# StarsX/RayTracedGGX

Hardware: AMD Instinct MI355X
Metric: Mrays/s + ms/frame, bunny 1920x1080 1spp+denoise, 1/2/4/8 GPUs (higher is better)
Workload: dtype f32; 1 GPU; configs[1]: bunny.obj + rnl_cross env, 1920x1080, 1spp GGX reflection + full denoise chain (refl H,V; diff H,V, shared-memory variant; temporal; tone map), all-metal default materials, dt=1/60; parallelism=row strips x1, history_apron_rows=18, history_overreach_rows=0, setup_priming_frames=256, trace_workgroup_waves=12

## Files before the change

### include/rtggx.h

```cpp
#ifndef RTGGX_H
#define RTGGX_H

#include <stddef.h>
#include <stdint.h>

#ifdef __cplusplus
extern "C" {
#endif

typedef struct rtggx_context rtggx_context;

enum { RTGGX_GROUND = 0, RTGGX_MODEL_OBJ = 1, RTGGX_NUM_MESH = 2 };

typedef struct RtggxCBGlobal {
  float    WorldViewProjs[2][16];
  float    WorldViewProjsPrev[2][16];
  float    Worlds[2][12];
  float    WorldITs0[12];
  float    WorldIT1[11];
  uint32_t FrameIndex;
} RtggxCBGlobal;
typedef struct RtggxRayGenConstants {
  float ProjToWorld[16];
  float EyePt[4];
  float ProjBias[2];
  float pad[2];
} RtggxRayGenConstants;
typedef struct RtggxCBPerObject {
  float WorldViewProj[16];
  float ProjBias[2];
  float pad[2];
} RtggxCBPerObject;
typedef struct RtggxCBMaterial {
  float BaseColors[2][4];
  float RoughMetals[2][4];
} RtggxCBMaterial;
typedef struct RtggxFrameConstants {
  RtggxCBGlobal        global;
  RtggxRayGenConstants rayGen;
  RtggxCBPerObject     perObject[2];
  RtggxCBMaterial      material;
} RtggxFrameConstants;

enum { RTGGX_FORMAT_RGBA32F = 2, RTGGX_FORMAT_RGBA16F = 10, RTGGX_FORMAT_BC6H_UF16 = 95, RTGGX_FORMAT_BC6H_SF16 = 96 };

enum {
  RTGGX_BUF_VISIBILITY = 0,
  RTGGX_BUF_DEPTH = 1,
  RTGGX_BUF_NORMAL = 2,
  RTGGX_BUF_ROUGH_METAL = 3,
  RTGGX_BUF_VELOCITY = 4,
  RTGGX_BUF_RT_REFL = 5,
  RTGGX_BUF_RT_DIFF = 6,
  RTGGX_BUF_TSS0 = 7,
  RTGGX_BUF_TSS1 = 8,
  RTGGX_BUF_FLT_RFL = 9,
  RTGGX_BUF_FLT_DFF = 10,
  RTGGX_BUF_BACKBUFFER = 11,
  RTGGX_BUF_SH_COEFFS = 12,
  RTGGX_BUF_BVH_NODES0 = 13,
  RTGGX_BUF_BVH_TRIS0 = 14,
  RTGGX_BUF_BVH_NODES1 = 15,
  RTGGX_BUF_BVH_TRIS1 = 16,
  RTGGX_BUF_TLAS = 17,
  RTGGX_BUF_ENV = 18,
  RTGGX_BUF_BVH4_NODES0 = 19,
  RTGGX_BUF_BVH4_NODES1 = 20,
  RTGGX_BUF_BIN_WORK = 21,
  RTGGX_BUF_BVH4_TOP0 = 22,
  RTGGX_BUF_BVH4_TOP1 = 23,
  RTGGX_BUF_EXCHANGE_TOKENS = 24,
  RTGGX_BUF_ACC_REFL = 25,
  RTGGX_BUF_ACC_DIFF = 26,
  RTGGX_BUF_CONVERGED = 27,
  RTGGX_BUF_COUNT = 28
};

typedef struct RtggxTimings {
  float update_as, visibility, ray_trace, spatial_refl_h, spatial_refl_v, spatial_diff_h, spatial_diff_v,
        temporal, tone_map, frame,
        ray_trace_kernel;
} RtggxTimings;

const char* rtggx_last_error(void);

int  rtggx_create(rtggx_context** out, uint32_t width, uint32_t height, int device);
void rtggx_destroy(rtggx_context* ctx);

int  rtggx_set_strip(rtggx_context* ctx, uint32_t row_begin, uint32_t row_end);

int  rtggx_set_history_apron(rtggx_context* ctx, uint32_t rows);
int  rtggx_history_overreach(rtggx_context* ctx, uint32_t* rows, int reset);

int  rtggx_set_stream(rtggx_context* ctx, void* hip_stream);
int  rtggx_get_stream(rtggx_context* ctx, void** hip_stream);
#define RTGGX_MAX_PEERS 16
#define RTGGX_IPC_HANDLE_BYTES 64
int  rtggx_set_history_peers(rtggx_context* ctx, uint32_t world, const uint32_t* bounds, void* const* tss0, void* const* tss1);
int  rtggx_history_ipc_export(rtggx_context* ctx, void* handles, size_t bytes);
int  rtggx_history_ipc_open(rtggx_context* ctx, const void* handles, size_t bytes, void** tss0, void** tss1);

int  rtggx_set_async_compute(rtggx_context* ctx, int enable);

int  rtggx_set_mesh(rtggx_context* ctx, uint32_t slot, const float* verts, uint32_t num_verts,
                    const uint32_t* indices, uint32_t num_indices);
int  rtggx_set_env(rtggx_context* ctx, int format, uint32_t size, uint32_t mips, const void* data, size_t bytes);
enum { RTGGX_ENV_EQUIRECT = 0, RTGGX_ENV_VCROSS = 1, RTGGX_ENV_HCROSS = 2 };
enum { RTGGX_PIXELS_RGBE8 = 0, RTGGX_PIXELS_RGB32F = 1 };
int  rtggx_set_env_image(rtggx_context* ctx, int layout, int pixels, uint32_t width, uint32_t height, const void* data, size_t bytes,
                         uint32_t cube_size);
int  rtggx_generate_env_mips(rtggx_context* ctx);
int  rtggx_set_material(rtggx_context* ctx, uint32_t mesh, const float base_color[4], float roughness, float metallic);
int  rtggx_set_metallic(rtggx_context* ctx, uint32_t mesh, float metallic);
int  rtggx_set_sampler(rtggx_context* ctx, int vndf);
int  rtggx_set_ray_rate(rtggx_context* ctx, uint32_t pixels_per_ray);
#define RTGGX_MAX_RECURSION_DEPTH 4u
int  rtggx_set_max_recursion_depth(rtggx_context* ctx, uint32_t depth);
#define RTGGX_MAX_SAMPLES_PER_PIXEL 8u
int  rtggx_set_samples_per_pixel(rtggx_context* ctx, uint32_t samples);
#define RTGGX_MIN_SAMPLE_SET 256u
#define RTGGX_MAX_SAMPLE_SET 65536u
int  rtggx_set_sample_set(rtggx_context* ctx, uint32_t size);
int  rtggx_set_accumulation(rtggx_context* ctx, int enable);
int  rtggx_reset_accumulation(rtggx_context* ctx);
int  rtggx_accumulated_frames(rtggx_context* ctx, uint32_t* frames);
int  rtggx_present_accumulation(rtggx_context* ctx);

typedef struct RtggxScore {
  uint64_t index;
  uint32_t frame_index;
  uint32_t pad;
  uint64_t pixels, covered;
  uint64_t skipped_out, skipped_raw;
  double se_out_rgb, se_out_luma;
  double se_raw_rgb, se_raw_luma;
  double ref_rgb2, ref_luma2;
  double se_out_rgb_cov, se_raw_rgb_cov, ref_rgb2_cov;
} RtggxScore;
enum { RTGGX_SCORE_RING = 256 };
int  rtggx_set_reference(rtggx_context* ctx, const void* rgba16f, size_t bytes);
int  rtggx_reference_from_accumulation(rtggx_context* ctx);
int  rtggx_set_scoring(rtggx_context* ctx, int enable);
int  rtggx_read_scores(rtggx_context* ctx, RtggxScore* out, uint32_t capacity, uint32_t* count);

int  rtggx_build_as(rtggx_context* ctx);

int  rtggx_refit_as(rtggx_context* ctx, uint32_t slot, const float* verts, uint32_t num_verts);
int  rtggx_refit_as_device(rtggx_context* ctx, uint32_t slot, const float* device_verts, uint32_t num_verts, void* hip_stream);
int  rtggx_set_refit_policy(rtggx_context* ctx, float rebuild_ratio, uint32_t steps_per_frame);
int  rtggx_refit_stats(rtggx_context* ctx, uint32_t slot, float* cost_ratio, uint32_t* refits, uint32_t* rebuilds);

int  rtggx_update_frame(rtggx_context* ctx, const RtggxFrameConstants* constants);
int  rtggx_update_as(rtggx_context* ctx);
int  rtggx_transform_sh(rtggx_context* ctx);
int  rtggx_render_visibility(rtggx_context* ctx);
int  rtggx_ray_trace(rtggx_context* ctx);
int  rtggx_denoise(rtggx_context* ctx, int use_shared_mem);
int  rtggx_tone_map(rtggx_context* ctx);

int  rtggx_debug_fuse_tone_map(rtggx_context* ctx, int mode);
int  rtggx_debug_placement(rtggx_context* ctx, int force_small, uint32_t* key, uint32_t* where);
int  rtggx_debug_tile_words(rtggx_context* ctx, int enable);
int  rtggx_debug_static_sky(rtggx_context* ctx, int enable);
int  rtggx_debug_sky_runs(rtggx_context* ctx, uint32_t* runs, uint32_t capacity, uint32_t* tiles_x, uint32_t* tiles_y, uint32_t* threshold);
int  rtggx_debug_collapse_weights(rtggx_context* ctx, const float* set, float* get);
int  rtggx_debug_fence_wait(rtggx_context* ctx, double* us_total, uint32_t* waits, int reset);

int  rtggx_sync(rtggx_context* ctx);
int  rtggx_ray_count(rtggx_context* ctx, uint64_t* rays);
int  rtggx_ray_total(rtggx_context* ctx, uint64_t* rays, int reset);
int  rtggx_debug_counters(rtggx_context* ctx, uint32_t* out, uint32_t n, int reset);
int  rtggx_debug_trace_split(rtggx_context* ctx, uint32_t work_per_wave, uint32_t max_shift, int capacity, uint32_t* last_demand);
int  rtggx_debug_trace_residency(rtggx_context* ctx, uint32_t force_waves, uint32_t* waves, float* share);
int  rtggx_debug_environment(rtggx_context* ctx, const float* dirs3, const float* levels, uint32_t n, int level0_path, float* rgb3);
int  rtggx_get_timings(rtggx_context* ctx, RtggxTimings* out);
#define RTGGX_KERNEL_RING 4096
int  rtggx_enable_timing(rtggx_context* ctx, int mode);
int  rtggx_kernel_times(rtggx_context* ctx, float* ms, uint32_t capacity, uint32_t* count);

int  rtggx_debug_shader_clock(rtggx_context* ctx, double* mhz);

int  rtggx_copy_bandwidth(rtggx_context* ctx, size_t bytes, int iterations, double* gbytes_per_s);

int  rtggx_buffer_size(rtggx_context* ctx, int buffer_id, size_t* bytes);
int  rtggx_readback(rtggx_context* ctx, int buffer_id, void* dst, size_t bytes);
int  rtggx_buffer_ptr(rtggx_context* ctx, int buffer_id, void** device_ptr);
int  rtggx_upload(rtggx_context* ctx, int buffer_id, const void* src, size_t bytes);
int  rtggx_frame_parity(rtggx_context* ctx, uint32_t* parity);
int  rtggx_bvh_root(rtggx_context* ctx, uint32_t slot, int32_t* root);

int  rtggx_trace_rays(rtggx_context* ctx, const float* rays, uint32_t n, float* out);

#ifdef __cplusplus
}
#endif
#endif
```

### raytracedggx_amd/capi.py

```python
import ctypes as C
import os

import numpy as np

_HERE = os.path.dirname(os.path.abspath(__file__))
LIB_PATH = os.path.join(_HERE, "librtggx.so")

BUF_VISIBILITY, BUF_DEPTH, BUF_NORMAL, BUF_ROUGH_METAL, BUF_VELOCITY, BUF_RT_REFL, BUF_RT_DIFF, BUF_TSS0, BUF_TSS1, \
    BUF_FLT_RFL, BUF_FLT_DFF, BUF_BACKBUFFER, BUF_SH_COEFFS, BUF_BVH_NODES0, BUF_BVH_TRIS0, BUF_BVH_NODES1, BUF_BVH_TRIS1, \
    BUF_TLAS, BUF_ENV, BUF_BVH4_NODES0, BUF_BVH4_NODES1, BUF_BIN_WORK, BUF_BVH4_TOP0, BUF_BVH4_TOP1, BUF_EXCHANGE_TOKENS, \
    BUF_ACC_REFL, BUF_ACC_DIFF, BUF_CONVERGED = range(28)
MAX_PEERS, IPC_HANDLE_BYTES = 16, 64
FORMAT_RGBA32F, FORMAT_RGBA16F, FORMAT_BC6H_UF16, FORMAT_BC6H_SF16 = 2, 10, 95, 96
ENV_EQUIRECT, ENV_VCROSS, ENV_HCROSS = 0, 1, 2
PIXELS_RGBE8, PIXELS_RGB32F = 0, 1

_BUF_DTYPE = {BUF_VISIBILITY: np.uint32, BUF_DEPTH: np.uint32, BUF_NORMAL: np.uint32, BUF_ROUGH_METAL: np.uint16,
              BUF_VELOCITY: np.uint32, BUF_RT_REFL: np.uint32, BUF_RT_DIFF: np.uint32, BUF_TSS0: np.uint64, BUF_TSS1: np.uint64,
              BUF_FLT_RFL: np.uint64, BUF_FLT_DFF: np.uint64, BUF_BACKBUFFER: np.uint32, BUF_SH_COEFFS: np.float32,
              BUF_BVH_NODES0: np.uint32, BUF_BVH_TRIS0: np.uint32, BUF_BVH_NODES1: np.uint32, BUF_BVH_TRIS1: np.uint32,
              BUF_TLAS: np.float32, BUF_ENV: np.uint16, BUF_BVH4_NODES0: np.uint32, BUF_BVH4_NODES1: np.uint32, BUF_BIN_WORK: np.uint32,
              BUF_BVH4_TOP0: np.uint32, BUF_BVH4_TOP1: np.uint32, BUF_EXCHANGE_TOKENS: np.uint32,
              BUF_ACC_REFL: np.float32, BUF_ACC_DIFF: np.float32, BUF_CONVERGED: np.uint64}

EXPORTS = ["rtggx_last_error", "rtggx_create", "rtggx_destroy", "rtggx_set_strip", "rtggx_set_stream", "rtggx_set_mesh",
           "rtggx_set_env", "rtggx_set_material", "rtggx_set_metallic", "rtggx_build_as", "rtggx_update_frame", "rtggx_update_as",
           "rtggx_transform_sh", "rtggx_render_visibility", "rtggx_ray_trace", "rtggx_denoise", "rtggx_tone_map", "rtggx_sync",
           "rtggx_ray_count", "rtggx_get_timings", "rtggx_enable_timing", "rtggx_buffer_size", "rtggx_readback", "rtggx_buffer_ptr",
           "rtggx_upload", "rtggx_frame_parity", "rtggx_bvh_root", "rtggx_trace_rays", "rtggx_ray_total", "rtggx_kernel_times", "rtggx_debug_counters", "rtggx_debug_trace_split", "rtggx_debug_trace_residency", "rtggx_get_stream", "rtggx_set_history_peers", "rtggx_history_ipc_export", "rtggx_history_ipc_open",
           "rtggx_set_async_compute", "rtggx_set_history_apron", "rtggx_history_overreach", "rtggx_copy_bandwidth", "rtggx_refit_as", "rtggx_refit_as_device", "rtggx_refit_stats", "rtggx_set_refit_policy", "rtggx_set_sampler", "rtggx_set_ray_rate", "rtggx_set_max_recursion_depth", "rtggx_set_samples_per_pixel", "rtggx_debug_fuse_tone_map", "rtggx_debug_placement", "rtggx_debug_tile_words", "rtggx_debug_static_sky", "rtggx_debug_sky_runs", "rtggx_debug_collapse_weights", "rtggx_debug_fence_wait", "rtggx_debug_shader_clock", "rtggx_debug_environment",
           "rtggx_set_accumulation", "rtggx_reset_accumulation", "rtggx_accumulated_frames", "rtggx_present_accumulation", "rtggx_set_sample_set",
           "rtggx_set_reference", "rtggx_reference_from_accumulation", "rtggx_set_scoring", "rtggx_read_scores",
           "rtggx_set_env_image", "rtggx_generate_env_mips"]
SCORE_RING = 256


class Timings(C.Structure):
    _fields_ = [(n, C.c_float) for n in ("update_as", "visibility", "ray_trace", "spatial_refl_h", "spatial_refl_v",
                                         "spatial_diff_h", "spatial_diff_v", "temporal", "tone_map", "frame", "ray_trace_kernel")]


class Score(C.Structure):
    _fields_ = [("index", C.c_uint64), ("frame_index", C.c_uint32), ("pad", C.c_uint32), ("pixels", C.c_uint64), ("covered", C.c_uint64),
                ("skipped_out", C.c_uint64), ("skipped_raw", C.c_uint64)] + \
               [(n, C.c_double) for n in ("se_out_rgb", "se_out_luma", "se_raw_rgb", "se_raw_luma", "ref_rgb2", "ref_luma2",
                                          "se_out_rgb_cov", "se_raw_rgb_cov", "ref_rgb2_cov")]

    def as_dict(self):
        return {n: getattr(self, n) for n, _ in self._fields_ if n != "pad"}


_lib = None


def load():
    global _lib
    if _lib is not None:
        return _lib
    if not os.path.exists(LIB_PATH):
        raise ImportError("librtggx.so is not built: run `python -c 'import __graft_entry__ as g; g.build()'` "
                          "or `make -C raytracedggx_amd` (hipcc, gfx950). There is no CPU path.")
    L = C.CDLL(LIB_PATH)
    L.rtggx_last_error.restype = C.c_char_p
    vp = C.c_void_p
    L.rtggx_create.argtypes = [C.POINTER(vp), C.c_uint32, C.c_uint32, C.c_int]
    L.rtggx_destroy.argtypes = [vp]
    L.rtggx_destroy.restype = None
    L.rtggx_set_strip.argtypes = [vp, C.c_uint32, C.c_uint32]
    L.rtggx_set_stream.argtypes = [vp, vp]
    L.rtggx_set_async_compute.argtypes = [vp, C.c_int]
    L.rtggx_set_ray_rate.argtypes = [vp, C.c_uint32]
    L.rtggx_set_max_recursion_depth.argtypes = [vp, C.c_uint32]
    L.rtggx_set_samples_per_pixel.argtypes = [vp, C.c_uint32]
    L.rtggx_set_sample_set.argtypes = [vp, C.c_uint32]
    L.rtggx_set_accumulation.argtypes = [vp, C.c_int]
    L.rtggx_reset_accumulation.argtypes = [vp]
    L.rtggx_accumulated_frames.argtypes = [vp, C.POINTER(C.c_uint32)]
    L.rtggx_present_accumulation.argtypes = [vp]
    L.rtggx_set_reference.argtypes = [vp, vp, C.c_size_t]
    L.rtggx_reference_from_accumulation.argtypes = [vp]
    L.rtggx_set_scoring.argtypes = [vp, C.c_int]
    L.rtggx_read_scores.argtypes = [vp, C.POINTER(Score), C.c_uint32, C.POINTER(C.c_uint32)]
    L.rtggx_set_history_apron.argtypes = [vp, C.c_uint32]
    L.rtggx_debug_shader_clock.argtypes = [vp, C.POINTER(C.c_double)]
    L.rtggx_refit_as.argtypes = [vp, C.c_uint32, vp, C.c_uint32]
    L.rtggx_set_refit_policy.argtypes = [vp, C.c_float, C.c_uint32]
    L.rtggx_refit_stats.argtypes = [vp, C.c_uint32, C.POINTER(C.c_float), C.POINTER(C.c_uint32), C.POINTER(C.c_uint32)]
    L.rtggx_copy_bandwidth.argtypes = [vp, C.c_size_t, C.c_int, C.POINTER(C.c_double)]
    L.rtggx_history_overreach.argtypes = [vp, C.POINTER(C.c_uint32), C.c_int]
    L.rtggx_set_mesh.argtypes = [vp, C.c_uint32, vp, C.c_uint32, vp, C.c_uint32]
    L.rtggx_set_env.argtypes = [vp, C.c_int, C.c_uint32, C.c_uint32, vp, C.c_size_t]
    L.rtggx_set_env_image.argtypes = [vp, C.c_int, C.c_int, C.c_uint32, C.c_uint32, vp, C.c_size_t, C.c_uint32]
    L.rtggx_generate_env_mips.argtypes = [vp]
    L.rtggx_set_material.argtypes = [vp, C.c_uint32, vp, C.c_float, C.c_float]
    L.rtggx_set_metallic.argtypes = [vp, C.c_uint32, C.c_float]
    for n in ("rtggx_build_as", "rtggx_update_as", "rtggx_transform_sh", "rtggx_render_visibility", "rtggx_ray_trace",
              "rtggx_tone_map", "rtggx_sync"):
        getattr(L, n).argtypes = [vp]
    L.rtggx_update_frame.argtypes = [vp, vp]
    L.rtggx_denoise.argtypes = [vp, C.c_int]
    L.rtggx_ray_count.argtypes = [vp, C.POINTER(C.c_uint64)]
    L.rtggx_get_timings.argtypes = [vp, C.POINTER(Timings)]
    L.rtggx_enable_timing.argtypes = [vp, C.c_int]
    L.rtggx_buffer_size.argtypes = [vp, C.c_int, C.POINTER(C.c_size_t)]
    L.rtggx_readback.argtypes = [vp, C.c_int, vp, C.c_size_t]
    L.rtggx_buffer_ptr.argtypes = [vp, C.c_int, C.POINTER(vp)]
    L.rtggx_upload.argtypes = [vp, C.c_int, vp, C.c_size_t]
    L.rtggx_frame_parity.argtypes = [vp, C.POINTER(C.c_uint32)]
    L.rtggx_bvh_root.argtypes = [vp, C.c_uint32, C.POINTER(C.c_int32)]
    L.rtggx_trace_rays.argtypes = [vp, vp, C.c_uint32, vp]
    L.rtggx_ray_total.argtypes = [vp, C.POINTER(C.c_uint64), C.c_int]
    L.rtggx_kernel_times.argtypes = [vp, vp, C.c_uint32, C.POINTER(C.c_uint32)]
    _lib = L
    return L


class RtggxError(RuntimeError):
    pass


def _p(a):
    return a.ctypes.data_as(C.c_void_p)


class Context:

    def __init__(self, width, height, device=0):
        self.L = load()
        self.W, self.H = int(width), int(height)
        h = C.c_void_p()
        self._check(self.L.rtggx_create(C.byref(h), self.W, self.H, int(device)))
        self.h = h

    def _check(self, rc):
        if rc != 0:
            raise RtggxError("librtggx: %s (code %d)" % (self.L.rtggx_last_error().decode(), rc))

    def close(self):
        if getattr(self, "h", None):
            self.L.rtggx_destroy(self.h)
            self.h = None

    def __del__(self):
        try:
            self.close()
        except Exception:
            pass

    def set_strip(self, row_begin, row_end):
        self._check(self.L.rtggx_set_strip(self.h, row_begin, row_end))

    def set_stream(self, stream_handle):
        self._check(self.L.rtggx_set_stream(self.h, C.c_void_p(stream_handle)))

    def shader_clock_mhz(self):
        m = C.c_double()
        self._check(self.L.rtggx_debug_shader_clock(self.h, C.byref(m)))
        return m.value

    def copy_bandwidth(self, nbytes=1 << 30, iterations=8):
        g = C.c_double()
        self._check(self.L.rtggx_copy_bandwidth(self.h, int(nbytes), int(iterations), C.byref(g)))
        return g.value

    def set_history_apron(self, rows):
        self._check(self.L.rtggx_set_history_apron(self.h, int(rows)))

    def history_overreach(self, reset=True):
        n = C.c_uint32()
        self._check(self.L.rtggx_history_overreach(self.h, C.byref(n), int(reset)))
        return n.value

    def set_async_compute(self, enable):
        self._check(self.L.rtggx_set_async_compute(self.h, int(bool(enable))))

    def set_mesh(self, slot, verts, indices):
        v = np.ascontiguousarray(verts, np.float32).reshape(-1, 6)
        i = np.ascontiguousarray(indices, np.uint32).reshape(-1)
        self._check(self.L.rtggx_set_mesh(self.h, slot, _p(v), v.shape[0], _p(i), i.size))

    def refit_as(self, slot, verts):
        v = np.ascontiguousarray(verts, np.float32).reshape(-1, 6)
        self._check(self.L.rtggx_refit_as(self.h, slot, _p(v), v.shape[0]))

    def refit_as_device(self, slot, device_ptr, num_verts, stream=0):
        self.L.rtggx_refit_as_device.argtypes = [C.c_void_p, C.c_uint32, C.c_void_p, C.c_uint32, C.c_void_p]
        self._check(self.L.rtggx_refit_as_device(self.h, slot, C.c_void_p(int(device_ptr)), int(num_verts), C.c_void_p(int(stream) or None)))

    def fence_wait(self, reset=True):
        us, n = C.c_double(0.0), C.c_uint32(0)
        self.L.rtggx_debug_fence_wait.argtypes = [C.c_void_p, C.POINTER(C.c_double), C.POINTER(C.c_uint32), C.c_int]
        self._check(self.L.rtggx_debug_fence_wait(self.h, C.byref(us), C.byref(n), 1 if reset else 0))
        return us.value, n.value

    def fuse_tone_map(self, mode):
        self._check(self.L.rtggx_debug_fuse_tone_map(self.h, -1 if mode is None else 1 if mode else 0))

    def tile_words(self, enable):
        self._check(self.L.rtggx_debug_tile_words(self.h, 1 if enable else 0))

    def static_sky(self, enable):
        self._check(self.L.rtggx_debug_static_sky(self.h, 1 if enable else 0))

    def sky_runs(self):
        tiles = ((self.W + 15) // 16) * ((self.H + 15) // 16 + 1)
        runs = np.zeros(tiles, np.uint32)
        tx, ty, th = C.c_uint32(), C.c_uint32(), C.c_uint32()
        self.L.rtggx_debug_sky_runs.argtypes = [C.c_void_p, C.c_void_p, C.c_uint32, C.c_void_p, C.c_void_p, C.c_void_p]
        self._check(self.L.rtggx_debug_sky_runs(self.h, _p(runs), tiles, C.byref(tx), C.byref(ty), C.byref(th)))
        return runs[:tx.value * ty.value].reshape(ty.value, tx.value), int(th.value)

    def placement(self, force_small=-1):
        k, w = C.c_uint32(), C.c_uint32()
        self.L.rtggx_debug_placement.argtypes = [C.c_void_p, C.c_int, C.c_void_p, C.c_void_p]
        self._check(self.L.rtggx_debug_placement(self.h, int(force_small), C.byref(k), C.byref(w)))
        names = ("main", "B", "C", "R", "?")
        key = {n: bool((k.value >> i) & 1) for i, n in enumerate(("small", "strip", "deforming", "diffuse", "caller_stream"))}
        where = {"raster": names[(w.value >> 16) & 15], "gen": names[w.value & 15], "trace": names[(w.value >> 4) & 15], "shade": names[(w.value >> 8) & 15], "frames_in_flight": (w.value >> 12) & 15}
        return key, where

    def collapse_weights(self, area=None, tris=None):
        self.L.rtggx_debug_collapse_weights.argtypes = [C.c_void_p, C.c_void_p, C.c_void_p]
        get = (C.c_float * 2)()
        if area is not None:
            st = (C.c_float * 2)(float(area), float(tris))
            self._check(self.L.rtggx_debug_collapse_weights(self.h, st, get))
        else:
            self._check(self.L.rtggx_debug_collapse_weights(self.h, None, get))
        return float(get[0]), float(get[1])

    def set_history_peers(self, bounds, tss0, tss1):
        self.L.rtggx_set_history_peers.argtypes = [C.c_void_p, C.c_uint32, C.c_void_p, C.c_void_p, C.c_void_p]
        if bounds is None:
            self._check(self.L.rtggx_set_history_peers(self.h, 0, None, None, None))
            return
        world = len(bounds) - 1
        b = (C.c_uint32 * (world + 1))(*[int(x) for x in bounds])
        p0 = (C.c_void_p * world)(*[C.c_void_p(int(x) or None) for x in tss0])
        p1 = (C.c_void_p * world)(*[C.c_void_p(int(x) or None) for x in tss1])
        self._check(self.L.rtggx_set_history_peers(self.h, world, b, p0, p1))

    def history_ipc_export(self):
        self.L.rtggx_history_ipc_export.argtypes = [C.c_void_p, C.c_void_p, C.c_size_t]
        buf = C.create_string_buffer(2 * IPC_HANDLE_BYTES)
        self._check(self.L.rtggx_history_ipc_export(self.h, buf, len(buf.raw)))
        return bytes(buf.raw)

    def history_ipc_open(self, handles):
        self.L.rtggx_history_ipc_open.argtypes = [C.c_void_p, C.c_char_p, C.c_size_t, C.c_void_p, C.c_void_p]
        p0, p1 = C.c_void_p(), C.c_void_p()
        self._check(self.L.rtggx_history_ipc_open(self.h, bytes(handles), len(handles), C.byref(p0), C.byref(p1)))
        return int(p0.value), int(p1.value)

    def set_sampler(self, vndf):
        self._check(self.L.rtggx_set_sampler(self.h, 1 if vndf else 0))

    def set_ray_rate(self, pixels_per_ray):
        self._check(self.L.rtggx_set_ray_rate(self.h, int(pixels_per_ray)))

    def set_max_recursion_depth(self, depth):
        self._check(self.L.rtggx_set_max_recursion_depth(self.h, int(depth)))

    def set_samples_per_pixel(self, samples):
        self._check(self.L.rtggx_set_samples_per_pixel(self.h, int(samples)))

    def set_sample_set(self, size):
        self._check(self.L.rtggx_set_sample_set(self.h, int(size)))

    def set_accumulation(self, enable):
        self._check(self.L.rtggx_set_accumulation(self.h, 1 if enable else 0))

    def reset_accumulation(self):
        self._check(self.L.rtggx_reset_accumulation(self.h))

    def accumulated_frames(self):
        n = C.c_uint32()
        self._check(self.L.rtggx_accumulated_frames(self.h, C.byref(n)))
        return int(n.value)

    def present_accumulation(self):
        self._check(self.L.rtggx_present_accumulation(self.h))

    def set_reference(self, rgba16f):
        if rgba16f is None:
            self._check(self.L.rtggx_set_reference(self.h, None, 0))
            return
        a = np.ascontiguousarray(rgba16f)
        self._check(self.L.rtggx_set_reference(self.h, _p(a), a.nbytes))

    def reference_from_accumulation(self):
        self._check(self.L.rtggx_reference_from_accumulation(self.h))

    def set_scoring(self, enable):
        self._check(self.L.rtggx_set_scoring(self.h, 1 if enable else 0))

    def read_scores(self, capacity=None):
        out = []
        while capacity is None or len(out) < capacity:
            room = SCORE_RING if capacity is None else min(SCORE_RING, capacity - len(out))
            buf, n = (Score * room)(), C.c_uint32()
            self._check(self.L.rtggx_read_scores(self.h, buf, room, C.byref(n)))
            out += [buf[i].as_dict() for i in range(n.value)]
            if n.value < room:
                break
        return out

    def set_refit_policy(self, rebuild_ratio=1.2, steps_per_frame=16):
        self._check(self.L.rtggx_set_refit_policy(self.h, rebuild_ratio, steps_per_frame))

    def refit_stats(self, slot=1):
        ratio, refits, rebuilds = C.c_float(), C.c_uint32(), C.c_uint32()
        self._check(self.L.rtggx_refit_stats(self.h, slot, C.byref(ratio), C.byref(refits), C.byref(rebuilds)))
        return {"cost_ratio": ratio.value, "refits": refits.value, "rebuilds": rebuilds.value}

    def set_env(self, fmt, size, mips, data):
        b = np.frombuffer(bytes(data), np.uint8) if not isinstance(data, np.ndarray) else np.ascontiguousarray(data).view(np.uint8).reshape(-1)
        self._check(self.L.rtggx_set_env(self.h, fmt, size, mips, _p(b), b.size))

    def set_env_image(self, layout, pixels, width, height, data, cube_size=0):
        if data is None:
            self._check(self.L.rtggx_set_env_image(self.h, int(layout), int(pixels), int(width), int(height), None, 0, int(cube_size)))
            return
        b = np.frombuffer(bytes(data), np.uint8) if not isinstance(data, np.ndarray) else np.ascontiguousarray(data).view(np.uint8).reshape(-1)
        self._check(self.L.rtggx_set_env_image(self.h, int(layout), int(pixels), int(width), int(height), _p(b), b.size, int(cube_size)))

    def generate_env_mips(self):
        self._check(self.L.rtggx_generate_env_mips(self.h))

    def set_material(self, mesh, base_color, roughness, metallic):
        bc = np.asarray(base_color, np.float32)
        self._check(self.L.rtggx_set_material(self.h, mesh, _p(bc), roughness, metallic))

    def set_metallic(self, mesh, metallic):
        self._check(self.L.rtggx_set_metallic(self.h, mesh, metallic))

    def build_as(self):
        self._check(self.L.rtggx_build_as(self.h))

    def update_frame(self, constants768):
        b = np.frombuffer(bytes(constants768), np.uint8).copy()
        if b.size != 768:
            raise ValueError("RtggxFrameConstants is 768 bytes")
        self._check(self.L.rtggx_update_frame(self.h, _p(b)))

    def update_as(self):
        self._check(self.L.rtggx_update_as(self.h))

    def transform_sh(self):
        self._check(self.L.rtggx_transform_sh(self.h))

    def render_visibility(self):
        self._check(self.L.rtggx_render_visibility(self.h))

    def ray_trace(self):
        self._check(self.L.rtggx_ray_trace(self.h))

    def denoise(self, use_shared_mem=False):
        self._check(self.L.rtggx_denoise(self.h, 1 if use_shared_mem else 0))

    def tone_map(self):
        self._check(self.L.rtggx_tone_map(self.h))

    def sync(self):
        self._check(self.L.rtggx_sync(self.h))

    def ray_count(self):
        n = C.c_uint64()
        self._check(self.L.rtggx_ray_count(self.h, C.byref(n)))
        return int(n.value)

    def ray_total(self, reset=False):
        n = C.c_uint64()
        self._check(self.L.rtggx_ray_total(self.h, C.byref(n), 1 if reset else 0))
        return int(n.value)

    def debug_trace_split(self, work_per_wave, max_shift, capacity=-1):
        d = C.c_uint32()
        self.L.rtggx_debug_trace_split.argtypes = [C.c_void_p, C.c_uint32, C.c_uint32, C.c_int, C.c_void_p]
        self._check(self.L.rtggx_debug_trace_split(self.h, work_per_wave, max_shift, capacity, C.byref(d)))
        return int(d.value)

    def stream(self):
        h = C.c_void_p()
        self.L.rtggx_get_stream.argtypes = [C.c_void_p, C.c_void_p]
        self._check(self.L.rtggx_get_stream(self.h, C.byref(h)))
        return int(h.value or 0)

    def trace_residency(self, force_waves=0):
        w, sh = C.c_uint32(), C.c_float()
        self.L.rtggx_debug_trace_residency.argtypes = [C.c_void_p, C.c_uint32, C.c_void_p, C.c_void_p]
        self._check(self.L.rtggx_debug_trace_residency(self.h, force_waves, C.byref(w), C.byref(sh)))
        return int(w.value), float(sh.value)

    def debug_counters(self, n=8, reset=True):
        out = np.zeros(n, np.uint32)
        self.L.rtggx_debug_counters.argtypes = [C.c_void_p, C.c_void_p, C.c_uint32, C.c_int]
        self._check(self.L.rtggx_debug_counters(self.h, _p(out), n, 1 if reset else 0))
        return out

    def debug_environment(self, dirs, levels, level0=False):
        d = np.ascontiguousarray(dirs, np.float32).reshape(-1, 3)
        lv = np.ascontiguousarray(np.broadcast_to(np.asarray(levels, np.float32), (d.shape[0],)))
        out = np.zeros((d.shape[0], 3), np.float32)
        self.L.rtggx_debug_environment.argtypes = [C.c_void_p, C.c_void_p, C.c_void_p, C.c_uint32, C.c_int, C.c_void_p]
        self._check(self.L.rtggx_debug_environment(self.h, _p(d), _p(lv), d.shape[0], 1 if level0 else 0, _p(out)))
        return out

    def enable_timing(self, mode=1):
        self._check(self.L.rtggx_enable_timing(self.h, int(mode)))

    def kernel_times(self):
        ms = np.zeros(4096, np.float32)
        n = C.c_uint32()
        self._check(self.L.rtggx_kernel_times(self.h, _p(ms), ms.size, C.byref(n)))
        return ms[:n.value].copy()

    def timings(self):
        t = Timings()
        self._check(self.L.rtggx_get_timings(self.h, C.byref(t)))
        return {n: getattr(t, n) for n, _ in Timings._fields_}

    def buffer_size(self, bid):
        n = C.c_size_t()
        self._check(self.L.rtggx_buffer_size(self.h, bid, C.byref(n)))
        return int(n.value)

    def buffer_ptr(self, bid):
        p = C.c_void_p()
        self._check(self.L.rtggx_buffer_ptr(self.h, bid, C.byref(p)))
        return int(p.value)

    def readback(self, bid):
        n = self.buffer_size(bid)
        dt = np.dtype(_BUF_DTYPE[bid])
        out = np.zeros(max(n // dt.itemsize, 0), dt)
        if n:
            self._check(self.L.rtggx_readback(self.h, bid, _p(out), n))
        if bid <= BUF_BACKBUFFER or bid == BUF_CONVERGED:
            return out.reshape(self.H, self.W)
        if bid in (BUF_ACC_REFL, BUF_ACC_DIFF):
            return out.reshape(self.H, self.W, 4)
        if bid == BUF_SH_COEFFS:
            return out.reshape(9, 3)
        if bid in (BUF_BVH_NODES0, BUF_BVH_NODES1):
            return out.reshape(-1, 16)
        if bid in (BUF_BVH_TRIS0, BUF_BVH_TRIS1):
            return out.reshape(-1, 16)
        if bid == BUF_TLAS:
            return out.reshape(2, 4, 4)
        if bid == BUF_ENV:
            return out.reshape(-1, 4)
        if bid in (BUF_BVH4_NODES0, BUF_BVH4_NODES1, BUF_BVH4_TOP0, BUF_BVH4_TOP1):
            return out.reshape(-1, 32)
        return out

    def upload(self, bid, array):
        a = np.ascontiguousarray(array)
        self._check(self.L.rtggx_upload(self.h, bid, _p(a), a.nbytes))

    def frame_parity(self):
        p = C.c_uint32()
        self._check(self.L.rtggx_frame_parity(self.h, C.byref(p)))
        return int(p.value)

    def bvh_root(self, slot):
        r = C.c_int32()
        self._check(self.L.rtggx_bvh_root(self.h, slot, C.byref(r)))
        return int(r.value)

    def trace_rays(self, rays):
        r = np.ascontiguousarray(rays, np.float32).reshape(-1, 8)
        out = np.zeros((r.shape[0], 6), np.float32)
        self._check(self.L.rtggx_trace_rays(self.h, _p(r), r.shape[0], _p(out)))
        return {"t": out[:, 0].copy(), "inst": out[:, 1].copy().view(np.uint32), "prim": out[:, 2].copy().view(np.uint32),
                "b1": out[:, 3].copy(), "b2": out[:, 4].copy(), "valid": out[:, 5] > 0.5}
```

### raytracedggx_amd/csrc/context.hip

```cpp
#include <cstdarg>
#include <cstdio>
#include <cstring>
#include <cmath>
#include <vector>
#include "capi_internal.h"
#include "rt_queue.h"

#ifndef RT_REFIT_REBUILD_RATIO
#define RT_REFIT_REBUILD_RATIO 1.2f
#endif
#ifndef RT_REBUILD_STEPS
#define RT_REBUILD_STEPS 16u
#endif
namespace rt {
static thread_local char g_err[512] = "";
void setError(const char* fmt, ...) {
  va_list ap; va_start(ap, fmt); vsnprintf(g_err, sizeof g_err, fmt, ap); va_end(ap);
}

__global__ void uploadParamsKernel(FrameParams src, FrameParams* dst) {
  const uint32_t* s = reinterpret_cast<const uint32_t*>(&src);
  uint32_t* d = reinterpret_cast<uint32_t*>(dst);
  for (uint32_t i = threadIdx.x; i < sizeof(FrameParams) / 4; i += blockDim.x) d[i] = s[i];
}
int uploadParams(rtggx_context* c, uint32_t slot, hipStream_t s) {
  hipLaunchKernelGGL(uploadParamsKernel, dim3(1), dim3(64), 0, s, c->slots[slot], c->dParams + slot);
  RT_HIP(hipGetLastError());
  return 0;
}
int allocSet(rtggx_context* c, uint32_t i) {
  InputSet& s = c->sets[i];
  const size_t n = (size_t)c->W * c->H, slots = (size_t)c->numBinsMax * c->binSlots;
  for (DevBuf<uint32_t>* p : {&s.normal, &s.depth32, &s.velocity, &s.rtRefl, &s.rtDiff}) if (!*p) RT_HIP(allocFilled(*p, n));
  if (!s.roughMetal) RT_HIP(allocFilled(s.roughMetal, n));
  if (!s.rayQueue) RT_HIP(alloc(s.rayQueue, slots * sizeof(rt::RayRec)));
  if (!s.hitQueue) RT_HIP(alloc(s.hitQueue, slots * 8));
  if (!s.binCount) RT_HIP(allocFilled(s.binCount, (size_t)c->numBinsMax));
  if (!s.splitList) RT_HIP(alloc(s.splitList, (size_t)RT_SPLIT_CAP));
  if (!s.skyRun) RT_HIP(allocFilled(s.skyRun, c->skyTiles));
  c->breakSkyRuns();
  s.splitCount = c->largeCountBase + 2 + i;
  if (!s.evRead) RT_HIP(create(s.evRead, RT_EVENT_FLAGS));
  return 0;
}

static int initContext(rtggx_context* c, uint32_t width, uint32_t height, int device) {
  c->device = device; c->W = width; c->H = height; c->rowBegin = 0; c->rowEnd = height;
  const size_t n = (size_t)width * height;
  int prioLeast = 0, prioGreatest = 0;
  RT_HIP(hipDeviceGetStreamPriorityRange(&prioLeast, &prioGreatest));
  const int prioMid = (prioLeast + prioGreatest) / 2;
  RT_HIP(create(c->ownMain, hipStreamNonBlocking, prioGreatest));
  RT_HIP(create(c->ownAS, hipStreamNonBlocking, prioLeast));
  c->streamMain = c->ownMain; c->streamAS = c->ownAS;
  RT_HIP(create(c->ownVis, hipStreamNonBlocking, prioLeast)); c->streamVis = c->ownVis;
  RT_HIP(create(c->streamRefit, hipStreamNonBlocking, prioMid));
  for (Event* e : {&c->evVis, &c->evRefit, &c->evAS, &c->evRT}) RT_HIP(create(*e, RT_EVENT_FLAGS));
  for (auto& f : c->frames) { RT_HIP(create(f.gen, RT_EVENT_FLAGS)); RT_HIP(create(f.trace, RT_EVENT_FLAGS)); }
  for (auto& e : c->tev) RT_HIP(create(e));
  c->rebuildRatio = RT_REFIT_REBUILD_RATIO; c->rebuildSteps = RT_REBUILD_STEPS;
  {
    hipDeviceProp_t prop;
    RT_HIP(hipGetDeviceProperties(&prop, device));
    c->numCUs = prop.multiProcessorCount > 0 ? (uint32_t)prop.multiProcessorCount : 256u;
  }
  c->numBinsMax = ((width + 15) / 16) * ((height + 15) / 16) * 4u;
  if (c->numBinsMax < 64u) c->numBinsMax = 64u;
  c->binSlots = RT_BIN_MIN;
  c->largeCapacity = 1u << 16;
  c->skyTiles = (size_t)((width + 15) / 16) * ((height + 15) / 16 + 1);
  for (auto& b : c->largeTrisBuf) RT_HIP(alloc(b, (size_t)c->largeCapacity * 56));
  RT_HIP(allocFilled(c->largeCountBase, 2 + RT_SETS));
  for (uint32_t i = 0; i < RT_SETS; ++i) { const int r = allocSet(c, i); if (r) return r; }
  for (auto& v : c->vis) { RT_HIP(allocFilled(v.depth, n)); RT_HIP(allocFilled(v.dirty, c->skyTiles, 0xFF)); }
  RT_HIP(allocFilled(c->visDirtyOnes, c->skyTiles, 0xFF));
  RT_HIP(allocFilled(c->backbuffer, n));
  RT_HIP(allocFilled(c->tss[0], n)); RT_HIP(allocFilled(c->tss[1], n)); RT_HIP(allocFilled(c->fltRfl, n)); RT_HIP(allocFilled(c->fltDff, n));
  RT_HIP(allocFilled(c->rayCounter, 512));
  RT_HIP(allocFilled(c->rayCounterBuf, 1792));
  c->lastRayCounter32 = c->rayCounterBuf;
  RT_HIP(allocFilled(c->traceStamps, 8));
  RT_HIP(alloc(c->hostRayCounters, 264)); memset(c->hostRayCounters, 0, 264 * 4); RT_HIP(create(c->evRayCounters, hipEventDisableTiming));
  for (auto& b : c->binWorkBuf) RT_HIP(allocFilled(b, (size_t)c->numBinsMax));
  c->selectSet(0);
  c->splitWork = RT_SPLIT_WORK; c->splitMaxShift = RT_SPLIT_MAX_SHIFT;
  RT_HIP(allocFilled(c->dEnvMipOffset, 16));
  RT_HIP(allocFilled(c->dummyRecord, 128));
  RT_HIP(allocFilled(c->histReach, 1));
  RT_HIP(allocFilled(c->exchangeTokens, 2 * RT_MAX_PEERS));
  RT_HIP(allocFilled(c->dPeerTable, sizeof(void*) * 2 * RT_MAX_PEERS + 4 * (RT_MAX_PEERS + 1)));
  RT_HIP(allocFilled(c->sh, 27));
  RT_HIP(alloc(c->cosSinTab, 512));
  RT_HIP(alloc(c->dParams, RT_SLOTS));
  {
    float tab[512];
    for (int s = 0; s < 256; ++s) { const double phi = 2.0 * 3.14159265358979323846 * (double)s / 256.0; tab[s] = (float)cos(phi); tab[256 + s] = (float)sin(phi); }
    RT_HIP(hipMemcpy(c->cosSinTab, tab, sizeof tab, hipMemcpyHostToDevice));
  }
  const float bc0[4] = {0.95f, 0.93f, 0.88f, 1.0f}, bc1[4] = {1.0f, 0.71f, 0.29f, 1.0f};
  const float rm0[4] = {0.5f, 1.0f, 0.0f, 0.0f}, rm1[4] = {0.16f, 1.0f, 0.0f, 0.0f};
  memcpy(c->material.BaseColors[0], bc0, 16); memcpy(c->material.BaseColors[1], bc1, 16);
  memcpy(c->material.RoughMetals[0], rm0, 16); memcpy(c->material.RoughMetals[1], rm1, 16);
  memset(c->invWorld, 0, sizeof c->invWorld);
  for (int i = 0; i < 2; ++i) for (int k = 0; k < 4; ++k) c->invWorld[i][k * 5] = 1.0f;
  memset(c->slots, 0, sizeof c->slots);
  { const int r = setMeshImpl(c, RTGGX_GROUND, &kGroundVerts[0][0], 24, kGroundIdx, 36); if (r) return r; }
  RT_HIP(hipStreamSynchronize(nullptr));
  return 0;
}
int allocSamples(rtggx_context* c) {
  if (c->sppAcc && c->sppParams) return 0;
  const size_t n = (size_t)c->W * c->H;
  if (!c->evSpp) RT_HIP(create(c->evSpp, hipEventDisableTiming));
  if (!c->sppParams) RT_HIP(alloc(c->sppParams, RT_SLOTS * RTGGX_MAX_SAMPLES_PER_PIXEL));
  if (!c->sppAcc) {
    RT_HIP(allocFilled(c->sppAcc, n * 2u * 3u));
    RT_HIP(hipStreamSynchronize(nullptr));
  }
  return 0;
}
int allocSampleTable(rtggx_context* c, uint32_t m) {
  DevBuf<float>& tab = c->cosSinWide[rtggx_context::sampleSetSlot(m)];
  if (tab) return 0;
  std::vector<float> host(2u * (size_t)m);
  for (uint32_t s = 0; s < m; ++s) { const double phi = 2.0 * 3.14159265358979323846 * (double)s / (double)m; host[2u * s] = (float)cos(phi); host[2u * s + 1u] = (float)sin(phi); }
  DevBuf<float> d;
  hipError_t e = alloc(d, host.size());
  if (e == hipSuccess) e = hipMemcpy(d, host.data(), host.size() * sizeof(float), hipMemcpyHostToDevice);
  if (e != hipSuccess) { setError("rtggx_set_sample_set: %s (%zu bytes for the table of %u samples)", hipGetErrorString(e), host.size() * sizeof(float), m); return -2; }
  tab = std::move(d);
  return 0;
}
int allocAccumulation(rtggx_context* c) {
  if (c->accRefl) return 0;
  const size_t n = (size_t)c->W * c->H;
  DevBuf<float4> a0, a1; DevBuf<uint2> cv;
  hipError_t e = alloc(a0, n);
  if (e == hipSuccess) e = alloc(a1, n);
  if (e == hipSuccess) e = alloc(cv, n);
  if (e == hipSuccess) e = hipMemset(a0, 0, n * 16);
  if (e == hipSuccess) e = hipMemset(a1, 0, n * 16);
  if (e == hipSuccess) e = hipMemset(cv, 0, n * 8);
  if (e == hipSuccess) e = hipStreamSynchronize(nullptr);
  if (e != hipSuccess) { setError("rtggx_set_accumulation: %s (%zu bytes for the sums and the mean image)", hipGetErrorString(e), n * 40); return -2; }
  c->accRefl = std::move(a0); c->accDiff = std::move(a1); c->converged = std::move(cv);
  return 0;
}
static int allocReference(rtggx_context* c, const char* who) {
  if (c->reference) return 0;
  const size_t n = (size_t)c->W * c->H;
  const hipError_t e = alloc(c->reference, n);
  if (e != hipSuccess) { setError("%s: %s (%zu bytes for the reference image)", who, hipGetErrorString(e), n * 8); return -2; }
  return 0;
}
static int allocScoring(rtggx_context* c) {
  if (c->scoreRing) return 0;
  const size_t chunks = ((size_t)c->W * c->H + RT_SCORE_CHUNK - 1u) / RT_SCORE_CHUNK;
  uint32_t stride = 1u; while (stride < chunks) stride <<= 1;
  const size_t half = stride > 1u ? stride / 2u : 1u;
  DevBuf<double> p0, p1; DevBuf<uint32_t> counts; DevBuf<RtggxScore> ring;
  hipError_t e = alloc(p0, (size_t)RT_SCORE_SUMS * stride);
  if (e == hipSuccess) e = alloc(p1, (size_t)RT_SCORE_SUMS * half);
  if (e == hipSuccess) e = alloc(counts, 3u * (size_t)stride);
  if (e == hipSuccess) e = allocFilled(ring, RTGGX_SCORE_RING);
  if (e == hipSuccess) e = hipStreamSynchronize(nullptr);
  if (e != hipSuccess) { setError("rtggx_set_scoring: %s (the ring of records and the partial sums)", hipGetErrorString(e)); return -2; }
  c->scorePartial[0] = std::move(p0); c->scorePartial[1] = std::move(p1); c->scoreCounts = std::move(counts); c->scoreRing = std::move(ring); c->scoreStride = stride;
  return 0;
}
}
using namespace rt;

extern "C" {
const char* rtggx_last_error(void) { return rt::g_err; }

int rtggx_create(rtggx_context** out, uint32_t width, uint32_t height, int device) {
  if (!out || width == 0 || height == 0 || width > 16384 || height > 16384) { setError("rtggx_create: bad arguments"); return -1; }
  int count = 0;
  if (hipGetDeviceCount(&count) != hipSuccess || count <= 0) { setError("rtggx_create: no HIP device available (this library has no CPU path)"); return -2; }
  if (device < 0 || device >= count) { setError("rtggx_create: device %d out of range (%d devices)", device, count); return -1; }
  RT_HIP(hipSetDevice(device));
  rtggx_context* c = new rtggx_context();
  const int r = initContext(c, width, height, device);
  if (r) { rtggx_destroy(c); return r; }
  *out = c;
  return 0;
}

void rtggx_destroy(rtggx_context* c) {
  if (!c) return;
  hipSetDevice(c->device);
  hipDeviceSynchronize();
  delete c;
}

int rtggx_set_strip(rtggx_context* c, uint32_t rowBegin, uint32_t rowEnd) {
  RT_CHECK_CTX(c);
  if (rowBegin > rowEnd || rowEnd > c->H) { setError("rtggx_set_strip: bad rows [%u,%u) for height %u", rowBegin, rowEnd, c->H); return -1; }
  if (c->rayRate != 1u && (rowBegin > 0u || rowEnd < c->H)) { setError("rtggx_set_strip: rows [%u,%u) of %u: a context tracing one pixel in %u renders whole frames", rowBegin, rowEnd, c->H, c->rayRate); return -1; }
  c->rowBegin = rowBegin; c->rowEnd = rowEnd; c->toneMapDone = false;
  c->breakSkyRuns();
  return 0;
}

int rtggx_set_history_apron(rtggx_context* c, uint32_t rows) {
  RT_CHECK_CTX(c);
  c->historyApron = rows;
  return 0;
}
int rtggx_history_overreach(rtggx_context* c, uint32_t* rows, int reset) {
  RT_CHECK_CTX(c);
  if (!rows) { setError("rtggx_history_overreach: null result"); return -1; }
  RT_HIP(syncStreams(c));
  RT_HIP(hipMemcpy(rows, c->histReach, 4, hipMemcpyDeviceToHost));
  if (reset) { RT_HIP(hipMemset(c->histReach, 0, 4)); RT_HIP(hipStreamSynchronize(nullptr)); }
  return 0;
}

int rtggx_set_stream(rtggx_context* c, void* stream) {
  RT_CHECK_CTX(c);
  RT_HIP(syncStreams(c));
  if (stream) { c->streamMain = (hipStream_t)stream; c->externalStream = true; }
  else { c->streamMain = c->ownMain; c->externalStream = false; }
  c->sppStream = nullptr;
  if (!c->asyncCompute) c->streamAS = c->streamMain;
  return 0;
}

int rtggx_set_history_peers(rtggx_context* c, uint32_t world, const uint32_t* bounds, void* const* tss0, void* const* tss1) {
  RT_CHECK_CTX(c);
  if (world == 0u) { RT_HIP(syncStreams(c)); c->peerWorld = 0u; return 0; }
  if (world > RT_MAX_PEERS || !bounds || !tss0 || !tss1) { setError("rtggx_set_history_peers: 1 .. %d ranks, boundaries and two pointer lists", RT_MAX_PEERS); return -1; }
  if (bounds[0] != 0u || bounds[world] != c->H) { setError("rtggx_set_history_peers: boundaries must run from 0 to the frame height %u", c->H); return -1; }
  for (uint32_t r = 0; r < world; ++r) if (bounds[r] > bounds[r + 1]) { setError("rtggx_set_history_peers: boundaries must ascend"); return -1; }
  RT_HIP(syncStreams(c));
  struct { const void* tss[2][RT_MAX_PEERS]; uint32_t bounds[RT_MAX_PEERS + 1]; } table;
  memset(&table, 0, sizeof table);
  for (uint32_t r = 0; r < world; ++r) {
    const bool own = bounds[r] <= c->rowBegin && c->rowEnd <= bounds[r + 1] && c->rowEnd > c->rowBegin;
    table.tss[0][r] = tss0[r] ? tss0[r] : own ? (void*)c->tss[0] : nullptr; table.tss[1][r] = tss1[r] ? tss1[r] : own ? (void*)c->tss[1] : nullptr;
    if (bounds[r + 1] > bounds[r] && (!table.tss[0][r] || !table.tss[1][r])) { setError("rtggx_set_history_peers: no history images for rank %u", r); return -1; }
  }
  for (uint32_t r = 0; r <= world; ++r) table.bounds[r] = bounds[r];
  for (uint32_t r = world + 1; r <= RT_MAX_PEERS; ++r) table.bounds[r] = c->H;
  static_assert(sizeof table == sizeof(void*) * 2 * RT_MAX_PEERS + 4 * (RT_MAX_PEERS + 1) + 4 || sizeof table == sizeof(void*) * 2 * RT_MAX_PEERS + 4 * (RT_MAX_PEERS + 1), "peer table layout");
  RT_HIP(hipMemcpy(c->dPeerTable, &table, sizeof(void*) * 2 * RT_MAX_PEERS + 4 * (RT_MAX_PEERS + 1), hipMemcpyHostToDevice));
  c->peerWorld = world;
  return 0;
}
int rtggx_history_ipc_export(rtggx_context* c, void* handles, size_t bytes) {
  RT_CHECK_CTX(c);
  static_assert(sizeof(hipIpcMemHandle_t) == RTGGX_IPC_HANDLE_BYTES, "hipIpcMemHandle_t size");
  if (!handles || bytes < 2 * sizeof(hipIpcMemHandle_t)) { setError("rtggx_history_ipc_export: room for two %zu-byte handles", sizeof(hipIpcMemHandle_t)); return -1; }
  hipIpcMemHandle_t h[2];
  for (int p = 0; p < 2; ++p) RT_HIP(hipIpcGetMemHandle(&h[p], c->tss[p]));
  memcpy(handles, h, sizeof h);
  return 0;
}
int rtggx_history_ipc_open(rtggx_context* c, const void* handles, size_t bytes, void** tss0, void** tss1) {
  RT_CHECK_CTX(c);
  if (!handles || bytes < 2 * sizeof(hipIpcMemHandle_t) || !tss0 || !tss1) { setError("rtggx_history_ipc_open: bad arguments"); return -1; }
  hipIpcMemHandle_t h[2]; memcpy(h, handles, sizeof h);
  void* p[2] = {nullptr, nullptr};
  for (int k = 0; k < 2; ++k) {
    IpcMapping mapped;
    RT_HIP(hipIpcOpenMemHandle(mapped.put(), h[k], hipIpcMemLazyEnablePeerAccess));
    p[k] = mapped;
    c->ipcMapped.push_back(std::move(mapped));
  }
  *tss0 = p[0]; *tss1 = p[1];
  return 0;
}

int rtggx_get_stream(rtggx_context* c, void** stream) {
  RT_CHECK_CTX(c);
  if (!stream) { setError("rtggx_get_stream: null"); return -1; }
  *stream = (void*)c->streamMain;
  return 0;
}

int rtggx_set_async_compute(rtggx_context* c, int enable) {
  RT_CHECK_CTX(c);
  if ((enable != 0) == c->asyncCompute) return 0;
  RT_HIP(syncStreams(c));
  c->asyncCompute = enable != 0; c->sppStream = nullptr;
  c->streamAS = c->asyncCompute ? c->ownAS : c->streamMain;
  c->streamVis = c->asyncCompute ? c->ownVis : nullptr;
  c->evVisStream = nullptr; for (auto& f : c->frames) f.genFrame = 0u;
  return 0;
}

int rtggx_set_ray_rate(rtggx_context* c, uint32_t pixelsPerRay) {
  RT_CHECK_CTX(c);
  if (pixelsPerRay != 1u && pixelsPerRay != 4u) { setError("rtggx_set_ray_rate: %u pixels per ray: 1 or 4", pixelsPerRay); return -1; }
  if (pixelsPerRay != 1u && c->samplesRequested > 1u) { setError("rtggx_set_ray_rate: rate %u on a context tracing %u samples per pixel (rtggx_set_samples_per_pixel): one asks for fewer rays, the other for more", pixelsPerRay, c->samplesRequested); return -1; }
  if (pixelsPerRay != 1u && c->accumulateRequested) { setError("rtggx_set_ray_rate: rate %u on an accumulating context (rtggx_set_accumulation): three quarters of such a frame are interpolations", pixelsPerRay); return -1; }
  if (pixelsPerRay != 1u && (c->rowBegin > 0u || c->rowEnd < c->H)) { setError("rtggx_set_ray_rate: rate %u on a strip (rows [%u,%u) of %u): whole frames only", pixelsPerRay, c->rowBegin, c->rowEnd, c->H); return -1; }
  if (pixelsPerRay == c->rayRate) return 0;
  RT_HIP(syncStreams(c));
  c->rayRate = pixelsPerRay;
  for (auto& b : c->binWorkBuf) RT_HIP(hipMemset(b, 0, (size_t)c->numBinsMax * 4));
  RT_HIP(hipDeviceSynchronize());
  c->splitDemand = 0u; c->rayCountersInFlight = false; c->lastFrameRays = 0xFFFFFFFFu; c->traceLaunches = 0u;
  return 0;
}

int rtggx_set_max_recursion_depth(rtggx_context* c, uint32_t depth) {
  RT_CHECK_CTX(c);
  if (depth < 1u || depth > RTGGX_MAX_RECURSION_DEPTH) { setError("rtggx_set_max_recursion_depth: depth %u: 1 to %u", depth, RTGGX_MAX_RECURSION_DEPTH); return -1; }
  c->depthRequested = depth;
  return 0;
}

int rtggx_set_samples_per_pixel(rtggx_context* c, uint32_t samples) {
  RT_CHECK_CTX(c);
  if (samples != 1u && samples != 2u && samples != 4u && samples != 8u) { setError("rtggx_set_samples_per_pixel: %u samples per pixel: 1, 2, 4 or %u", samples, RTGGX_MAX_SAMPLES_PER_PIXEL); return -1; }
  if (samples > 1u && c->rayRate != 1u) { setError("rtggx_set_samples_per_pixel: %u samples per pixel on a context tracing one pixel in %u (rtggx_set_ray_rate): one asks for more rays, the other for fewer", samples, c->rayRate); return -1; }
  if (samples > 1u) { const int r = allocSamples(c); if (r) return r; }
  c->samplesRequested = samples;
  return 0;
}

int rtggx_set_sample_set(rtggx_context* c, uint32_t size) {
  RT_CHECK_CTX(c);
  if (size < RTGGX_MIN_SAMPLE_SET || size > RTGGX_MAX_SAMPLE_SET || (size & (size - 1u)) != 0u) { setError("rtggx_set_sample_set: %u samples: a power of two from %u to %u", size, RTGGX_MIN_SAMPLE_SET, RTGGX_MAX_SAMPLE_SET); return -1; }
  if (size == c->sampleSetRequested) return 0;
  RT_HIP(syncStreams(c));
  if (size > RTGGX_MIN_SAMPLE_SET) { const int r = allocSampleTable(c, size); if (r) return r; }
  c->sampleSetRequested = size;
  return 0;
}

int rtggx_set_accumulation(rtggx_context* c, int enable) {
  RT_CHECK_CTX(c);
  if (enable && c->rayRate != 1u) { setError("rtggx_set_accumulation: on a context tracing one pixel in %u (rtggx_set_ray_rate): three quarters of such a frame are interpolations", c->rayRate); return -1; }
  if (enable) { const int r = allocAccumulation(c); if (r) return r; }
  c->accumulateRequested = enable != 0;
  return 0;
}
int rtggx_reset_accumulation(rtggx_context* c) {
  RT_CHECK_CTX(c);
  if (c->accRefl) {
    const size_t n = (size_t)c->W * c->H;
    RT_HIP(hipMemsetAsync(c->accRefl, 0, n * 16, c->streamMain));
    RT_HIP(hipMemsetAsync(c->accDiff, 0, n * 16, c->streamMain));
  }
  c->accumFrames = 0u;
  return 0;
}
int rtggx_accumulated_frames(rtggx_context* c, uint32_t* frames) {
  RT_CHECK_CTX(c);
  if (!frames) { setError("rtggx_accumulated_frames: null result"); return -1; }
  *frames = c->accumFrames;
  return 0;
}
int rtggx_present_accumulation(rtggx_context* c) {
  RT_CHECK_CTX(c);
  if (!c->accRefl) { setError("rtggx_present_accumulation: accumulation was never enabled (rtggx_set_accumulation)"); return -1; }
  if (c->rowBegin > 0u || c->rowEnd < c->H) { setError("rtggx_present_accumulation: on a strip (rows [%u,%u) of %u): whole frames only", c->rowBegin, c->rowEnd, c->H); return -1; }
  if (c->accumFrames == 0u) { setError("rtggx_present_accumulation: no frame has been accumulated"); return -1; }
  FrameParams fp = c->slots[c->slot];
  fp.W = c->W; fp.H = c->H; fp.rowBegin = 0u; fp.rowEnd = c->H;
  int r = launchPresentAccumulation(c, c->streamMain);
  if (!r) r = launchToneMap(c, fp, c->streamMain, nullptr, c->converged);
  c->toneMapDone = false;
  return r;
}

int rtggx_set_reference(rtggx_context* c, const void* rgba16f, size_t bytes) {
  RT_CHECK_CTX(c);
  const size_t want = (size_t)c->W * c->H * 8u;
  if (!rgba16f && bytes == 0u) {
    RT_HIP(syncStreams(c));
    c->reference.reset();
    c->scoring = c->scoringRequested = false;
    return 0;
  }
  if (!rgba16f || bytes != want) { setError("rtggx_set_reference: %zu bytes for a %u x %u RGBA16F image of %zu", bytes, c->W, c->H, want); return -1; }
// ... 106 lines not shown
```

### raytracedggx_amd/csrc/debug.hip

```cpp
#include <cstring>
#include "capi_internal.h"
#include "rt_queue.h"
namespace rt {
__global__ void __launch_bounds__(256) copyKernel(const float4* __restrict__ src, float4* __restrict__ dst, size_t n) {
  for (size_t i = (size_t)blockIdx.x * 256u + threadIdx.x; i < n; i += (size_t)gridDim.x * 256u) dst[i] = src[i];
}
typedef float __attribute__((ext_vector_type(4))) CopyVec4;
__global__ void __launch_bounds__(256) copyKernelNT(const CopyVec4* __restrict__ src, CopyVec4* __restrict__ dst, size_t n) {
  for (size_t i = (size_t)blockIdx.x * 256u + threadIdx.x; i < n; i += (size_t)gridDim.x * 256u) __builtin_nontemporal_store(__builtin_nontemporal_load(&src[i]), &dst[i]);
}
}
using namespace rt;

extern "C" {
int rtggx_ray_count(rtggx_context* c, uint64_t* rays) {
  RT_CHECK_CTX(c);
  uint32_t h[256];
  RT_HIP(syncStreams(c));
  RT_HIP(hipMemcpy(h, c->lastRayCounter32, sizeof h, hipMemcpyDeviceToHost));
  uint64_t s = 0; for (auto v : h) s += v;
  *rays = s;
  return 0;
}

int rtggx_debug_counters(rtggx_context* c, uint32_t* out, uint32_t n, int reset) {
  RT_CHECK_CTX(c);
  if (n > 768) { setError("rtggx_debug_counters: at most 768 words"); return -1; }
  RT_HIP(syncStreams(c));
  RT_HIP(hipMemcpy(out, c->rayCounterBuf + 1024, (size_t)n * 4, hipMemcpyDeviceToHost));
  if (reset) { RT_HIP(hipMemset(c->rayCounterBuf + 1024, 0, 768 * 4)); RT_HIP(hipStreamSynchronize(nullptr)); }
  return 0;
}

int rtggx_debug_fence_wait(rtggx_context* c, double* usTotal, uint32_t* waits, int reset) {
  RT_CHECK_CTX(c);
  if (usTotal) *usTotal = c->fenceWaitUs;
  if (waits) *waits = c->fenceWaits;
  if (reset) { c->fenceWaitUs = 0.0; c->fenceWaits = 0u; }
  return 0;
}
int rtggx_debug_fuse_tone_map(rtggx_context* c, int mode) {
  RT_CHECK_CTX(c);
  c->fuseToneMap = mode < 0 ? -1 : mode != 0;
  return 0;
}
int rtggx_debug_tile_words(rtggx_context* c, int enable) {
  RT_CHECK_CTX(c);
  c->useTileWords = enable != 0;
  c->breakSkyRuns();
  return 0;
}
int rtggx_debug_static_sky(rtggx_context* c, int enable) {
  RT_CHECK_CTX(c);
  c->staticSky = enable != 0;
  c->breakSkyRuns();
  return 0;
}
int rtggx_debug_sky_runs(rtggx_context* c, uint32_t* runs, uint32_t capacity, uint32_t* tilesX, uint32_t* tilesY, uint32_t* threshold) {
  RT_CHECK_CTX(c);
  const uint32_t n = c->skyGen.tilesX * c->skyGen.tilesY;
  if (!runs || capacity < n || n > c->skyTiles) { setError("rtggx_debug_sky_runs: room for %u words", n); return -1; }
  RT_HIP(syncStreams(c));
  if (n) RT_HIP(hipMemcpy(runs, c->cur().skyRun, (size_t)n * 4, hipMemcpyDeviceToHost));
  for (uint32_t i = 0; i < n; ++i) runs[i] = (runs[i] >> 8) == c->skyEpoch ? runs[i] & 0xFFu : 0u;
  if (tilesX) *tilesX = c->skyGen.tilesX;
  if (tilesY) *tilesY = c->skyGen.tilesY;
  if (threshold) *threshold = RT_SKY_PREV_RUN + 1u;
  return 0;
}
int rtggx_debug_placement(rtggx_context* c, int forceSmall, uint32_t* key, uint32_t* where) {
  RT_CHECK_CTX(c);
  if (forceSmall < -1 || forceSmall > 1) { setError("rtggx_debug_placement: force_small is -1, 0 or 1"); return -1; }
  c->forcePlacement = forceSmall;
  if (forceSmall >= 0) c->lastTraceSmall = forceSmall == 1;
  if (key) *key = c->lastPlacement[0];
  if (where) *where = c->lastPlacement[1];
  return 0;
}
int rtggx_debug_collapse_weights(rtggx_context* c, const float* set, float* get) {
  RT_CHECK_CTX(c);
  if (set) { if (!(set[0] >= 0.0f) || !(set[1] >= 0.0f) || !(set[0] + set[1] > 0.0f)) { setError("rtggx_debug_collapse_weights: two non-negative weights, not both zero"); return -1; }
             c->collapseWeights[0] = set[0]; c->collapseWeights[1] = set[1]; }
  if (get) { get[0] = c->collapseWeights[0]; get[1] = c->collapseWeights[1]; }
  return 0;
}
int rtggx_debug_trace_residency(rtggx_context* c, uint32_t forceWaves, uint32_t* waves, float* share) {
  RT_CHECK_CTX(c);
  if (forceWaves != 0u && forceWaves != 10u && forceWaves != 12u && forceWaves != 14u && forceWaves != 16u) { setError("rtggx_debug_trace_residency: %u waves: 0, 10, 12, 14 or 16", forceWaves); return -1; }
  c->traceWavesForced = forceWaves;
  if (forceWaves) c->traceWaves = forceWaves;
  if (waves) *waves = c->traceWaves;
  if (share) *share = c->traceShare;
  return 0;
}

int rtggx_debug_environment(rtggx_context* c, const float* dirs3, const float* levels, uint32_t n, int level0Path, float* rgb3) {
  RT_CHECK_CTX(c);
  if (!c->env.texels) { setError("rtggx_debug_environment: no environment map"); return -1; }
  if (n == 0 || !dirs3 || !rgb3 || (!levels && !level0Path)) { setError("rtggx_debug_environment: no directions, levels or result (n %u)", n); return -1; }
  DevBuf<float> dD, dL, dO;
  hipError_t e = alloc(dD, (size_t)n * 3);
  if (e == hipSuccess) e = alloc(dO, (size_t)n * 3);
  if (e == hipSuccess && levels) e = alloc(dL, (size_t)n);
  if (e == hipSuccess) e = hipMemcpy(dD, dirs3, (size_t)n * 12, hipMemcpyHostToDevice);
  if (e == hipSuccess && levels) e = hipMemcpy(dL, levels, (size_t)n * 4, hipMemcpyHostToDevice);
  int r = 0;
  if (e == hipSuccess) r = launchDebugEnvironment(c, dD, dL, n, level0Path, dO, c->streamMain);
  if (e == hipSuccess && !r) e = hipStreamSynchronize(c->streamMain);
  if (e == hipSuccess && !r) e = hipMemcpy(rgb3, dO, (size_t)n * 12, hipMemcpyDeviceToHost);
  if (e != hipSuccess) { setError("rtggx_debug_environment: %s", hipGetErrorString(e)); return -2; }
  return r;
}

int rtggx_debug_trace_split(rtggx_context* c, uint32_t workPerWave, uint32_t maxShift, int capacity, uint32_t* lastDemand) {
  RT_CHECK_CTX(c);
  if (maxShift > 3u) { setError("rtggx_debug_trace_split: max_shift %u > 3", maxShift); return -1; }
  if (capacity > (int)RT_SPLIT_CAP) { setError("rtggx_debug_trace_split: capacity %d > %u", capacity, RT_SPLIT_CAP); return -1; }
  RT_HIP(syncStreams(c));
  if (lastDemand) RT_HIP(hipMemcpy(lastDemand, c->cur().splitCount, 4, hipMemcpyDeviceToHost));
  c->splitWork = workPerWave; c->splitMaxShift = maxShift;
  c->splitCapForced = capacity < 0 ? 0xFFFFFFFFu : ((uint32_t)capacity / 32u) * 32u;
  return 0;
}

int rtggx_ray_total(rtggx_context* c, uint64_t* rays, int reset) {
  RT_CHECK_CTX(c);
  unsigned long long h[256];
  RT_HIP(syncStreams(c));
  RT_HIP(hipMemcpy(h, c->rayCounter + 256, sizeof h, hipMemcpyDeviceToHost));
  uint64_t s = 0; for (auto v : h) s += v;
  *rays = s;
  if (reset) { RT_HIP(hipMemset(c->rayCounter + 256, 0, sizeof h)); RT_HIP(hipStreamSynchronize(nullptr)); }
  return 0;
}

int rtggx_enable_timing(rtggx_context* c, int mode) {
  RT_CHECK_CTX(c);
  c->timing = mode == 1; c->timingsPending = false;
  c->kernelRing = mode == 2 || mode == 3; c->kevCount = 0; c->ringStride = mode == 3 ? 8u : 1u; c->ringTick = 0;
  if (c->kernelRing && c->kevBegin.empty()) {
    c->kevBegin.resize(RTGGX_KERNEL_RING); c->kevEnd.resize(RTGGX_KERNEL_RING);
    for (uint32_t i = 0; i < RTGGX_KERNEL_RING; ++i) { RT_HIP(create(c->kevBegin[i])); RT_HIP(create(c->kevEnd[i])); }
  }
  return 0;
}
int rtggx_kernel_times(rtggx_context* c, float* ms, uint32_t capacity, uint32_t* count) {
  RT_CHECK_CTX(c);
  RT_HIP(syncStreams(c));
  const uint32_t n = c->kevCount < capacity ? c->kevCount : capacity;
  for (uint32_t i = 0; i < n; ++i) RT_HIP(hipEventElapsedTime(&ms[i], c->kevBegin[i], c->kevEnd[i]));
  *count = n;
  c->kevCount = 0;
  return 0;
}
int rtggx_get_timings(rtggx_context* c, RtggxTimings* out) {
  RT_CHECK_CTX(c);
  if (!c->timing || !c->timingsPending) { setError("rtggx_get_timings: timing not enabled or no complete frame"); return -1; }
  RT_HIP(syncStreams(c));
  auto ms = [&](int a, int b) { float t = 0.0f; hipEventElapsedTime(&t, c->tev[a], c->tev[b]); return t; };
  RtggxTimings t;
  t.update_as = ms(0, 1); t.visibility = ms(2, 13); t.ray_trace = ms(3, 14); t.spatial_refl_h = ms(9, 4); t.spatial_refl_v = ms(4, 5);
  t.spatial_diff_h = ms(5, 6); t.spatial_diff_v = ms(6, 7); t.temporal = ms(7, 8); t.tone_map = ms(8, 10); t.frame = ms(2, 10);
  t.ray_trace_kernel = ms(11, 12);
  *out = t;
  return 0;
}

static int bufferInfo(rtggx_context* c, int id, void** ptr, size_t* bytes) {
  const size_t n = (size_t)c->W * c->H;
  switch (id) {
    case RTGGX_BUF_VISIBILITY: case RTGGX_BUF_DEPTH: *ptr = nullptr; *bytes = n * 4; return 0;
    case RTGGX_BUF_NORMAL: *ptr = c->cur().normal; *bytes = n * 4; return 0;
    case RTGGX_BUF_ROUGH_METAL: *ptr = c->cur().roughMetal; *bytes = n * 2; return 0;
    case RTGGX_BUF_VELOCITY: *ptr = c->cur().velocity; *bytes = n * 4; return 0;
    case RTGGX_BUF_RT_REFL: *ptr = c->cur().rtRefl; *bytes = n * 4; return 0;
    case RTGGX_BUF_RT_DIFF: *ptr = c->cur().rtDiff; *bytes = n * 4; return 0;
    case RTGGX_BUF_TSS0: *ptr = c->tss[0]; *bytes = n * 8; return 0;
    case RTGGX_BUF_TSS1: *ptr = c->tss[1]; *bytes = n * 8; return 0;
    case RTGGX_BUF_FLT_RFL: *ptr = c->fltRflIsFltDff ? c->fltDff.get() : c->fltRfl.get(); *bytes = n * 8; return 0;
    case RTGGX_BUF_FLT_DFF: *ptr = c->fltDff; *bytes = n * 8; return 0;
    case RTGGX_BUF_BACKBUFFER: *ptr = c->backbuffer; *bytes = n * 4; return 0;
    case RTGGX_BUF_SH_COEFFS: *ptr = c->sh; *bytes = 108; return 0;
    case RTGGX_BUF_BVH_NODES0: case RTGGX_BUF_BVH_NODES1: { const MeshDev& m = c->mesh[id == RTGGX_BUF_BVH_NODES1]; *ptr = m.nodes; *bytes = m.numTris > 1 && m.nodes ? (size_t)(m.numTris - 1) * 64 : 0; return 0; }
    case RTGGX_BUF_BVH_TRIS0: case RTGGX_BUF_BVH_TRIS1: { const MeshDev& m = c->mesh[id == RTGGX_BUF_BVH_TRIS1]; *ptr = m.tris; *bytes = m.tris ? (size_t)m.numTris * 64 : 0; return 0; }
    case RTGGX_BUF_TLAS: *ptr = nullptr; *bytes = 128; return 0;
    case RTGGX_BUF_BVH4_NODES0: case RTGGX_BUF_BVH4_NODES1: { const MeshDev& m = c->mesh[id == RTGGX_BUF_BVH4_NODES1]; *ptr = m.nodes4; *bytes = m.numTris > 1 && m.nodes4 ? (size_t)(m.numTris - 1) * sizeof(Bvh4Node) : 0; return 0; }
    case RTGGX_BUF_BVH4_TOP0: case RTGGX_BUF_BVH4_TOP1: { const MeshDev& m = c->mesh[id == RTGGX_BUF_BVH4_TOP1]; *ptr = m.top; *bytes = m.top ? (size_t)m.topCount * sizeof(Bvh4Node) : 0; return 0; }
    case RTGGX_BUF_BIN_WORK: *ptr = c->binWork; *bytes = (size_t)(((c->W + 15) / 16) * ((c->H + 15) / 16)) * 4u * 4u; return 0;
    case RTGGX_BUF_ENV: *ptr = c->env.texels; *bytes = (size_t)c->env.totalTexels * 8; return 0;
    case RTGGX_BUF_EXCHANGE_TOKENS: *ptr = c->exchangeTokens; *bytes = 4 * 2 * RT_MAX_PEERS; return 0;
    case RTGGX_BUF_ACC_REFL: case RTGGX_BUF_ACC_DIFF: case RTGGX_BUF_CONVERGED:
      if (!c->accRefl) { setError("buffer %d exists once accumulation has been enabled (rtggx_set_accumulation)", id); return -1; }
      *ptr = id == RTGGX_BUF_ACC_REFL ? (void*)c->accRefl : id == RTGGX_BUF_ACC_DIFF ? (void*)c->accDiff : (void*)c->converged;
      *bytes = n * (id == RTGGX_BUF_CONVERGED ? 8u : 16u); return 0;
    default: setError("unknown buffer id %d", id); return -1;
  }
}

int rtggx_buffer_size(rtggx_context* c, int id, size_t* bytes) { RT_CHECK_CTX(c); void* p; return bufferInfo(c, id, &p, bytes); }

int rtggx_buffer_ptr(rtggx_context* c, int id, void** dptr) {
  RT_CHECK_CTX(c);
  size_t bytes;
  const int r = bufferInfo(c, id, dptr, &bytes);
  if (r) return r;
  if (id == RTGGX_BUF_VISIBILITY || id == RTGGX_BUF_DEPTH) *dptr = c->curVis().depth;
  if (!*dptr) { setError("buffer %d has no device storage", id); return -1; }
  return 0;
}

int rtggx_readback(rtggx_context* c, int id, void* dst, size_t bytes) {
  RT_CHECK_CTX(c);
  void* p; size_t need;
  int r = bufferInfo(c, id, &p, &need);
  if (r) return r;
  if (bytes < need) { setError("rtggx_readback: buffer %d needs %zu bytes, %zu given", id, need, bytes); return -1; }
  RT_HIP(syncStreams(c));
  if (id == RTGGX_BUF_TLAS) { memcpy(dst, c->invWorld, 128); return 0; }
  if (id == RTGGX_BUF_VISIBILITY || id == RTGGX_BUF_DEPTH) {
    DevBuf<uint32_t> dVis, dDepth;
    RT_HIP(alloc(dVis, need / 4)); RT_HIP(alloc(dDepth, need / 4));
    r = unpackVisDepth(c, dVis, dDepth, c->streamMain);
    if (!r && hipStreamSynchronize(c->streamMain) != hipSuccess) { setError("readback: stream sync failed"); r = -2; }
    if (!r) { hipError_t e = hipMemcpy(dst, id == RTGGX_BUF_VISIBILITY ? dVis.get() : dDepth.get(), need, hipMemcpyDeviceToHost); if (e != hipSuccess) { setError("hipMemcpy: %s", hipGetErrorString(e)); r = -2; } }
    return r;
  }
  if (need == 0) return 0;
  RT_HIP(hipMemcpy(dst, p, need, hipMemcpyDeviceToHost));
  return 0;
}

int rtggx_upload(rtggx_context* c, int id, const void* src, size_t bytes) {
  RT_CHECK_CTX(c);
  void* p; size_t need;
  int r = bufferInfo(c, id, &p, &need);
  if (r) return r;
  if (bytes != need) { setError("rtggx_upload: buffer %d is %zu bytes, %zu given", id, need, bytes); return -1; }
  RT_HIP(syncStreams(c));
  c->toneMapDone = false;
  c->curVis().flags.rasterFrame = 0u;
  c->breakSkyRuns();
  if (id == RTGGX_BUF_VISIBILITY || id == RTGGX_BUF_DEPTH) {
    DevBuf<uint32_t> dVis, dDepth;
    RT_HIP(alloc(dVis, need / 4)); RT_HIP(alloc(dDepth, need / 4));
    r = unpackVisDepth(c, dVis, dDepth, c->streamMain);
    if (!r && hipStreamSynchronize(c->streamMain) != hipSuccess) { setError("upload: stream sync failed"); r = -2; }
    if (!r) { hipError_t e = hipMemcpy(id == RTGGX_BUF_VISIBILITY ? dVis.get() : dDepth.get(), src, need, hipMemcpyHostToDevice); if (e != hipSuccess) { setError("hipMemcpy: %s", hipGetErrorString(e)); r = -2; } }
    if (!r) r = packVisDepth(c, dVis, dDepth, c->streamMain);
    if (!r && id == RTGGX_BUF_DEPTH && hipMemcpy(c->cur().depth32, src, need, hipMemcpyHostToDevice) != hipSuccess) { setError("upload: depth copy failed"); r = -2; }
    hipStreamSynchronize(c->streamMain);
    return r;
  }
  if (id == RTGGX_BUF_SH_COEFFS) c->shDone = true;
  if (!p || id >= RTGGX_BUF_BVH_NODES0) { setError("rtggx_upload: buffer %d is not writable", id); return -1; }
  RT_HIP(hipMemcpy(p, src, need, hipMemcpyHostToDevice));
  return 0;
}

static const uint32_t kCopyShapes[] = {2u, 4u, 8u, 16u};
int rtggx_copy_bandwidth(rtggx_context* c, size_t bytes, int iterations, double* gbytesPerS) {
  RT_CHECK_CTX(c);
  if (!gbytesPerS || bytes < 1024 || iterations < 1) { setError("rtggx_copy_bandwidth: bad arguments"); return -1; }
  RT_HIP(syncStreams(c));
  const size_t n = bytes / 16;
  DevBuf<float4> src, dst;
  RT_HIP(alloc(src, n));
  if (alloc(dst, n) != hipSuccess) { setError("rtggx_copy_bandwidth: out of device memory"); return -2; }
  hipMemsetAsync(src, 0x3C, n * 16, c->streamMain);
  Event e0, e1; RT_HIP(create(e0)); RT_HIP(create(e1));
  hipError_t e = hipSuccess;
  double best = 0.0;
  for (uint32_t shape : kCopyShapes) {
    const uint32_t blocks = c->numCUs * shape;
    for (int nt = 0; nt < 2 && e == hipSuccess; ++nt) {
      const auto launch = [&]() { if (nt) hipLaunchKernelGGL(copyKernelNT, dim3(blocks), dim3(256), 0, c->streamMain, (const CopyVec4*)src.get(), (CopyVec4*)dst.get(), n);
                                  else hipLaunchKernelGGL(copyKernel, dim3(blocks), dim3(256), 0, c->streamMain, (const float4*)src, dst.get(), n); };
      for (int i = 0; i < 2; ++i) launch();
      hipEventRecord(e0, c->streamMain);
      for (int i = 0; i < iterations; ++i) launch();
      hipEventRecord(e1, c->streamMain);
      e = hipEventSynchronize(e1);
      float ms = 0.0f;
      if (e == hipSuccess) e = hipEventElapsedTime(&ms, e0, e1);
      if (e != hipSuccess || !(ms > 0.0f)) { if (e == hipSuccess) e = hipErrorUnknown; break; }
      const double rate = 2.0 * (double)(n * 16) * iterations / ((double)ms * 1e-3) / 1e9;
      if (rate > best) best = rate;
    }
    if (e != hipSuccess) break;
  }
  if (e != hipSuccess) { setError("rtggx_copy_bandwidth: %s", hipGetErrorString(e)); return -2; }
  *gbytesPerS = best;
  return 0;
}

__global__ void clockProbeKernel(unsigned long long* out) {
  const unsigned long long c0 = __builtin_amdgcn_s_memtime(), r0 = __builtin_amdgcn_s_memrealtime();
  unsigned long long r1 = r0;
  while (r1 - r0 < 2000ull) { __builtin_amdgcn_s_sleep(32); r1 = __builtin_amdgcn_s_memrealtime(); }
  const unsigned long long c1 = __builtin_amdgcn_s_memtime();
  if (threadIdx.x == 0) { out[0] = c1 - c0; out[1] = r1 - r0; }
}
int rtggx_debug_shader_clock(rtggx_context* c, double* mhz) {
  RT_CHECK_CTX(c);
  if (!mhz) { setError("rtggx_debug_shader_clock: null result"); return -1; }
  DevBuf<unsigned long long> d; unsigned long long h[2] = {0, 1};
  RT_HIP(alloc(d, 2));
  hipLaunchKernelGGL(clockProbeKernel, dim3(1), dim3(64), 0, c->streamRefit, d.get());
  RT_HIP(hipMemcpyAsync(h, d, 16, hipMemcpyDeviceToHost, c->streamRefit));
  RT_HIP(hipStreamSynchronize(c->streamRefit));
  *mhz = (double)h[0] / (double)h[1] * 100.0;
  return 0;
}

int rtggx_frame_parity(rtggx_context* c, uint32_t* parity) { RT_CHECK_CTX(c); *parity = c->frameParity; return 0; }
int rtggx_bvh_root(rtggx_context* c, uint32_t slot, int32_t* root) { RT_CHECK_CTX(c); if (slot > 1) { setError("bad slot"); return -1; } *root = c->mesh[slot].root; return 0; }

int rtggx_trace_rays(rtggx_context* c, const float* rays, uint32_t n, float* out) {
  RT_CHECK_CTX(c);
  if (!c->asBuilt || !c->haveConstants) { setError("rtggx_trace_rays: build_as / update_frame / update_as first"); return -1; }
  RT_HIP(syncStreams(c));
  c->breakSkyRuns();
  { const int r = ensureParams(c); if (r) return r; }
  DevBuf<float> dR, dO;
  RT_HIP(alloc(dR, (size_t)n * 8)); RT_HIP(alloc(dO, (size_t)n * 6));
  RT_HIP(hipMemcpy(dR, rays, (size_t)n * 32, hipMemcpyHostToDevice));
  int r = 0;
  const uint32_t perLaunch = c->numBinsMax * c->binSlots;
  for (uint32_t done = 0; done < n && !r; done += perLaunch) {
    const uint32_t m = n - done < perLaunch ? n - done : perLaunch;
    r = launchTraceRays(c, c->slots[c->slot], dR + (size_t)done * 8, m, dO + (size_t)done * 6, c->streamMain);
  }
  if (!r) { hipError_t e = hipStreamSynchronize(c->streamMain); if (e == hipSuccess) e = hipMemcpy(out, dO, (size_t)n * 24, hipMemcpyDeviceToHost); if (e != hipSuccess) { setError("trace_rays: %s", hipGetErrorString(e)); r = -2; } }
  return r;
}

}
```

### raytracedggx_amd/csrc/denoise.hip

```cpp
#include <cstring>
#include <type_traits>
#include "rtggx_context.h"

namespace rt {

#define RT_RADIUS 16
#ifndef RT_VBW
#define RT_VBW 16
#define RT_VBH 16
#endif

RT_DEV float rcpFast(float x) { return __builtin_amdgcn_rcpf(x); }

struct GTexel { float nx, ny, nz, nw, rough, metal, depth; };

RT_DEV GTexel loadG(const uint32_t* __restrict__ normal, const uint16_t* __restrict__ roughMetal, const uint32_t* __restrict__ depth32,
                    int x, int y, int W, int H) {
  GTexel g;
  if (x < 0 || y < 0 || x >= W || y >= H) { g.nx = g.ny = g.nz = -1023.0f; g.nw = 0.0f; g.rough = 0.0f; g.metal = 0.0f; g.depth = 0.0f; return g; }
  const size_t i = (size_t)y * W + x;
  const uint32_t n = normal[i];
  g.nx = (float)(2 * (int)(n & 1023u) - 1023);
  g.ny = (float)(2 * (int)((n >> 10) & 1023u) - 1023);
  g.nz = (float)(2 * (int)((n >> 20) & 1023u) - 1023);
  g.nw = (float)(n >> 30) * (1.0f / 3.0f);
  const uint32_t rm = roughMetal[i];
  g.rough = (float)(rm & 0xFFu) * (1.0f / 255.0f); g.metal = (rm >> 8) == 255u ? 1.0f : (float)(rm >> 8) * (1.0f / 255.0f);
  g.depth = (float)depth32[i] * (1.0f / 16777215.0f);
  return g;
}
RT_DEV f3 TM3(f3 c) { const float r = rcpFast(1.0f + ((c.x * 0.25f + c.y * 0.5f) + c.z * 0.25f)); return mk3(c.x * r, c.y * r, c.z * r); }
RT_DEV f3 ITM3(f3 c) { const float r = rcpFast(1.0f - ((c.x * 0.25f + c.y * 0.5f) + c.z * 0.25f)); return mk3(c.x * r, c.y * r, c.z * r); }
struct Targets {
  const uint32_t* normal; const uint16_t* roughMetal; const uint32_t* depth32; const uint32_t* velocity;
  const uint32_t* rtRefl; const uint32_t* rtDiff;
  uint2* scratch; const uint2* history; uint2* fltRfl; uint2* fltDff; uint32_t* backbuffer;
  int W, H, rowBegin, rowEnd;
  int histLo, histHi; uint32_t* histReach;
  const uint2* const* peerHist; const uint32_t* peerBounds; int peerWorld;
  int outBegin, outEnd;
  const uint32_t* tileWords; int tilesX, tileRow0;
  const uint32_t* skyRun; uint32_t skyEpoch;
};
#define RT_SGPR(v) ((uint32_t)__builtin_amdgcn_readfirstlane((int)(v)))
RT_DEV uint32_t tileWordsOr(const uint32_t* words, uint32_t i0, uint32_t i1, uint32_t i2, uint32_t i3) {
  uint32_t a, b, c, d;
  asm volatile("s_load_dword %0, %4, %5\n\ts_load_dword %1, %4, %6\n\ts_load_dword %2, %4, %7\n\ts_load_dword %3, %4, %8\n\ts_waitcnt lgkmcnt(0)"
               : "=&s"(a), "=&s"(b), "=&s"(c), "=&s"(d) : "s"(words), "s"(RT_SGPR(i0 * 4u)), "s"(RT_SGPR(i1 * 4u)), "s"(RT_SGPR(i2 * 4u)), "s"(RT_SGPR(i3 * 4u)) : "memory");
  return a | b | c | d;
}

RT_DEV uint32_t tileWordsOr6(const uint32_t* words, uint32_t i0, uint32_t i1, uint32_t i2, uint32_t i3, uint32_t i4, uint32_t i5) {
  uint32_t a, b, c, d, e, f;
  asm volatile("s_load_dword %0, %6, %7\n\ts_load_dword %1, %6, %8\n\ts_load_dword %2, %6, %9\n\ts_load_dword %3, %6, %10\n\ts_load_dword %4, %6, %11\n\ts_load_dword %5, %6, %12\n\ts_waitcnt lgkmcnt(0)"
               : "=&s"(a), "=&s"(b), "=&s"(c), "=&s"(d), "=&s"(e), "=&s"(f)
               : "s"(words), "s"(RT_SGPR(i0 * 4u)), "s"(RT_SGPR(i1 * 4u)), "s"(RT_SGPR(i2 * 4u)), "s"(RT_SGPR(i3 * 4u)), "s"(RT_SGPR(i4 * 4u)), "s"(RT_SGPR(i5 * 4u)) : "memory");
  return a | b | c | d | e | f;
}
RT_DEV uint32_t skyRunMin6(const uint32_t* words, uint32_t epoch, uint32_t i0, uint32_t i1, uint32_t i2, uint32_t i3, uint32_t i4, uint32_t i5) {
  uint32_t w[6];
  asm volatile("s_load_dword %0, %6, %7\n\ts_load_dword %1, %6, %8\n\ts_load_dword %2, %6, %9\n\ts_load_dword %3, %6, %10\n\ts_load_dword %4, %6, %11\n\ts_load_dword %5, %6, %12\n\ts_waitcnt lgkmcnt(0)"
               : "=&s"(w[0]), "=&s"(w[1]), "=&s"(w[2]), "=&s"(w[3]), "=&s"(w[4]), "=&s"(w[5])
               : "s"(words), "s"(RT_SGPR(i0 * 4u)), "s"(RT_SGPR(i1 * 4u)), "s"(RT_SGPR(i2 * 4u)), "s"(RT_SGPR(i3 * 4u)), "s"(RT_SGPR(i4 * 4u)), "s"(RT_SGPR(i5 * 4u)) : "memory");
  uint32_t run = 0xFFu;
#pragma unroll
  for (int k = 0; k < 6; ++k) run = min(run, (w[k] >> 8) == epoch ? w[k] & 0xFFu : 0u);
  return run;
}

#define RT_LOG2E 1.44269504088896341f

struct Centre { float nx, ny, nz, depth, rough, gaussK , depthK ; };
#define RT_NORMAL_SCALE_SQ 1046529.0f
RT_DEV float log2OfDot(float I) {
  const float d = fmaxf((I - RT_NORMAL_SCALE_SQ) * (1.0f / RT_NORMAL_SCALE_SQ), -1.0f);
  const float xr = 1.0f + d;
  const float dropped = (1.0f - xr) + d;
  return __builtin_fmaf(dropped, RT_LOG2E, __builtin_amdgcn_logf(xr));
}
template <bool DIFFUSE, int UNIFORM = 0>
RT_DEV float tapWeight(const Centre& c, int i, float nx, float ny, float nz, float depth, float rough) {
#pragma clang fp contract(fast)
  const float I = __builtin_fmaf(c.nz, nz, __builtin_fmaf(c.ny, ny, c.nx * nx));
  const float lg = log2OfDot(I);
  const float dd = fabsf(c.depth - depth) * c.depthK;
  if (DIFFUSE) return __builtin_amdgcn_exp2f(__builtin_fmaf(32.0f, lg, -dd));
  const float pw = 512.0f * lg;
  const float e = __builtin_fmaf(c.gaussK, (float)(i * i), -dd);
  const float w = __builtin_amdgcn_exp2f(pw >= 128.0f ? pw : pw + e);
  if (UNIFORM == 2) return w;
  const float flag = (__float_as_uint(rough) >> 31) ? 0.0f : 1.0f;
  if (UNIFORM == 1) return w * flag;
  const float t = saturatef(fabsf(fabsf(rough) - c.rough) * 2.0f);
  return (w * (1.0f - t * t * (3.0f - 2.0f * t))) * flag;
}
template <bool DIFFUSE>
RT_DEV Centre makeCentre(float nx, float ny, float nz, float depth, float rough, int W, int H) {
  Centre c; c.nx = nx; c.ny = ny; c.nz = nz; c.depth = depth; c.rough = rough;
  const int br = DIFFUSE ? 0 : (int)clampf(0.1f * rough * (float)W, 0.0f, (float)H * 0.05f);
  const float sigma = (float)(br + 1) * (1.0f / 3.0f);
  c.gaussK = (-0.5f * RT_LOG2E) * rcpFast(sigma * sigma);
  c.depthK = depth * (4.0f * RT_LOG2E);
  return c;
}
template <int MODE>
RT_DEV void storeFiltered(const Targets& T, size_t pix, float mx, float my, float mz, float wsum) {
  const float rw = rcpFast(wsum);
  f3 mu = mk3(mx * rw, my * rw, mz * rw);
  if (MODE == 0 || MODE == 2) T.scratch[pix] = packRGBA16F(mu.x, mu.y, mu.z, 0.0f);
  if (MODE == 1) { mu = ITM3(mu); const uint2 v = packRGBA16F(mu.x, mu.y, mu.z, 1.0f); if (T.fltRfl) T.fltRfl[pix] = v; T.fltDff[pix] = v; }
  if (MODE == 3) {
    const f4 dest = unpackRGBA16F(T.fltRfl[pix]);
    mu = ITM3(mu);
    T.fltDff[pix] = packRGBA16F(dest.x + mu.x, dest.y + mu.y, dest.z + mu.z, dest.w);
  }
}
template <int MODE>
RT_DEV void storeSkipped(const Targets& T, size_t pix) {
  if (MODE == 1) { const f3 s = unpackR11G11B10F(T.rtRefl[pix]); const uint2 v = packRGBA16F(s.x, s.y, s.z, 0.0f); if (T.fltRfl) T.fltRfl[pix] = v; T.fltDff[pix] = v; }
}
template <int MODE>
RT_DEV f3 tapColour(const Targets& T, size_t ti) {
  if (MODE & 1) { const f4 v = unpackRGBA16F(T.scratch[ti]); return mk3(v.x, v.y, v.z); }
  return TM3(unpackR11G11B10F(MODE >= 2 ? T.rtDiff[ti] : T.rtRefl[ti]));
}

template <int MODE>
__global__ void __launch_bounds__(256) spatialDirectKernel(Targets T) {
  constexpr bool vertical = (MODE & 1) != 0;
  constexpr bool diffuse = MODE >= 2;
  const int x = blockIdx.x * 64 + (threadIdx.x & 63);
  const int y = T.rowBegin + blockIdx.y * 4 + (threadIdx.x >> 6);
  if (x >= T.W || y >= T.rowEnd) return;
  const size_t pix = (size_t)y * T.W + x;
  const GTexel gc = loadG(T.normal, T.roughMetal, T.depth32, x, y, T.W, T.H);
  if (diffuse ? (gc.nw <= 0.0f || gc.metal >= 1.0f) : (gc.nw <= 0.0f)) { storeSkipped<MODE>(T, pix); return; }
  const Centre c = makeCentre<diffuse>(gc.nx, gc.ny, gc.nz, gc.depth, gc.rough, T.W, T.H);
  float mx = 0.0f, my = 0.0f, mz = 0.0f, wsum = 0.0f;
  for (int i = -RT_RADIUS; i <= RT_RADIUS; ++i) {
    const int tx = vertical ? x : x + i, ty = vertical ? y + i : y;
    const bool inside = tx >= 0 && ty >= 0 && tx < T.W && ty < T.H;
    const GTexel g = loadG(T.normal, T.roughMetal, T.depth32, tx, ty, T.W, T.H);
    if (diffuse && (g.nw <= 0.0f || g.metal >= 1.0f)) continue;
    const f3 src = inside ? tapColour<MODE>(T, (size_t)ty * T.W + tx) : mk3(0.0f, 0.0f, 0.0f);
    const float w = tapWeight<diffuse>(c, i, g.nx, g.ny, g.nz, g.depth, g.nw > 0.0f ? g.rough : __uint_as_float(__float_as_uint(g.rough) | 0x80000000u));
    mx = __builtin_fmaf(src.x, w, mx); my = __builtin_fmaf(src.y, w, my); mz = __builtin_fmaf(src.z, w, mz);
    wsum += w;
  }
  storeFiltered<MODE>(T, pix, mx, my, mz, wsum);
}

typedef float V4 __attribute__((ext_vector_type(4)));
template <int MODE>
__global__ void __launch_bounds__(256) spatialTiledKernel(Targets T) {
  constexpr bool vertical = (MODE & 1) != 0;
  constexpr bool diffuse = MODE >= 2;
  constexpr int BW = vertical ? RT_VBW : 64, BH = vertical ? RT_VBH : 4;
  constexpr int TW = vertical ? RT_VBW : 96, TH = vertical ? RT_VBH + 2 * RT_RADIUS : 4;
  constexpr int PER = vertical ? BW * BH / 256 : 1, ROWSTEP = 256 / BW;
  constexpr int N = TW * TH;
  __shared__ V4 smA[N], smB[N];
  __shared__ uint32_t roughLo, roughHi, unflagged;
  if (threadIdx.x == 0) { roughLo = 0xFFFFFFFFu; roughHi = 0u; unflagged = 0u; }
  const int bx0 = blockIdx.x * BW, by0 = T.rowBegin + blockIdx.y * BH;
  const int lx = threadIdx.x % BW, ly = threadIdx.x / BW;
  const int x = bx0 + lx;

  static_assert(RT_VBW <= 32 && RT_VBH <= 32, "the V block spans at most two tiles across and three down");
  bool nothingDrawn;
  { const uint32_t txLast = (uint32_t)T.tilesX - 1u, tx0 = (uint32_t)bx0 >> 4, tx1 = min(tx0 + 1u, txLast);
    const uint32_t ty0 = (uint32_t)(by0 - T.tileRow0) >> 4, ty1 = (uint32_t)(min(by0 + BH, T.rowEnd) - 1 - T.tileRow0) >> 4;
    const uint32_t r0 = ty0 * (uint32_t)T.tilesX, r1 = ty1 * (uint32_t)T.tilesX, rm = ((ty0 + ty1) >> 1) * (uint32_t)T.tilesX;
    if (MODE == 1 && T.skyRun != nullptr && skyRunMin6(T.skyRun, T.skyEpoch, r0 + tx0, r0 + tx1, rm + tx0, rm + tx1, r1 + tx0, r1 + tx1) >= RT_SKY_V_RUN) return;
    nothingDrawn = vertical ? tileWordsOr6(T.tileWords, r0 + tx0, r0 + tx1, rm + tx0, rm + tx1, r1 + tx0, r1 + tx1) == 0u
                            : tileWordsOr(T.tileWords, r0 + tx0, r0 + tx1, r0 + min(tx0 + 2u, txLast), r0 + min(tx0 + 3u, txLast)) == 0u; }
  if (nothingDrawn) {
    if (MODE == 1) {
#pragma unroll
      for (int k = 0; k < PER; ++k) { const int y = by0 + ly + k * ROWSTEP; if (x < T.W && y < T.rowEnd) storeSkipped<MODE>(T, (size_t)y * T.W + x); }
    }
    return;
  }
  bool todo[PER]; bool any = false;
#pragma unroll
  for (int k = 0; k < PER; ++k) {
    const int y = by0 + ly + k * ROWSTEP;
    todo[k] = false;
    if (x < T.W && y < T.rowEnd) {
      const size_t pix = (size_t)y * T.W + x;
      const bool skip = (T.normal[pix] >> 30) == 0u || (diffuse && (T.roughMetal[pix] >> 8) == 255u);
      if (skip) storeSkipped<MODE>(T, pix); else { todo[k] = true; any = true; }
    }
  }
  if (!__syncthreads_or(any ? 1 : 0)) return;

  const int ox = vertical ? bx0 : bx0 - RT_RADIUS, oy = vertical ? by0 - RT_RADIUS : by0;
  uint32_t myLo = 0xFFFFFFFFu, myHi = 0u, myUnflagged = 0u;
  for (int t = threadIdx.x; t < N; t += 256) {
    const int tx = ox + t % TW, ty = oy + t / TW;
    float v[8] = {0.0f, 0.0f, 0.0f, 0.0f, 0.0f, 0.0f, 0.0f, 0.0f};
    const bool inside = tx >= 0 && ty >= 0 && tx < T.W && ty < T.H;
    const GTexel g = loadG(T.normal, T.roughMetal, T.depth32, tx, ty, T.W, T.H);
    v[3] = g.depth; v[4] = g.rough;
    if (diffuse) {
      if (g.nw > 0.0f && g.metal < 1.0f) {
        const f3 src = tapColour<MODE>(T, (size_t)ty * T.W + tx);
        v[0] = g.nx; v[1] = g.ny; v[2] = g.nz; v[5] = src.x; v[6] = src.y; v[7] = src.z;
      }
    } else {
      v[0] = g.nx; v[1] = g.ny; v[2] = g.nz;
      if (g.nw <= 0.0f) { v[4] = __uint_as_float(__float_as_uint(g.rough) | 0x80000000u); myUnflagged = 1u; }
      else { myLo = min(myLo, __float_as_uint(g.rough)); myHi = max(myHi, __float_as_uint(g.rough)); }
      if (inside) { const f3 src = tapColour<MODE>(T, (size_t)ty * T.W + tx); v[5] = src.x; v[6] = src.y; v[7] = src.z; }
    }
    smA[t] = V4{v[0], v[1], v[2], v[3]}; smB[t] = V4{v[4], v[5], v[6], v[7]};
  }
  if (!diffuse) {
    for (int o = 32; o > 0; o >>= 1) { myLo = min(myLo, (uint32_t)__shfl_down((int)myLo, o)); myHi = max(myHi, (uint32_t)__shfl_down((int)myHi, o)); }
    const unsigned long long anyUnflagged = __ballot(myUnflagged != 0u);
    if ((threadIdx.x & 63) == 0) { atomicMin(&roughLo, myLo); atomicMax(&roughHi, myHi); if (anyUnflagged) atomicOr(&unflagged, 1u); }
  }
  __syncthreads();
  const int uniform = diffuse ? 0 : (roughLo != roughHi ? 0 : unflagged ? 1 : 2);

  auto filter = [&](auto uniformTag) {
    constexpr int UNIFORM = decltype(uniformTag)::value;
#pragma unroll
    for (int k = 0; k < PER; ++k) {
      if (!todo[k]) continue;
      const int y = by0 + ly + k * ROWSTEP;
      const int ci = vertical ? (ly + k * ROWSTEP + RT_RADIUS) * TW + lx : ly * TW + lx + RT_RADIUS;
      const V4 ca = smA[ci];
      const Centre c = makeCentre<diffuse>(ca.x, ca.y, ca.z, ca.w, smB[ci].x, T.W, T.H);
      float mx = 0.0f, my = 0.0f, mz = 0.0f, wsum = 0.0f;
      typedef __attribute__((address_space(3))) const V4 LdsV4;
      LdsV4* pa = (LdsV4*)&smA[ci - RT_RADIUS * (vertical ? TW : 1)]; LdsV4* pb = (LdsV4*)&smB[ci - RT_RADIUS * (vertical ? TW : 1)];
      asm volatile("" : "+v"(pa)); asm volatile("" : "+v"(pb));
#pragma unroll
      for (int i = -RT_RADIUS; i <= RT_RADIUS; ++i) {
        const int ti = (i + RT_RADIUS) * (vertical ? TW : 1);
        const V4 a = pa[ti], b = pb[ti];
        const float w = tapWeight<diffuse, UNIFORM>(c, i, a.x, a.y, a.z, a.w, b.x);
        mx = __builtin_fmaf(b.y, w, mx); my = __builtin_fmaf(b.z, w, my); mz = __builtin_fmaf(b.w, w, mz);
        wsum += w;
      }
      storeFiltered<MODE>(T, (size_t)y * T.W + x, mx, my, mz, wsum);
    }
  };
  if (uniform == 2) filter(std::integral_constant<int, 2>{});
  else if (uniform == 1) filter(std::integral_constant<int, 1>{});
  else filter(std::integral_constant<int, 0>{});
}

RT_DEV f3 rgbToYCoCg(f3 c) {
  return mk3((c.x * 1.0f + c.y * 2.0f) + c.z * 1.0f, (c.x * 2.0f + c.y * 0.0f) + c.z * -2.0f, (c.x * -1.0f + c.y * 2.0f) + c.z * -1.0f);
}
RT_DEV f3 yCoCgToRGB(f3 c) {
  const float y = c.x * 0.25f, co = c.y * 0.25f, cg = c.z * 0.25f;
  return mk3(y + co - cg, y + cg, y - co - cg);
}
RT_DEV f3 tssTM(f3 hdr) {
  const f3 c = rgbToYCoCg(hdr); const float d = 4.0f + c.x;
  f3 q; div3Shared(c.x, c.y, c.z, d, q.x, q.y, q.z); return q;
}
RT_DEV f3 tssITM(f3 col) { const float k = 4.0f * rcpFast(1.0f - col.x); return yCoCgToRGB(mk3(col.x * k, col.y * k, col.z * k)); }
RT_DEV f3 tssTMSmooth(f3 hdr) { const f3 c = rgbToYCoCg(hdr); const float r = rcpFast(4.0f + c.x); return mk3(c.x * r, c.y * r, c.z * r); }
RT_DEV f2 loadVel(const uint32_t* __restrict__ vel, int x, int y, int W, int H) {
  f2 v; v.x = 0.0f; v.y = 0.0f;
  if (x < 0 || y < 0 || x >= W || y >= H) return v;
  const uint32_t p = vel[(size_t)y * W + x];
  v.x = f16ToF32(p & 0xFFFFu); v.y = f16ToF32(p >> 16);
  return v;
}
RT_DEV f4 loadRGBA16(const uint2* __restrict__ b, int x, int y, int W, int H) {
  if (x < 0 || y < 0 || x >= W || y >= H) { f4 z; z.x = z.y = z.z = z.w = 0.0f; return z; }
  return unpackRGBA16F(b[(size_t)y * W + x]);
}

RT_DEV const uint2* peerHistoryRow(const Targets& T, int iy) {
  int r = 0;
  while (r + 1 < T.peerWorld && (int)T.peerBounds[r + 1] <= iy) ++r;
  return T.peerHist[r] + (size_t)iy * T.W;
}
template <int ROWS, int PITCH>
RT_DEV uint2 temporalPixel(const Targets& T, const float4 (&tile)[ROWS][PITCH], const uint32_t (&velRaw)[ROWS][PITCH], const float (&velSq)[ROWS][PITCH], int x, int y, int lx, int ly) {
  const int W = T.W, H = T.H;
  const float Wf = (float)W, Hf = (float)H;
  const float uvx = ((float)x + 0.5f) * rcpFast(Wf), uvy = ((float)y + 0.5f) * rcpFast(Hf);
  const float4 cur = tile[ly][lx];
  const f3 currentTM = mk3(cur.x, cur.y, cur.z);
  f4 current; current.x = current.y = current.z = 0.0f; current.w = cur.w;
  const int ox[8] = {-1, 1, 0, 0, -1, 1, 1, -1}, oy[8] = {0, 0, -1, 1, -1, -1, 1, 1};
  f2 vmax;
  {
    float speedSq = velSq[ly][lx];
    uint32_t raw = velRaw[ly][lx];
    for (int i = 4; i < 8; ++i) {
      const float sq = velSq[ly + oy[i]][lx + ox[i]];
      const uint32_t r = velRaw[ly + oy[i]][lx + ox[i]];
      if (sq > speedSq) { raw = r; speedSq = sq; }
    }
    vmax.x = f16ToF32(raw & 0xFFFFu); vmax.y = f16ToF32(raw >> 16);
  }
  float alphaFiltered = cur.w;
  for (int i = 0; i < 8; ++i) alphaFiltered = __builtin_fmaf(tile[ly + oy[i]][lx + ox[i]].w, i < 4 ? 0.5f : 0.25f, alphaFiltered);
  alphaFiltered /= 4.0f;
  const bool plain = !(alphaFiltered > 0.0f);
  f4 history;
  {
#pragma clang fp contract(fast)
    const float sx = (uvx - vmax.x) * Wf - 0.5f, sy = (uvy - vmax.y) * Hf - 0.5f;
    const float x0 = floorf(sx), y0 = floorf(sy);
    const float fx = sx - x0, fy = sy - y0;
    const int ix0 = x0 < 0.0f ? 0 : (x0 > (float)(W - 1) ? W - 1 : (int)x0);
    const int ix1 = x0 + 1.0f < 0.0f ? 0 : (x0 + 1.0f > (float)(W - 1) ? W - 1 : (int)(x0 + 1.0f));
    const int iy0 = y0 < 0.0f ? 0 : (y0 > (float)(H - 1) ? H - 1 : (int)y0);
    const int iy1 = y0 + 1.0f < 0.0f ? 0 : (y0 + 1.0f > (float)(H - 1) ? H - 1 : (int)(y0 + 1.0f));
    const float w00 = (1.0f - fx) * (1.0f - fy), w10 = fx * (1.0f - fy), w01 = (1.0f - fx) * fy, w11 = fx * fy;
    const uint2* row0 = T.history + (size_t)iy0 * W; const uint2* row1 = T.history + (size_t)iy1 * W;
    if (T.histReach != nullptr) {
      const int over = max(T.histLo - iy0, iy1 - (T.histHi - 1));
      if (over > 0) {
        atomicMax(T.histReach, (uint32_t)over);
        if (T.peerHist != nullptr) {
          if (iy0 < T.histLo || iy0 >= T.histHi) row0 = peerHistoryRow(T, iy0);
          if (iy1 < T.histLo || iy1 >= T.histHi) row1 = peerHistoryRow(T, iy1);
        }
      }
    }
    const uint2* h00 = row0 + ix0; const uint2* h10 = row0 + ix1;
    const uint2* h01 = row1 + ix0; const uint2* h11 = row1 + ix1;
    if (plain) {
      history.x = history.y = history.z = 0.0f;
      history.w = ((f16ToF32(h00->y >> 16) * w00 + f16ToF32(h10->y >> 16) * w10) + f16ToF32(h01->y >> 16) * w01) + f16ToF32(h11->y >> 16) * w11;
    } else {
      const f4 t00 = unpackRGBA16F(*h00), t10 = unpackRGBA16F(*h10), t01 = unpackRGBA16F(*h01), t11 = unpackRGBA16F(*h11);
      history.x = ((t00.x * w00 + t10.x * w10) + t01.x * w01) + t11.x * w11;
      history.y = ((t00.y * w00 + t10.y * w10) + t01.y * w01) + t11.y * w11;
      history.z = ((t00.z * w00 + t10.z * w10) + t01.z * w01) + t11.z * w11;
      history.w = ((t00.w * w00 + t10.w * w10) + t01.w * w01) + t11.w * w11;
    }
  }
  float curHistoryBlur = fabsf(vmax.x) * (4.0f * Wf) + fabsf(vmax.y) * (4.0f * Hf);
  float historyBlur = 1.0f - history.w;
  historyBlur = fmaxf(historyBlur, curHistoryBlur);
  history.w = history.w * 15.0f + 1.0f;
  f3 result; float hw;
  if (plain) {
    float fl[3] = {currentTM.x, currentTM.y, currentTM.z};
    float mu0 = currentTM.x, m20 = mu0 * mu0;
    for (int i = 0; i < 8; ++i) {
      const float4 t = tile[ly + oy[i]][lx + ox[i]];
      const float wgt = i < 4 ? 0.5f : 0.25f;
      fl[0] = __builtin_fmaf(t.x, wgt, fl[0]); fl[1] = __builtin_fmaf(t.y, wgt, fl[1]); fl[2] = __builtin_fmaf(t.z, wgt, fl[2]);
      mu0 += t.x; m20 += t.x * t.x;
    }
    for (int k = 0; k < 3; ++k) fl[k] /= 4.0f;
    mu0 = divBy9(mu0);
    const float sigma0 = sqrtRN(fabsf(divBy9(m20) - mu0 * mu0));
    const float nmin3 = mu0 - sigma0, nmax3 = mu0 + sigma0;
    {
#pragma clang fp contract(fast)
      curHistoryBlur = saturatef(curHistoryBlur);
      historyBlur = saturatef(historyBlur);
      const float contrast = nmax3 - nmin3;
      float addAlias = historyBlur * 0.5f + 0.25f;
      addAlias = saturatef(addAlias + rcpFast(1.0f + contrast * (32.0f * 4.0f)));
      result = tssITM(mk3(lerpf(fl[0], currentTM.x, addAlias), lerpf(fl[1], currentTM.y, addAlias), lerpf(fl[2], currentTM.z, addAlias)));
      hw = fminf(history.w * (1.0f / 15.0f), 1.0f - curHistoryBlur);
    }
  } else {
  float gamma = current.w <= 0.0f ? 1.0f : clampf(8.0f * rcpFast(historyBlur), 1.0f, 32.0f);
  float fl[4] = {currentTM.x, currentTM.y, currentTM.z, current.w};
  float nmin[4], nmax[4];
  {
    float mu[3] = {currentTM.x, currentTM.y, currentTM.z};
    const float alpha = current.w;
    float m2[3] = {mu[0] * mu[0], mu[1] * mu[1], mu[2] * mu[2]};
    for (int i = 0; i < 8; ++i) {
      const float4 t = tile[ly + oy[i]][lx + ox[i]];
      const float nb[4] = {t.x, t.y, t.z, t.w};
      const float wgt = i < 4 ? 0.5f : 0.25f;
      for (int k = 0; k < 4; ++k) fl[k] = __builtin_fmaf(nb[k], wgt, fl[k]);
      for (int k = 0; k < 3; ++k) { mu[k] += nb[k]; m2[k] += nb[k] * nb[k]; }
    }
    for (int k = 0; k < 4; ++k) fl[k] /= 4.0f;
    gamma = fabsf(alpha - fl[3]) < 1.0f / 255.0f ? gamma : 1.0f;
    float sigma[3];
    for (int k = 0; k < 3; ++k) {
      mu[k] = divBy9(mu[k]);
      sigma[k] = sqrtRN(fabsf(divBy9(m2[k]) - mu[k] * mu[k]));
      const float gs = gamma * sigma[k];
      nmin[k] = fminf(mu[k] - gs, fl[k]);
      nmax[k] = fmaxf(mu[k] + gs, fl[k]);
    }
    nmin[3] = mu[0] - sigma[0]; nmax[3] = mu[0] + sigma[0];
  }
  {
#pragma clang fp contract(fast)
  curHistoryBlur = saturatef(curHistoryBlur);
  historyBlur = saturatef(historyBlur);
  const f3 hTM = tssTMSmooth(mk3(history.x, history.y, history.z));
  float historyTM[3] = {fminf(fmaxf(hTM.x, nmin[0]), nmax[0]), fminf(fmaxf(hTM.y, nmin[1]), nmax[1]), fminf(fmaxf(hTM.z, nmin[2]), nmax[2])};
  const float contrast = nmax[3] - nmin[3];
  const float lumContrastFactor = 32.0f * 4.0f;
  float addAlias = historyBlur * 0.5f + 0.25f;
  addAlias = saturatef(addAlias + rcpFast(1.0f + contrast * lumContrastFactor));
  const float ctm[3] = {currentTM.x, currentTM.y, currentTM.z};
  for (int k = 0; k < 3; ++k) fl[k] = lerpf(fl[k], ctm[k], addAlias);
  const float lumHist = historyTM[0];
  const float distToClamp = fminf(fabsf(nmin[3] - lumHist), fabsf(nmax[3] - lumHist));
  const float historyAmt = fminf(rcpFast(history.w) + historyBlur * 0.125f, 1.0f);
  float blend = 0.25f * rcpFast(lerpf(8.0f, distToClamp + contrast, historyAmt));
  blend = fminf(blend, 0.25f);
  blend = fl[3] > 0.0f ? blend : 1.0f;
  result = tssITM(mk3(lerpf(historyTM[0], fl[0], blend), lerpf(historyTM[1], fl[1], blend), lerpf(historyTM[2], fl[2], blend)));
  if (isnan(result.x) || isnan(result.y) || isnan(result.z)) result = tssITM(mk3(fl[0], fl[1], fl[2]));
  hw = fminf(history.w * (1.0f / 15.0f), 1.0f - curHistoryBlur);
  }
  }
  return packRGBA16F(result.x, result.y, result.z, hw);
}
template <int ROWS, int PITCH, int THREADS>
RT_DEV void stageTemporalTiles(const Targets& T, float4 (&tile)[ROWS][PITCH], uint32_t (&velRaw)[ROWS][PITCH], float (&velSq)[ROWS][PITCH], int ox, int oy) {
  const int W = T.W, H = T.H;
  for (int t = threadIdx.x; t < ROWS * PITCH; t += THREADS) {
    const int tx = ox + t % PITCH, ty = oy + t / PITCH;
    const bool inside = tx >= 0 && ty >= 0 && tx < W && ty < H;
    const size_t ti = inside ? (size_t)ty * W + tx : 0;
    const f4 raw = inside ? unpackRGBA16F(T.fltDff[ti]) : f4{0.0f, 0.0f, 0.0f, 0.0f};
    const uint32_t vr = inside ? T.velocity[ti] : 0u;
    const f3 tm = tssTM(mk3(raw.x, raw.y, raw.z));
    tile[t / PITCH][t % PITCH] = make_float4(tm.x, tm.y, tm.z, raw.w);
    const float vx = f16ToF32(vr & 0xFFFFu), vy = f16ToF32(vr >> 16);
    velRaw[t / PITCH][t % PITCH] = vr;
    velSq[t / PITCH][t % PITCH] = vx * vx + vy * vy;
  }
}
#define RT_TP_ROWS 4
__global__ void __launch_bounds__(256) temporalKernel(Targets T) {
  __shared__ float4 tile[RT_TP_ROWS + 2][66];
  __shared__ uint32_t velRaw[RT_TP_ROWS + 2][66];
  __shared__ float velSq[RT_TP_ROWS + 2][66];
  stageTemporalTiles<RT_TP_ROWS + 2, 66, 256>(T, tile, velRaw, velSq, (int)blockIdx.x * 64 - 1, T.rowBegin + (int)blockIdx.y * RT_TP_ROWS - 1);
  __syncthreads();
  const int lx = (threadIdx.x & 63) + 1, ly = (threadIdx.x >> 6) + 1;
  const int x = blockIdx.x * 64 + (threadIdx.x & 63), y = T.rowBegin + blockIdx.y * RT_TP_ROWS + (threadIdx.x >> 6);
  if (x >= T.W || y >= T.rowEnd) return;
  T.scratch[(size_t)y * T.W + x] = temporalPixel<RT_TP_ROWS + 2, 66>(T, tile, velRaw, velSq, x, y, lx, ly);
}

#ifndef RT_TT_TW
#define RT_TT_TW 64
#define RT_TT_TH 16
#endif
#define RT_TT_W (RT_TT_TW - 2)
#define RT_TT_H (RT_TT_TH - 2)
__global__ void __launch_bounds__(RT_TT_TW * RT_TT_TH) temporalToneKernel(Targets T) {
  constexpr int TW = RT_TT_TW, TH = RT_TT_TH;
  __shared__ float4 tile[TH + 2][TW + 2];
  __shared__ uint32_t velRaw[TH + 2][TW + 2];
  __shared__ float velSq[TH + 2][TW + 2];
  __shared__ float4 tm[TH][TW];
  const int x0 = (int)blockIdx.x * RT_TT_W - 1, y0 = T.outBegin + (int)blockIdx.y * RT_TT_H - 1;
  stageTemporalTiles<TH + 2, TW + 2, TW * TH>(T, tile, velRaw, velSq, x0 - 1, y0 - 1);
  __syncthreads();
  const int tx = threadIdx.x % TW, ty = threadIdx.x / TW;
  const int x = x0 + tx, y = y0 + ty;
  float4 c = make_float4(0.0f, 0.0f, 0.0f, 0.0f);
  if (x >= 0 && x < T.W && y >= T.rowBegin && y < T.rowEnd) {
    const uint2 packed = temporalPixel<TH + 2, TW + 2>(T, tile, velRaw, velSq, x, y, tx + 1, ty + 1);
    const bool mine = tx >= 1 && tx <= RT_TT_W && (ty >= 1 && ty <= RT_TT_H ? true : ty == 0 ? blockIdx.y == 0 : blockIdx.y == gridDim.y - 1);
    if (mine) T.scratch[(size_t)y * T.W + x] = packed;
    {
#pragma clang fp contract(fast)
      const f4 v = unpackRGBA16F(packed);
      c = make_float4(v.x * rcpFast(v.x + 0.5f), v.y * rcpFast(v.y + 0.5f), v.z * rcpFast(v.z + 0.5f), v.w);
    }
  }
  tm[ty][tx] = c;
  __syncthreads();
  if (tx < 1 || tx > RT_TT_W || ty < 1 || ty > RT_TT_H || x >= T.W || y >= T.outEnd) return;
  {
#pragma clang fp contract(fast)
    const float4 c0 = tm[ty][tx], c1 = tm[ty][tx - 1], c2 = tm[ty][tx + 1], c3 = tm[ty - 1][tx], c4 = tm[ty + 1][tx];
    float lx_ = -4.0f * c0.x, ly_ = -4.0f * c0.y, lz_ = -4.0f * c0.z;
    lx_ += c1.x; ly_ += c1.y; lz_ += c1.z;
    lx_ += c2.x; ly_ += c2.y; lz_ += c2.z;
    lx_ += c3.x; ly_ += c3.y; lz_ += c3.z;
    lx_ += c4.x; ly_ += c4.y; lz_ += c4.z;
    T.backbuffer[(size_t)y * T.W + x] = packRGBA8(c0.x - 0.2f * lx_, c0.y - 0.2f * ly_, c0.z - 0.2f * lz_, c0.w);
  }
}

#ifndef RT_TM_ROWS
#define RT_TM_ROWS 16
#endif
__global__ void __launch_bounds__(256) toneMapKernel(Targets T) {
#pragma clang fp contract(fast)
  __shared__ float4 tile[RT_TM_ROWS + 2][66];
  const int W = T.W, H = T.H;
  {
    const int ox = blockIdx.x * 64 - 1, oy = T.rowBegin + blockIdx.y * RT_TM_ROWS - 1;
    constexpr int N = (RT_TM_ROWS + 2) * 66, PER = (N + 255) / 256;
    f4 c[PER];
#pragma unroll
    for (int k = 0; k < PER; ++k) { const int t = threadIdx.x + 256 * k; c[k] = t < N ? loadRGBA16(T.scratch, ox + t % 66, oy + t / 66, W, H) : f4{0.0f, 0.0f, 0.0f, 0.0f}; }
#pragma unroll
    for (int k = 0; k < PER; ++k) {
      const int t = threadIdx.x + 256 * k;
      if (t < N) tile[t / 66][t % 66] = make_float4(c[k].x * rcpFast(c[k].x + 0.5f), c[k].y * rcpFast(c[k].y + 0.5f), c[k].z * rcpFast(c[k].z + 0.5f), c[k].w);
    }
  }
  __syncthreads();
  const int lx = (threadIdx.x & 63) + 1;
  const int x = blockIdx.x * 64 + (threadIdx.x & 63);
  if (x >= T.W) return;
#pragma unroll
  for (int k = 0; k < RT_TM_ROWS / 4; ++k) {
    const int ly = (threadIdx.x >> 6) + 4 * k + 1;
    const int y = T.rowBegin + blockIdx.y * RT_TM_ROWS + (threadIdx.x >> 6) + 4 * k;
    if (y >= T.rowEnd) continue;
    const float4 c0 = tile[ly][lx], c1 = tile[ly][lx - 1], c2 = tile[ly][lx + 1], c3 = tile[ly - 1][lx], c4 = tile[ly + 1][lx];
    float lx_ = -4.0f * c0.x, ly_ = -4.0f * c0.y, lz_ = -4.0f * c0.z;
    lx_ += c1.x; ly_ += c1.y; lz_ += c1.z;
    lx_ += c2.x; ly_ += c2.y; lz_ += c2.z;
    lx_ += c3.x; ly_ += c3.y; lz_ += c3.z;
    lx_ += c4.x; ly_ += c4.y; lz_ += c4.z;
    T.backbuffer[(size_t)y * W + x] = packRGBA8(c0.x - 0.2f * lx_, c0.y - 0.2f * ly_, c0.z - 0.2f * lz_, c0.w);
  }
}

static Targets makeTargets(rtggx_context* c, const FrameParams& fp, RowPass pass) {
  Targets T;
  const InputSet& set = c->cur();
  T.normal = set.normal; T.roughMetal = set.roughMetal; T.depth32 = set.depth32; T.velocity = set.velocity;
  T.rtRefl = set.rtRefl; T.rtDiff = set.rtDiff;
  T.scratch = c->tss[c->frameParity]; T.history = c->tss[c->frameParity ^ 1u]; T.fltRfl = c->fltRfl; T.fltDff = c->fltDff; T.backbuffer = c->backbuffer;
  T.W = (int)fp.W; T.H = (int)fp.H;
  uint32_t rb, re; passRows(fp, pass, rb, re);
  T.rowBegin = (int)rb; T.rowEnd = (int)re;
  passRows(fp, ROWS_FINAL, rb, re);
  T.outBegin = (int)rb; T.outEnd = (int)re;
  const bool strip = fp.rowBegin > 0u || fp.rowEnd < fp.H;
  T.histLo = (int)(fp.rowBegin > c->historyApron ? fp.rowBegin - c->historyApron : 0u);
  T.histHi = (int)(fp.rowEnd + c->historyApron < fp.H ? fp.rowEnd + c->historyApron : fp.H);
  T.histReach = strip ? c->histReach : nullptr;
  const bool peers = strip && c->peerWorld > 1u && c->dPeerTable != nullptr;
  T.peerHist = peers ? reinterpret_cast<const uint2* const*>(c->dPeerTable.get()) + (c->frameParity ^ 1u) * RT_MAX_PEERS : nullptr;
  T.peerBounds = peers ? reinterpret_cast<const uint32_t*>(reinterpret_cast<const uint2* const*>(c->dPeerTable.get()) + 2 * RT_MAX_PEERS) : nullptr;
  T.peerWorld = peers ? (int)c->peerWorld : 0;
  { uint32_t gb, ge; passRows(fp, ROWS_GBUFFER, gb, ge);
    T.tileWords = c->tileWords(gb, ge); T.tilesX = (int)((fp.W + 15) / 16); T.tileRow0 = (int)gb; }
  T.skyRun = nullptr; T.skyEpoch = 0u;
  return T;
}

static bool skyVPassMaySkip(rtggx_context* c, const Targets& TV, uint32_t gbufferRow0, uint32_t* epoch) {
  rtggx_context::SkyV now;
  const bool genValid = c->skyGen.any && c->skyGen.frame == c->frameCounter && c->skyGen.epoch == c->skyEpoch && c->skyGen.rows[0] == gbufferRow0;
  now.any = true; now.fltRflNull = TV.fltRfl == nullptr; now.frame = c->frameCounter; now.genEpoch = genValid ? c->skyGen.epoch : 0xFFFFFFFFu;
  now.rows[0] = (uint32_t)TV.rowBegin; now.rows[1] = (uint32_t)TV.rowEnd;
  const rtggx_context::SkyV& was = c->skyV;
  const bool may = c->staticSky && genValid && was.any && (was.frame == now.frame || was.frame + 1u == now.frame) && was.genEpoch == now.genEpoch
                   && was.rows[0] == now.rows[0] && was.rows[1] == now.rows[1] && was.fltRflNull == now.fltRflNull;
  c->skyV = now;
  *epoch = c->skyEpoch;
  return may;
}

int launchDenoise(rtggx_context* c, const FrameParams& fp, int useLds, hipStream_t s, hipEvent_t done, bool fuseToneMap) {
  c->frameParity ^= 1u;
  if (fp.rowEnd <= fp.rowBegin) return 0;
  const Targets TH = makeTargets(c, fp, ROWS_GBUFFER), TV = makeTargets(c, fp, ROWS_VFILTER), TT = makeTargets(c, fp, ROWS_TEMPORAL);
  const dim3 block(256);
  auto grid = [&](const Targets& T, uint32_t bw, uint32_t bh) { return dim3((fp.W + bw - 1) / bw, (T.rowEnd - T.rowBegin + bh - 1) / bh); };
  auto mark = [&](int i) { if (c->timing) hipEventRecord(c->tev[i], s); };
  const bool anyDiffuse = fp.mat.RoughMetals[0][1] < 1.0f || fp.mat.RoughMetals[1][1] < 1.0f;
  c->fltRflIsFltDff = !anyDiffuse;
  Targets TVr = TV; if (!anyDiffuse) TVr.fltRfl = nullptr;
  { uint32_t epoch;
    if (skyVPassMaySkip(c, TVr, (uint32_t)TV.tileRow0, &epoch) && useLds) { TVr.skyRun = c->cur().skyRun; TVr.skyEpoch = epoch; } }
  if (useLds) {
    hipLaunchKernelGGL(spatialTiledKernel<0>, grid(TH, 64, 4), block, 0, s, TH); mark(4);
    hipLaunchKernelGGL(spatialTiledKernel<1>, grid(TV, RT_VBW, RT_VBH), block, 0, s, TVr); mark(5);
    if (anyDiffuse) hipLaunchKernelGGL(spatialTiledKernel<2>, grid(TH, 64, 4), block, 0, s, TH);
    mark(6);
    if (anyDiffuse) hipLaunchKernelGGL(spatialTiledKernel<3>, grid(TV, RT_VBW, RT_VBH), block, 0, s, TV);
    mark(7);
  } else if (!anyDiffuse) {
    hipLaunchKernelGGL(spatialDirectKernel<0>, grid(TH, 64, 4), block, 0, s, TH); mark(4);
    hipLaunchKernelGGL(spatialDirectKernel<1>, grid(TV, 64, 4), block, 0, s, TVr); mark(5); mark(6); mark(7);
  } else {
    hipLaunchKernelGGL(spatialDirectKernel<0>, grid(TH, 64, 4), block, 0, s, TH); mark(4);
    hipLaunchKernelGGL(spatialDirectKernel<1>, grid(TV, 64, 4), block, 0, s, TV); mark(5);
    hipLaunchKernelGGL(spatialDirectKernel<2>, grid(TH, 64, 4), block, 0, s, TH); mark(6);
    hipLaunchKernelGGL(spatialDirectKernel<3>, grid(TV, 64, 4), block, 0, s, TV); mark(7);
  }
  if (fuseToneMap) {
    const dim3 g((fp.W + RT_TT_W - 1) / RT_TT_W, (uint32_t)(TT.outEnd - TT.outBegin + RT_TT_H - 1) / RT_TT_H), b(RT_TT_TW * RT_TT_TH);
    launch(temporalToneKernel, g, b, s, nullptr, done, TT);
  } else launch(temporalKernel, grid(TT, 64, RT_TP_ROWS), block, s, nullptr, done, TT);
  mark(8);
  RT_HIP(hipGetLastError());
  return 0;
}

int launchToneMap(rtggx_context* c, const FrameParams& fp, hipStream_t s, hipEvent_t done, const uint2* source) {
  if (fp.rowEnd <= fp.rowBegin) return 0;
  Targets T = makeTargets(c, fp, ROWS_FINAL);
  if (source) T.scratch = const_cast<uint2*>(source);
  const dim3 grid((fp.W + 63) / 64, (uint32_t)(T.rowEnd - T.rowBegin + RT_TM_ROWS - 1) / RT_TM_ROWS), block(256);
  launch(toneMapKernel, grid, block, s, nullptr, done, T);
  RT_HIP(hipGetLastError());
  return 0;
}

}
```

### raytracedggx_amd/csrc/raytrace.hip

```cpp
#include <cstring>
#include "rt_queue.h"
#include "rt_traverse.h"

namespace rt {

#define RT_PI 3.1415926535897f
#define RT_SGPR(v) ((uint32_t)__builtin_amdgcn_readfirstlane((int)(v)))

struct EnvRef { const uint2* __restrict__ texels; uint32_t size, mips; const uint32_t* __restrict__ mipOffset; };

RT_DEV void cubeFaceUV(f3 d, int& face, float& u, float& v) {
  const float ax = fabsf(d.x), ay = fabsf(d.y), az = fabsf(d.z);
  if (ax >= ay && ax >= az) { face = d.x >= 0.0f ? 0 : 1; u = (d.x >= 0.0f ? -d.z : d.z) / ax; v = -d.y / ax; }
  else if (ay >= az) { face = d.y >= 0.0f ? 2 : 3; u = d.x / ay; v = (d.y >= 0.0f ? d.z : -d.z) / ay; }
  else { face = d.z >= 0.0f ? 4 : 5; u = (d.z >= 0.0f ? d.x : -d.x) / az; v = -d.y / az; }
}
RT_DEV f3 cubeFaceDir(int face, float u, float v) {
  switch (face) {
    case 0: return mk3(1.0f, -v, -u);
    case 1: return mk3(-1.0f, -v, u);
    case 2: return mk3(u, 1.0f, v);
    case 3: return mk3(u, -1.0f, -v);
    case 4: return mk3(u, -v, 1.0f);
    default: return mk3(-u, -v, -1.0f);
// ... 540 lines not shown
            uint32_t s = rng(rc.x); s += fp.g.FrameIndex; s = rng(s); s %= 256u;
            xiY = (float)(rng(s) & 0xffffu) / 65536.0f; cosPhi = A.cosSin[s]; sinPhi = A.cosSin[256 + s];
          }
          const uint32_t toDiffImage = (rc.z ^ (rc.z >> 1)) & 1u;
          f3 w, L;
          if (rm.y > 0.5f) {
            const bool vndf = (fp.flags & RT_FLAG_VNDF) != 0u;
            const f3 Hh = reflectionHalfVector(vndf, N, V, rm.x * rm.x, cosPhi, sinPhi, xiY);
            L = reflect3(-V, Hh);
            const float NoL = dot3(N, L);
            if (NoL <= 0.0f) col = mk3(0.0f, 0.0f, 0.0f);
            else { w = reflectionWeight(vndf, N, V, Hh, NoL, rm, color); child = true; cr.flags = toDiffImage << 1; }
          } else {
            if (diffuseGroup) color = color * (1.0f - rm.y);
            L = diffuseDirection(N, cosPhi, sinPhi, xiY);
            w = color; child = true; cr.flags = 1u | ((toDiffImage ^ 1u) << 1);
          }
          if (child) {
            cr.ox = P.x; cr.oy = P.y; cr.oz = P.z; cr.dx = L.x; cr.dy = L.y; cr.dz = L.z;
            cr.pixel = rc.x; cr.skip = hitId;
            cr.wx = rw.x * w.x; cr.wy = rw.y * w.y; cr.wz = rw.z * w.z;
          }
        }
      }
    }
    if constexpr (shadeSpawns(PASS)) {
      const unsigned long long mask = __ballot(child);
      if (child) {
        const size_t k = (size_t)bin * A.binSlots + spawned + (uint32_t)__popcll(mask & ((1ull << (threadIdx.x & 63u)) - 1ull));
        A.spawnRays[k] = cr; A.spawnHits[k] = hitKey(RT_RAY_TMAX, 0xFFFFFFFFu);
      }
      spawned += (uint32_t)__popcll(mask);
      if (child) continue;
    }
    if constexpr (shadeAccumulates(PASS)) {
      float* acc = (((rc.z ^ (rc.z >> 1)) & 1u) != 0u ? A.accDiff : A.accRefl) + 3u * (size_t)rc.x;
      acc[0] = acc[0] + col.x * rw.x; acc[1] = acc[1] + col.y * rw.y; acc[2] = acc[2] + col.z * rw.z;
      continue;
    }
    const uint32_t packed = packR11G11B10F(mk3(col.x * rw.x, col.y * rw.y, col.z * rw.z));
    const bool toDiff = PASS == SHADE_FINAL ? diffuseGroup : ((rc.z ^ (rc.z >> 1)) & 1u) != 0u;
    if (toDiff) A.diffOut[rc.x] = packed; else A.reflOut[rc.x] = packed;
  }
  if constexpr (shadeSpawns(PASS)) { if ((threadIdx.x & 63u) == 0u) A.spawnCount[bin] = spawned; }
}

struct ReconArgs {
  const unsigned long long* visDepth; const uint32_t* normal; const uint16_t* roughMetal; const uint32_t* depth32;
  uint32_t* reflOut; uint32_t* diffOut;
  const uint32_t* diffPrev; uint32_t carryMask, diffMask;
  const uint32_t* tileWords; uint32_t tilesX, rowBegin, rowEnd;
};
struct ReconTexel { float nx, ny, nz, depth, rough; };
RT_DEV ReconTexel reconTexel(const ReconArgs& A, size_t i) {
  const uint32_t n = A.normal[i];
  ReconTexel t;
  t.nx = (float)(2 * (int)(n & 1023u) - 1023); t.ny = (float)(2 * (int)((n >> 10) & 1023u) - 1023); t.nz = (float)(2 * (int)((n >> 20) & 1023u) - 1023);
  t.depth = (float)A.depth32[i] * (1.0f / 16777215.0f);
  t.rough = (float)(A.roughMetal[i] & 0xFFu) * (1.0f / 255.0f);
  return t;
}
RT_DEV float reconNormalDepthWeight(const ReconTexel& c, const ReconTexel& q) {
  const float I = (c.nx * q.nx + c.ny * q.ny) + c.nz * q.nz;
  float x = fmaxf(I * (1.0f / 1046529.0f), 0.0f);
  x = x * x; x = x * x; x = x * x; x = x * x; x = x * x;
  return x * (float)exp((double)(-fabsf(c.depth - q.depth) * c.depth * 4.0f));
}
RT_DEV f3 reconDivide(f3 s, float w) {
  const double d = (double)w;
  return mk3((float)((double)s.x / d), (float)((double)s.y / d), (float)((double)s.z / d));
}
__global__ void __launch_bounds__(256) reconstructKernel(const FrameParams* __restrict__ fpp, ReconArgs A) {
  const FrameParams& fp = *fpp;
  const uint32_t tile = blockIdx.x;
  { uint32_t word;
    asm volatile("s_load_dword %0, %1, %2\n\ts_waitcnt lgkmcnt(0)" : "=s"(word) : "s"(A.tileWords), "s"(tile * 4u) : "memory");
    if (word == 0u) return; }
  const uint32_t W = fp.W;
  const uint32_t px = (tile % A.tilesX) * 16u + (threadIdx.x & 15u), py = A.rowBegin + (tile / A.tilesX) * 16u + (threadIdx.x >> 4);
  if (px >= W || py >= A.rowEnd) return;
  const size_t pix = (size_t)py * W + px;
  const uint32_t vis = (uint32_t)A.visDepth[pix];
  if (vis == 0u) return;
  const uint32_t inst = (vis - 1u) >> 24;
  if ((A.carryMask >> inst) & 1u) A.diffOut[pix] = A.diffPrev[pix];
  const uint32_t f = fp.g.FrameIndex & 3u, ox = (0x6u >> f) & 1u, oy = (0xAu >> f) & 1u;
  if ((px & 1u) == ox && (py & 1u) == oy) return;
  const bool diffuse = ((A.diffMask >> inst) & 1u) != 0u;
  const ReconTexel c = reconTexel(A, pix);
  f3 sumR = mk3(0.0f, 0.0f, 0.0f), sumD = sumR, meanR = sumR, meanD = sumR;
  float wR = 0.0f, wD = 0.0f;
  uint32_t n = 0u;
  for (int dy = -1; dy <= 1; ++dy)
    for (int dx = -1; dx <= 1; ++dx) {
      const int qx = (int)px + dx, qy = (int)py + dy;
      if (qx < 0 || qy < 0 || qx >= (int)W || qy >= (int)fp.H || ((uint32_t)qx & 1u) != ox || ((uint32_t)qy & 1u) != oy) continue;
      const size_t q = (size_t)qy * W + (uint32_t)qx;
      const uint32_t vq = (uint32_t)A.visDepth[q];
      if (vq == 0u || ((vq - 1u) >> 24) != inst) continue;
      const ReconTexel t = reconTexel(A, q);
      const float wnd = reconNormalDepthWeight(c, t);
      const float ts = saturatef(fabsf(t.rough - c.rough) * 2.0f);
      const float w = wnd * (1.0f - ts * ts * (3.0f - 2.0f * ts));
      const f3 L = unpackR11G11B10F(A.reflOut[q]);
      sumR = sumR + L * w; wR += w; meanR = meanR + L;
      if (diffuse) { const f3 Ld = unpackR11G11B10F(A.diffOut[q]); sumD = sumD + Ld * wnd; wD += wnd; meanD = meanD + Ld; }
      ++n;
    }
  if (n == 0u) {
#pragma unroll 1
    for (int dy = -2; dy <= 2; ++dy)
#pragma unroll 1
      for (int dx = -2; dx <= 2; ++dx) {
        const int qx = (int)px + dx, qy = (int)py + dy;
        if (qx < 0 || qy < 0 || qx >= (int)W || qy >= (int)fp.H || ((uint32_t)qx & 1u) != ox || ((uint32_t)qy & 1u) != oy) continue;
        const size_t q = (size_t)qy * W + (uint32_t)qx;
        const uint32_t vq = (uint32_t)A.visDepth[q];
        if (vq == 0u || ((vq - 1u) >> 24) != inst) continue;
        meanR = meanR + unpackR11G11B10F(A.reflOut[q]);
        if (diffuse) meanD = meanD + unpackR11G11B10F(A.diffOut[q]);
        ++n;
      }
  }
  A.reflOut[pix] = packR11G11B10F(wR > 0.0f ? reconDivide(sumR, wR) : n ? reconDivide(meanR, (float)n) : meanR);
  if (diffuse) A.diffOut[pix] = packR11G11B10F(wD > 0.0f ? reconDivide(sumD, wD) : n ? reconDivide(meanD, (float)n) : meanD);
}

__global__ void sampleParamsKernel(const FrameParams* __restrict__ src, FrameParams* __restrict__ dst, uint32_t samples) {
  constexpr uint32_t words = sizeof(FrameParams) / 4u, indexWord = (offsetof(FrameParams, g) + offsetof(RtggxCBGlobal, FrameIndex)) / 4u;
  for (uint32_t i = threadIdx.x; i < words * samples; i += blockDim.x) {
    const uint32_t k = i / words, w = i % words, v = reinterpret_cast<const uint32_t*>(src)[w];
    reinterpret_cast<uint32_t*>(dst + k)[w] = w == indexWord ? v * samples + k : v;
  }
}

struct SampleGenArgs {
  const unsigned long long* visDepth; const float4* fat0; const float4* fat1; const float* cosSin;
  RayRec* rays; HitKey* hits; uint32_t* binCount; uint32_t binSlots;
  const uint32_t* tileWords; uint32_t tilesX, rowBegin, rowEnd;
};
template <bool WIDE>
__global__ void __launch_bounds__(256, RT_GEN_MIN_BLOCKS) sampleGenKernel(const FrameParams* __restrict__ fpp, SampleGenArgs A) {
  const FrameParams& fp = *fpp;
  const uint32_t tile = blockIdx.x;
  { uint32_t word;
    asm volatile("s_load_dword %0, %1, %2\n\ts_waitcnt lgkmcnt(0)" : "=s"(word) : "s"(A.tileWords), "s"(tile * 4u) : "memory");
    if (word == 0u) return; }
  const uint32_t wave = threadIdx.x >> 6, lane = threadIdx.x & 63u;
  const uint32_t px = (tile % A.tilesX) * 16 + (wave & 1u) * 8 + (lane & 7u);
  const uint32_t py = A.rowBegin + (tile / A.tilesX) * 16 + (wave >> 1) * 8 + (lane >> 3);
  bool wantRefl = false, wantDiff = false;
  RayRec rr, rd;
  if (px < fp.W && py < A.rowEnd) {
    const uint32_t W = fp.W, H = fp.H;
    const size_t pix = (size_t)py * W + px;
    uint32_t visibility = (uint32_t)A.visDepth[pix];
    float xiY, cosPhi, sinPhi;
    if constexpr (WIDE) sampleParamWide(fp, A.cosSin, py * W + px, xiY, cosPhi, sinPhi);
    else {
      uint32_t s = py * W + px;
      s = rng(s); s += fp.g.FrameIndex; s = rng(s); s %= 256u;
      xiY = (float)(rng(s) & 0xffffu) / 65536.0f; cosPhi = A.cosSin[s]; sinPhi = A.cosSin[256 + s];
    }
    if (visibility > 0) {
      --visibility;
      const uint32_t inst = visibility >> 24;
      uint32_t prim = visibility & 0xFFFFFFu;
      asm volatile("" : "+v"(prim));
      f2 screenPos; screenPos.x = ((float)px + 0.5f) / (float)W * 2.0f - 1.0f; screenPos.y = ((float)py + 0.5f) / (float)H * 2.0f - 1.0f;
      screenPos.y = -screenPos.y;
      const f3 eye = mk3(fp.rg.EyePt[0], fp.rg.EyePt[1], fp.rg.EyePt[2]);
      const Tri3 v = getVertices(inst ? A.fat1 : A.fat0, prim);
      const M4 wvp = cbLoad4x4(fp.g.WorldViewProjs[inst]);
      f4 p[3];
      for (int k = 0; k < 3; ++k) p[k] = mulPoint(v.pos[k], wvp);
      screenPos.x -= fp.rg.ProjBias[0]; screenPos.y -= fp.rg.ProjBias[1];
      const f2 bary = calcBarycentrics(p, screenPos);
      const Attrib a = interpAttrib(v, bary.x, bary.y);
      const f3 color = mk3(fp.mat.BaseColors[inst][0], fp.mat.BaseColors[inst][1], fp.mat.BaseColors[inst][2]);
      const f2 rghMtl = getRoughMetal(fp.mat, inst, a.UV);
      const f4 P4 = mulPoint(a.Pos, cbLoad4x3(fp.g.Worlds[inst]));
      const f3 P = mk3(P4.x, P4.y, P4.z);
      const f3 N = normalize3(mulDir(a.Nrm, cbLoad3x3(inst ? fp.g.WorldIT1 : fp.g.WorldITs0)));
      const f3 V = normalize3(eye - P);
      const uint32_t skip = (inst << 24) | prim;
      {
        const bool vndf = (fp.flags & RT_FLAG_VNDF) != 0u;
        const f3 Hh = reflectionHalfVector(vndf, N, V, rghMtl.x * rghMtl.x, cosPhi, sinPhi, xiY);
        const f3 R = reflect3(-V, Hh);
        const float NoL = dot3(N, R);
        if (NoL > 0.0f) {
          const f3 w = reflectionWeight(vndf, N, V, Hh, NoL, rghMtl, color);
          wantRefl = true;
          rr.ox = P.x; rr.oy = P.y; rr.oz = P.z; rr.dx = R.x; rr.dy = R.y; rr.dz = R.z;
          rr.pixel = (uint32_t)pix; rr.skip = skip; rr.flags = 0u;
          rr.wx = w.x; rr.wy = w.y; rr.wz = w.z;
        }
      }
      if (rghMtl.y < 1.0f) {
        const f3 dir = diffuseDirection(N, cosPhi, sinPhi, xiY);
        wantDiff = true;
        rd.ox = P.x; rd.oy = P.y; rd.oz = P.z; rd.dx = dir.x; rd.dy = dir.y; rd.dz = dir.z;
        rd.pixel = (uint32_t)pix; rd.skip = skip; rd.flags = 1u;
        rd.wx = color.x * (1.0f - 0.04f); rd.wy = color.y * (1.0f - 0.04f); rd.wz = color.z * (1.0f - 0.04f);
      }
    }
  }
  const uint32_t bin = blockIdx.x * 4u + wave;
  const unsigned long long maskR = __ballot(wantRefl), maskD = __ballot(wantDiff), below = (1ull << lane) - 1ull;
  const uint32_t nR = (uint32_t)__popcll(maskR);
  RayRec* dst = A.rays + (size_t)bin * A.binSlots;
  HitKey* keys = A.hits + (size_t)bin * A.binSlots;
  if (wantRefl) { const uint32_t k = (uint32_t)__popcll(maskR & below); dst[k] = rr; keys[k] = hitKey(RT_RAY_TMAX, 0xFFFFFFFFu); }
  const uint32_t kD = nR + (uint32_t)__popcll(maskD & below);
  if (wantDiff && kD < A.binSlots) { dst[kD] = rd; keys[kD] = hitKey(RT_RAY_TMAX, 0xFFFFFFFFu); }
  if (lane == 0) A.binCount[bin] = min(nR + (uint32_t)__popcll(maskD), A.binSlots);
}

struct ResolveArgs {
  const unsigned long long* visDepth; float* accRefl; float* accDiff; uint32_t* reflOut; uint32_t* diffOut;
  const uint32_t* tileWords; uint32_t tilesX, rowBegin, rowEnd, diffMask; float scale;
};
__global__ void __launch_bounds__(256) resolveSamplesKernel(const FrameParams* __restrict__ fpp, ResolveArgs A) {
  const FrameParams& fp = *fpp;
  const uint32_t tile = blockIdx.x;
  { uint32_t word;
    asm volatile("s_load_dword %0, %1, %2\n\ts_waitcnt lgkmcnt(0)" : "=s"(word) : "s"(A.tileWords), "s"(tile * 4u) : "memory");
    if (word == 0u) return; }
  const uint32_t px = (tile % A.tilesX) * 16u + (threadIdx.x & 15u), py = A.rowBegin + (tile / A.tilesX) * 16u + (threadIdx.x >> 4);
  if (px >= fp.W || py >= A.rowEnd) return;
  const size_t pix = (size_t)py * fp.W + px;
  const uint32_t vis = (uint32_t)A.visDepth[pix];
  if (vis == 0u) return;
  float* r = A.accRefl + 3u * pix;
  A.reflOut[pix] = packR11G11B10F(mk3(r[0] * A.scale, r[1] * A.scale, r[2] * A.scale));
  r[0] = 0.0f; r[1] = 0.0f; r[2] = 0.0f;
  if ((A.diffMask >> ((vis - 1u) >> 24)) & 1u) {
    float* d = A.accDiff + 3u * pix;
    A.diffOut[pix] = packR11G11B10F(mk3(d[0] * A.scale, d[1] * A.scale, d[2] * A.scale));
    d[0] = 0.0f; d[1] = 0.0f; d[2] = 0.0f;
  }
}

static uint32_t skyEpochForGen(rtggx_context* c, const FrameParams& fp, uint32_t rb, uint32_t re, hipStream_t sGen, bool adaptive, uint32_t sliceShift) {
  rtggx_context::SkyGen now;
  now.any = true; now.adaptive = adaptive; now.frame = c->frameCounter; now.rows[0] = rb; now.rows[1] = re; now.rate = c->rayRate; now.sliceShift = sliceShift; now.stream = sGen;
  now.tilesX = (fp.W + 15u) / 16u; now.tilesY = (re - rb + 15u) / 16u;
  memcpy(now.camera, fp.rg.ProjToWorld, 64); memcpy(now.camera + 16, fp.rg.EyePt, 16);
  const rtggx_context::SkyGen& was = c->skyGen;
  bool same = was.any && (was.frame == now.frame || was.frame + 1u == now.frame) && was.rows[0] == rb && was.rows[1] == re && was.rate == now.rate
              && was.adaptive == adaptive && was.sliceShift == sliceShift && was.stream == sGen;
#ifndef RT_SKY_NO_CAMERA_CHECK
  same = same && memcmp(was.camera, now.camera, sizeof now.camera) == 0;
#endif
  if (!same) c->breakSkyRuns();
  now.epoch = c->skyEpoch;
  c->skyGen = now;
  return now.epoch;
}

int launchRayTrace(rtggx_context* c, const FrameParams& fp, hipStream_t sGen, hipStream_t s, hipEvent_t done) {
  uint32_t rb, re;
  passRows(fp, ROWS_GBUFFER, rb, re);
  if (re <= rb) return 0;
  const uint32_t tilesX = (fp.W + 15) / 16, tilesY = (re - rb + 15) / 16;
  const bool quad = c->rayRate == 4u;
  const uint32_t quadX = (tilesX + 1u) / 2u, quadY = (tilesY + 1u) / 2u;
  if ((fp.mat.RoughMetals[0][1] < 1.0f || fp.mat.RoughMetals[1][1] < 1.0f) && c->binSlots < RT_BIN) {
    setError("rtggx_ray_trace: a material with metallic below 1 (a diffuse ray per pixel as well) but ray bins of %u slots: rtggx_update_frame sizes them", c->binSlots); return -1;
  }
  GenArgs G;
  const InputSet& set = c->cur();
  { const uint32_t thenFrame = c->frameCounter + 2u;
    VisTarget& vn = c->visOf(thenFrame);
    G.visNext = vn.depth; G.zeroNext0 = c->largeCountBase + (thenFrame & 1u); G.zeroNext1 = c->next().splitCount;
    vn.cleared.frame = thenFrame; vn.cleared.rows[0] = rb; vn.cleared.rows[1] = re;
    if (c->traceShare > 0.93f) c->traversalBound = true; else if (c->traceShare < 0.89f) c->traversalBound = false;
    G.visDirty = c->tileWords(rb, re); c->traceTileWords = quad ? c->visDirtyOnes : G.visDirty;
    G.visDirtyNextOut = vn.dirty;
    G.visDirtyNext = c->useTileWords && !c->traversalBound && vn.flags.rows[0] == rb && vn.flags.rows[1] == re ? vn.dirty : c->visDirtyOnes;
    vn.flags.rows[0] = rb; vn.flags.rows[1] = re;
  }
  G.visDepth = c->curVis().depth; G.depthOut = set.depth32; G.normalOut = set.normal; G.roughMetalOut = set.roughMetal; G.velocityOut = set.velocity; G.reflOut = set.rtRefl; G.diffOut = set.rtDiff;
  G.roughMetalPrev = c->prev().roughMetal;
  G.diffPrev = c->genCarriesDiff ? c->prev().rtDiff : nullptr;
  G.fat0 = c->mesh[0].fat; G.fat1 = c->mesh[1].fat;
  G.env = c->env.texels; G.envMipOffset = c->dEnvMipOffset; G.envSize = c->env.size; G.envMips = c->env.mips; G.cosSin = c->sampleTable();
  G.rays = (RayRec*)set.rayQueue.get(); G.hits = (HitKey*)set.hitQueue.get(); G.binCount = set.binCount; G.binSlots = c->binSlots; G.frameRays = c->rayCounter32;
  G.tilesX = tilesX; G.numTiles = tilesX * tilesY; G.rowBegin = rb; G.rowEnd = re;
  const uint32_t splitWork = c->splitWork, splitMaxShift = c->splitMaxShift;
  const uint32_t numBins = quad ? quadX * quadY * 4u : G.numTiles * 4u;
  const uint32_t sliceShift = chooseSliceShift(c, true, numBins);
  c->lastTraceSmall = c->forcePlacement >= 0 ? c->forcePlacement == 1 : (sliceShift > 0u || c->lastFrameRays < RT_WIDE_RAYS);
  const bool adaptive = splitWork != 0u && sliceShift == 0u;
  const uint32_t splitCap = !adaptive ? 0u : c->splitCapForced != 0xFFFFFFFFu ? c->splitCapForced
                          : c->splitDemand == 0u ? 0u : ((c->splitDemand + c->splitDemand / 8u + 64u + 31u) / 32u) * 32u;
  G.binWork = adaptive ? c->binWork : nullptr; G.splitList = set.splitList; G.splitCount = set.splitCount;
  G.frontWork = RT_SPLIT_FRONT < splitWork ? RT_SPLIT_FRONT : splitWork;
  G.splitWork = splitWork; G.splitMaxShift = splitMaxShift < 3u ? splitMaxShift : 3u; G.splitCap = splitCap < RT_SPLIT_CAP ? splitCap : RT_SPLIT_CAP;
  G.skyEpoch = skyEpochForGen(c, fp, rb, re, sGen, adaptive, sliceShift);
  if (c->skyEpochWrapped) {
    RT_HIP(hipDeviceSynchronize());
    for (auto& st : c->sets) RT_HIP(hipMemset(st.skyRun, 0, c->skyTiles * 4));
    RT_HIP(hipStreamSynchronize(nullptr));
    c->skyEpochWrapped = false;
  }
  G.skyPrev = c->prev().skyRun; G.skyOut = set.skyRun; G.skyPrevRun = c->staticSky ? RT_SKY_PREV_RUN : RT_SKY_RUN_CAP + 1u;
  FrameEvents& ev = c->frameEvents(c->frameCounter);
  const FrameParams* genParams = c->dParams + c->slot;
  if (c->samples > 1u) {
    FrameParams* const sp = c->sppParams + (size_t)c->slot * RTGGX_MAX_SAMPLES_PER_PIXEL;
    hipLaunchKernelGGL(sampleParamsKernel, dim3(1), dim3(256), 0, sGen, genParams, sp, c->samples);
    genParams = sp;
  }
  const bool wide = c->sampleSet > RTGGX_MIN_SAMPLE_SET;
  launch(wide ? (quad ? rayGenKernel<4, true> : rayGenKernel<1, true>) : quad ? rayGenKernel<4> : rayGenKernel<1>, dim3(quad ? numBins : G.numTiles), dim3(256), sGen, nullptr, sGen != s ? ev.gen : nullptr, genParams, G);
  ev.genFrame = 0u; ev.genStream = sGen;
  if (sGen != s) {
    RT_HIP(hipStreamWaitEvent(s, ev.gen, 0));
    ev.genFrame = c->frameCounter;
  }
  if (c->timing) hipEventRecord(c->tev[11], s);
  const bool ring = c->kernelRing && c->kevCount < c->kevBegin.size() && (c->ringTick++ % c->ringStride) == 0u;
  const TraceQueue q{G.rays, G.hits, G.binCount};
  c->traceGrid[0] = numBins; c->traceGrid[1] = quad ? quadX : tilesX; c->traceGrid[2] = quad ? quadY : tilesY; c->traceGrid[3] = sliceShift;
  { const int r = launchTrace(c, fp, s, q, numBins, true, quad ? quadX : tilesX, quad ? quadY : tilesY, sliceShift, adaptive ? (int)G.splitCap : -1,
                              ring ? c->kevBegin[c->kevCount] : nullptr, ring ? c->kevEnd[c->kevCount] : done); if (r) return r; }
  if (c->timing) hipEventRecord(c->tev[12], s);
  if (ring) ++c->kevCount;
  if (done && ring) hipEventRecord(done, s);
  RT_HIP(hipGetLastError());
  return 0;
}

static void (*const kShade[3][2])(const FrameParams*, ShadeArgs) = {
    {shadeKernel<1, SHADE_FINAL>, shadeKernel<4, SHADE_FINAL>}, {shadeKernel<1, SHADE_SPAWN>, shadeKernel<4, SHADE_SPAWN>},
    {shadeKernel<1, SHADE_FINAL_DEEP>, shadeKernel<4, SHADE_FINAL_DEEP>}};
static void (*const kShadeSpawnWide[2])(const FrameParams*, ShadeArgs) = {shadeKernel<1, SHADE_SPAWN, true>, shadeKernel<4, SHADE_SPAWN, true>};
static int launchShadeSamples(rtggx_context* c, const FrameParams& fp, hipStream_t s, hipEvent_t done, ShadeArgs S, uint32_t numTiles, int spillPart) {
  const uint32_t N = c->samples, depth = c->maxDepth;
  const bool wide = c->sampleSet > RTGGX_MIN_SAMPLE_SET;
  if (!c->sppAcc || !c->sppParams) { setError("rtggx_ray_trace: %u samples per pixel without their buffers", N); return -1; }
  if (c->sppStream && c->sppStream != s) { RT_HIP(hipEventRecord(c->evSpp, c->sppStream)); RT_HIP(hipStreamWaitEvent(s, c->evSpp, 0)); }
  c->sppStream = s;
  const InputSet& set = c->cur();
  const FrameParams* const sp = c->sppParams + (size_t)c->slot * RTGGX_MAX_SAMPLES_PER_PIXEL;
  S.accRefl = c->sppAcc; S.accDiff = c->sppAcc + 3u * (size_t)c->W * c->H;
  SampleGenArgs G;
  G.visDepth = S.visDepth; G.fat0 = S.fat0; G.fat1 = S.fat1; G.cosSin = S.cosSin;
  G.rays = S.spawnRays; G.hits = S.spawnHits; G.binCount = S.spawnCount; G.binSlots = S.binSlots;
  G.tileWords = S.tileWords; G.tilesX = S.tilesX; G.rowBegin = S.rowBegin; G.rowEnd = S.rowEnd;
  const TraceQueue q{S.rays, S.spawnHits, S.binCount};
  for (uint32_t k = 0; k < N; ++k) {
    for (uint32_t level = 0; level < depth; ++level) {
      if (k > 0 && level == 0) launch(wide ? sampleGenKernel<true> : sampleGenKernel<false>, dim3(numTiles), dim3(256), s, nullptr, nullptr, sp + k, G);
      if (k > 0 || level > 0) {
        const int r = launchTrace(c, fp, s, q, c->traceGrid[0], true, c->traceGrid[1], c->traceGrid[2], c->traceGrid[3], -1, nullptr, nullptr, spillPart);
        if (r) return r;
      }
      launch(level + 1u < depth ? (wide ? shadeKernel<1, SHADE_SPAWN_ACCUM, true> : shadeKernel<1, SHADE_SPAWN_ACCUM>) : shadeKernel<1, SHADE_ACCUM>, dim3(numTiles), dim3(256), s, nullptr, nullptr, sp + k, S);
      S.carryMask = 0u;
      RT_HIP(hipGetLastError());
    }
  }
  ResolveArgs R;
  R.visDepth = S.visDepth; R.accRefl = S.accRefl; R.accDiff = S.accDiff; R.reflOut = set.rtRefl; R.diffOut = set.rtDiff;
  R.tileWords = S.tileWords; R.tilesX = S.tilesX; R.rowBegin = S.rowBegin; R.rowEnd = S.rowEnd;
  R.diffMask = (fp.mat.RoughMetals[0][1] < 1.0f ? 1u : 0u) | (fp.mat.RoughMetals[1][1] < 1.0f ? 2u : 0u);
  R.scale = 1.0f / (float)N;
  launch(resolveSamplesKernel, dim3(numTiles), dim3(256), s, nullptr, done, c->dParams + c->slot, R);
  RT_HIP(hipGetLastError());
  return 0;
}
int launchShade(rtggx_context* c, const FrameParams& fp, hipStream_t s, hipEvent_t done) {
  uint32_t rb, re;
  passRows(fp, ROWS_GBUFFER, rb, re);
  if (re <= rb) return 0;
  const uint32_t tilesX = (fp.W + 15) / 16, numTiles = tilesX * ((re - rb + 15) / 16);
  const InputSet& set = c->cur();
  ShadeArgs S;
  S.diffPrev = c->prev().rtDiff; S.visDepth = c->curVis().depth; S.tilesX = tilesX; S.rowBegin = rb; S.rowEnd = re;
  S.carryMask = (fp.mat.RoughMetals[0][1] >= 1.0f ? 1u : 0u) | (fp.mat.RoughMetals[1][1] >= 1.0f ? 2u : 0u);
  if (c->genCarriesDiff) S.carryMask = 0u;
  S.tileWords = c->tileWords(rb, re);
  const bool quad = c->rayRate == 4u;
  const uint32_t grid = quad ? ((tilesX + 1u) / 2u) * ((re - rb + 31u) / 32u) : numTiles;
  if (quad) S.carryMask = 0u;
  S.rays = (const RayRec*)set.rayQueue.get(); S.hits = (const HitKey*)set.hitQueue.get(); S.binCount = set.binCount; S.binSlots = c->binSlots;
  S.fat0 = c->mesh[0].fat; S.fat1 = c->mesh[1].fat;
  S.env = c->env.texels; S.envMipOffset = c->dEnvMipOffset; S.envSize = c->env.size; S.envMips = c->env.mips; S.sh = c->sh;
  S.reflOut = set.rtRefl; S.diffOut = set.rtDiff;
  S.spawnRays = (RayRec*)set.rayQueue.get(); S.spawnHits = (HitKey*)set.hitQueue.get(); S.spawnCount = set.binCount; S.cosSin = c->sampleTable();
  S.accRefl = nullptr; S.accDiff = nullptr;
  const FrameParams* const dfp = c->dParams + c->slot;
  const uint32_t depth = c->maxDepth;
  const int spillPart = s == c->streamMain ? 2 : (int)c->traceSpillHalf;
  if (c->samples > 1u && !quad) return launchShadeSamples(c, fp, s, done, S, numTiles, spillPart);
  for (uint32_t level = 0; level < depth; ++level) {
    if (level > 0) {
      const TraceQueue q{S.rays, S.spawnHits, S.binCount};
      const int r = launchTrace(c, fp, s, q, c->traceGrid[0], true, c->traceGrid[1], c->traceGrid[2], c->traceGrid[3], -1, nullptr, nullptr, spillPart);
      if (r) return r;
      S.carryMask = 0u;
    }
    const int pass = level + 1u < depth ? SHADE_SPAWN : level == 0 ? SHADE_FINAL : SHADE_FINAL_DEEP;
    launch(pass == SHADE_SPAWN && c->sampleSet > RTGGX_MIN_SAMPLE_SET ? kShadeSpawnWide[quad] : kShade[pass][quad], dim3(grid), dim3(256), s, nullptr, pass == SHADE_SPAWN ? nullptr : done, dfp, S);
    RT_HIP(hipGetLastError());
  }
  return 0;
}

int launchReconstruct(rtggx_context* c, const FrameParams& fp, hipStream_t s) {
  uint32_t rb, re;
  passRows(fp, ROWS_GBUFFER, rb, re);
  if (re <= rb) return 0;
  const uint32_t tilesX = (fp.W + 15) / 16, numTiles = tilesX * ((re - rb + 15) / 16);
  const InputSet& set = c->cur();
  ReconArgs R;
  R.visDepth = c->curVis().depth; R.normal = set.normal; R.roughMetal = set.roughMetal; R.depth32 = set.depth32;
  R.reflOut = set.rtRefl; R.diffOut = set.rtDiff;
  R.diffPrev = c->prev().rtDiff;
  const uint32_t metal = (fp.mat.RoughMetals[0][1] >= 1.0f ? 1u : 0u) | (fp.mat.RoughMetals[1][1] >= 1.0f ? 2u : 0u);
  R.carryMask = c->genCarriesDiff ? 0u : metal; R.diffMask = ~metal & 3u;
  R.tileWords = c->tileWords(rb, re); R.tilesX = tilesX; R.rowBegin = rb; R.rowEnd = re;
  hipLaunchKernelGGL(reconstructKernel, dim3(numTiles), dim3(256), 0, s, c->dParams + c->slot, R);
  RT_HIP(hipGetLastError());
  return 0;
}

__global__ void fillTestQueue(const float* __restrict__ rays, uint32_t n, uint32_t binSlots, RayRec* q0, HitKey* keys, uint32_t* binCount, float2* tRange) {
  const uint32_t i = blockIdx.x * blockDim.x + threadIdx.x;
  if (i % binSlots == 0 && i < n) binCount[i / binSlots] = n - i < binSlots ? n - i : binSlots;
  if (i >= n) return;
  const float* r = rays + 8 * (size_t)i;
  RayRec rr;
  rr.ox = r[0]; rr.oy = r[1]; rr.oz = r[2]; rr.dx = r[3]; rr.dy = r[4]; rr.dz = r[5];
  rr.pixel = 0u; rr.skip = 0xFFFFFFFFu; rr.flags = 0u; rr.wx = rr.wy = rr.wz = 0.0f;
  q0[i] = rr;
  tRange[i] = make_float2(r[6], r[7]);
  keys[i] = hitKey(r[7], 0xFFFFFFFFu);
}
__global__ void exportTestHits(const FrameParams* __restrict__ fpp, const RayRec* __restrict__ rays, const HitKey* __restrict__ hits, uint32_t n,
                               const float4* __restrict__ fat0, const float4* __restrict__ fat1, float* __restrict__ out) {
  const uint32_t i = blockIdx.x * blockDim.x + threadIdx.x;
  if (i >= n) return;
  const HitKey k = hits[i];
  const uint32_t id = hitKeyId(k);
  float* o = out + 6 * (size_t)i;
  const bool valid = id != 0xFFFFFFFFu;
  float t = hitKeyT(k), b1 = 0.0f, b2 = 0.0f;
  if (valid) {
    const RayRec rr = rays[i];
    const uint32_t inst = id >> 24;
    uint32_t prim = id & 0xFFFFFFu;
    asm volatile("" : "+v"(prim));
    const Tri3 v = getVertices(inst ? fat1 : fat0, prim);
    woopTestVerts(toObject(rr.ox, rr.oy, rr.oz, rr.dx, rr.dy, rr.dz, inst ? fpp->invWorld[1] : fpp->invWorld[0]), v.pos[0], v.pos[1], v.pos[2], t, b1, b2);
  }
  o[0] = t; o[1] = u2f(valid ? id >> 24 : 0u); o[2] = u2f(valid ? id & 0xFFFFFFu : 0u); o[3] = b1; o[4] = b2; o[5] = valid ? 1.0f : 0.0f;
}
int launchTraceRays(rtggx_context* c, const FrameParams& fp, const float* dRays, uint32_t n, float* dOut, hipStream_t s) {
  if (!n) return 0;
  if (n > c->numBinsMax * c->binSlots) { setError("rtggx_trace_rays: at most %u rays per launch", c->numBinsMax * c->binSlots); return -1; }
  const uint32_t numBins = (((n + c->binSlots - 1u) / c->binSlots) + 3u) & ~3u;
  const InputSet& set = c->cur();
  RT_HIP(hipMemsetAsync(set.binCount, 0, (size_t)numBins * 4, s));
  if (!c->testRayRange) RT_HIP(alloc(c->testRayRange, (size_t)c->numBinsMax * RT_BIN * sizeof(float2)));
  hipLaunchKernelGGL(fillTestQueue, dim3((n + 255) / 256), dim3(256), 0, s, dRays, n, c->binSlots, (RayRec*)set.rayQueue.get(), (HitKey*)set.hitQueue.get(), set.binCount, (float2*)c->testRayRange.get());
  c->traceRayRange = c->testRayRange;
  const TraceQueue q{(const RayRec*)set.rayQueue.get(), (HitKey*)set.hitQueue.get(), set.binCount};
  { const int r = launchTrace(c, fp, s, q, numBins, false, 0u, 0u, chooseSliceShift(c, false, numBins), -1); c->traceRayRange = nullptr; if (r) return r; }
  hipLaunchKernelGGL(exportTestHits, dim3((n + 255) / 256), dim3(256), 0, s, c->dParams + c->slot, (const RayRec*)set.rayQueue.get(), (const HitKey*)set.hitQueue.get(), n,
                     (const float4*)c->mesh[0].fat, (const float4*)c->mesh[1].fat, dOut);
  RT_HIP(hipGetLastError());
  return 0;
}

__global__ void debugEnvironmentKernel(EnvRef env, const float* __restrict__ dirs, const float* __restrict__ levels, uint32_t n, int level0, float* __restrict__ rgb) {
  const uint32_t i = blockIdx.x * blockDim.x + threadIdx.x;
  if (i >= n) return;
  const f3 d = mk3(dirs[3 * (size_t)i], dirs[3 * (size_t)i + 1], dirs[3 * (size_t)i + 2]);
  const f3 c = level0 ? environmentLevel0(env, d) : environment(env, d, levels[i]);
  rgb[3 * (size_t)i] = c.x; rgb[3 * (size_t)i + 1] = c.y; rgb[3 * (size_t)i + 2] = c.z;
}
int launchDebugEnvironment(rtggx_context* c, const float* dDirs, const float* dLevels, uint32_t n, int level0, float* dOut, hipStream_t s) {
  const EnvRef env{c->env.texels, c->env.size, c->env.mips, c->dEnvMipOffset};
  hipLaunchKernelGGL(debugEnvironmentKernel, dim3((n + 255) / 256), dim3(256), 0, s, env, dDirs, dLevels, n, level0, dOut);
  RT_HIP(hipGetLastError());
  return 0;
}

struct AccumArgs {
  const unsigned long long* visDepth; const uint32_t* refl; const uint32_t* diff; float4* accRefl; float4* accDiff;
  uint32_t first, count, diffMask;
};
RT_DEV float4 accumulateWord(float4 a, uint32_t word) {
#pragma clang fp contract(off)
  const f3 c = unpackR11G11B10F(word);
  const float y = (0.25f * c.x + 0.5f * c.y) + 0.25f * c.z;
  return make_float4(a.x + c.x, a.y + c.y, a.z + c.z, a.w + y * y);
}
__global__ void __launch_bounds__(256) accumulateKernel(AccumArgs A) {
  const uint32_t i = blockIdx.x * 256u + threadIdx.x;
  if (i >= A.count) return;
  const size_t pix = (size_t)A.first + i;
  const uint32_t vis = (uint32_t)A.visDepth[pix];
  A.accRefl[pix] = accumulateWord(A.accRefl[pix], A.refl[pix]);
  const uint32_t inst = (vis - 1u) >> 24;
  if (vis != 0u && inst < 2u && ((A.diffMask >> inst) & 1u)) A.accDiff[pix] = accumulateWord(A.accDiff[pix], A.diff[pix]);
}
int launchAccumulate(rtggx_context* c, const FrameParams& fp, hipStream_t s) {
  if (!c->accRefl || !c->accDiff) { setError("rtggx_ray_trace: accumulation without its buffers"); return -1; }
  if (fp.rowEnd <= fp.rowBegin) return 0;
  const InputSet& set = c->cur();
  AccumArgs A;
  A.visDepth = c->curVis().depth; A.refl = set.rtRefl; A.diff = set.rtDiff; A.accRefl = c->accRefl; A.accDiff = c->accDiff;
  A.first = fp.rowBegin * fp.W; A.count = (fp.rowEnd - fp.rowBegin) * fp.W;
  A.diffMask = (fp.mat.RoughMetals[0][1] < 1.0f ? 1u : 0u) | (fp.mat.RoughMetals[1][1] < 1.0f ? 2u : 0u);
  hipLaunchKernelGGL(accumulateKernel, dim3((A.count + 255u) / 256u), dim3(256), 0, s, A);
  RT_HIP(hipGetLastError());
  return 0;
}

__global__ void __launch_bounds__(256) presentAccumulationKernel(const float4* __restrict__ accRefl, const float4* __restrict__ accDiff, uint2* __restrict__ out, uint32_t count, uint32_t frames) {
#pragma clang fp contract(off)
  const uint32_t i = blockIdx.x * 256u + threadIdx.x;
  if (i >= count) return;
  const double n = (double)frames;
  const float4 a = accRefl[i], d = accDiff[i];
  const float r = (float)((double)a.x / n) + (float)((double)d.x / n);
  const float g = (float)((double)a.y / n) + (float)((double)d.y / n);
  const float b = (float)((double)a.z / n) + (float)((double)d.z / n);
  out[i] = packRGBA16F(r, g, b, 1.0f);
}
int launchPresentAccumulation(rtggx_context* c, hipStream_t s) {
  const uint32_t count = c->W * c->H;
  hipLaunchKernelGGL(presentAccumulationKernel, dim3((count + 255u) / 256u), dim3(256), 0, s, (const float4*)c->accRefl, (const float4*)c->accDiff, c->converged, count, c->accumFrames);
  RT_HIP(hipGetLastError());
  return 0;
}

}
```

### raytracedggx_amd/csrc/rtggx_context.h

```cpp
#pragma once
#include <hip/hip_runtime.h>
#include <hip/hip_ext.h>
#include <stdint.h>
#include <stdlib.h>
#include <string>
#include <utility>
#include <vector>
#include <memory>
#include "rtggx_device.h"
#include "rt_owned_hip.h"

#ifndef RT_SETS
#define RT_SETS 4
#endif
#define RT_SLOTS (RT_SETS + 1)
#define RT_VIS_RING (RT_SETS + 2)
#define RT_VIS_CLEAR 0x00FFFFFF00000000ull
#define RT_SKY_PREV_RUN (RT_SETS + 2)
#define RT_SKY_V_RUN 2u
#define RT_SKY_RUN_CAP 255u
namespace rt {

#define RT_TREELET_LEVELS 3
struct BuildResult {
  uint32_t numRounds;
  uint32_t treelets[RT_TREELET_LEVELS];
  uint32_t topCount;
  uint32_t depth;
  uint32_t stack4, depth4, nodes4;
  uint32_t error;
  uint32_t itemCursor, roundCursor;
  uint32_t finalEntry, finalLds;
  float cost, pad2;
};
struct BvhTopo {
  DevBuf<uint32_t> order;
  DevBuf<int32_t> left, right, nodeParent, leafParent;
  DevBuf<float> nodeBox, triBox;
  DevBuf<uint32_t> cnt[RT_TREELET_LEVELS];
  DevBuf<uint32_t> roundBase;
  DevBuf<void> dTreelets, dRefitItems; DevBuf<uint32_t> dRefitRounds; DevBuf<int32_t> treeletRoots;
  DevBuf<int32_t> topList, topRank;
  DevBuf<float4> cost4;
  DevBuf<int4> ent4; DevBuf<uint32_t> lvl4;
  DevBuf<BuildResult> dResult; PinnedBuf<BuildResult> hResult;
  BuildResult result{};
  uint32_t numTris = 0; int32_t root = -1;
  bool refittable = false;
};

struct MeshDev {
  MeshDev(); ~MeshDev();
  float* verts = nullptr;
  DevBuf<float> vertsOwn[RT_SETS]; float* vertsBuf[RT_SETS] = {};
  float4* fat = nullptr; DevBuf<float4> fatOwn[RT_SETS]; float4* fatBuf[RT_SETS] = {};
  uint32_t vertsVersion[RT_SETS] = {}, version = 0, latestSet = 0;
  bool deforming = false;
  PinnedBuf<float> stage[RT_SLOTS];
  uint32_t stageNext = 0; int pendingStage = -1;
  DevBuf<float> deviceStage[RT_SLOTS];
  uint32_t deviceStageNext = 0; int pendingDeviceStage = -1; Event evProduced, evStaged;
  BvhTopo topo;
  std::unique_ptr<struct BuildJob> job;
  bool wantRebuild = false;
  uint32_t topoVersion = 0, topoVersionOfSet[RT_SETS] = {};
  DevBuf<float> dCost;
  PinnedBuf<float> hCost;
  Event evCost; bool costInFlight = false;
  float builtCost = 0.0f, lastCost = 0.0f;
  uint32_t refits = 0, rebuilds = 0;
  DevBuf<uint32_t> indices;
  uint32_t numVerts = 0, numIndices = 0, numTris = 0;
  BvhNode* nodes = nullptr;
  Bvh4Node* nodes4 = nullptr;
  BvhTri* tris = nullptr;
  DevBuf<BvhNode> nodesOwn[RT_SETS]; DevBuf<Bvh4Node> nodes4Own[RT_SETS]; DevBuf<BvhTri> trisOwn[RT_SETS];
  BvhNode* nodesBuf[RT_SETS] = {}; Bvh4Node* nodes4Buf[RT_SETS] = {}; BvhTri* trisBuf[RT_SETS] = {};
  uint32_t topCount = 0; uint32_t topCountBuf[RT_SETS] = {};
  Bvh4Node* top = nullptr; DevBuf<Bvh4Node> topOwn[RT_SETS]; Bvh4Node* topBuf[RT_SETS] = {};
  int32_t root = -1;
  uint32_t depth = 0;
  uint32_t stack4 = 0;
  float bmin[3] = {0, 0, 0}, bmax[3] = {0, 0, 0};
};

struct EnvDev {
  DevBuf<uint2> texels;
  uint32_t size = 0, mips = 0;
  uint32_t mipOffset[16] = {};
  uint64_t totalTexels = 0;
};

struct FrameParams {
  RtggxCBGlobal g;
  RtggxRayGenConstants rg;
  RtggxCBPerObject po[2];
  RtggxCBMaterial mat;
  float invWorld[2][16];
  uint32_t W, H;
  uint32_t rowBegin, rowEnd;
  uint32_t flags;
  uint32_t sampleMask;
  uint32_t pad[2];
};
#define RT_FLAG_VNDF 1u

struct InputSet {
  DevBuf<uint32_t> normal, velocity, rtRefl, rtDiff;
  DevBuf<uint16_t> roughMetal;
  DevBuf<uint32_t> depth32;
  DevBuf<void> rayQueue, hitQueue;
  DevBuf<uint32_t> binCount;
  DevBuf<uint32_t> splitList; uint32_t* splitCount = nullptr;
  DevBuf<uint32_t> skyRun;
  Event evRead;
  bool readRecorded = false;
};

struct VisTarget {
  DevBuf<unsigned long long> depth;
  DevBuf<uint32_t> dirty;
  struct { uint32_t frame = 0, rows[2] = {0, 0}; } cleared;
  struct { uint32_t rows[2] = {0, 0}; uint32_t rasterFrame = 0; } flags;
};

struct FrameEvents {
  Event gen;
  uint32_t genFrame = 0;
  hipStream_t genStream = nullptr;
  Event trace;
  bool traceRecorded = false;
};

}

#ifndef RT_COLLAPSE_AREA_WEIGHT
#define RT_COLLAPSE_AREA_WEIGHT 1.0f
#define RT_COLLAPSE_TRIS_WEIGHT 0.0f
#endif
#define RT_MAX_PEERS 16

struct rtggx_context {
  int device = 0;
  uint32_t W = 0, H = 0;
  uint32_t rowBegin = 0, rowEnd = 0;
  uint32_t historyApron = 18;
  rt::DevBuf<uint32_t> histReach;
  rt::Stream ownMain; hipStream_t streamMain = nullptr, streamAS = nullptr;
  rt::Stream streamRefit;
  bool refitIssued = false;
  uint32_t frameCounter = 0;
  rt::FrameEvents frames[4];
  rt::FrameEvents& frameEvents(uint32_t f) { return frames[f & 3u]; }
  rt::Stream ownAS, ownVis;
  bool asyncCompute = true;
  hipStream_t streamVis = nullptr;
  rt::Event evVis;
  hipStream_t evVisStream = nullptr;
  rt::Event evAS;
  rt::Event evRefit;
  rt::Event evRT;
  int setReadDeferred = -1;
  double fenceWaitUs = 0.0; uint32_t fenceWaits = 0;
  int fuseToneMap = -1; bool toneMapDone = false, denoiseIssued = false;
  rt::DevBuf<uint32_t> exchangeTokens;
  float collapseWeights[2] = {RT_COLLAPSE_AREA_WEIGHT, RT_COLLAPSE_TRIS_WEIGHT};
  uint32_t peerWorld = 0; rt::DevBuf<void> dPeerTable; std::vector<rt::IpcMapping> ipcMapped;
  uint32_t lastPlacement[2] = {0, 0};
  int forcePlacement = -1;
  bool fltRflIsFltDff = false;
  bool externalStream = false;

  bool vndf = false;
  uint32_t rayRate = 1;
  uint32_t maxDepth = 1, depthRequested = 1;
  uint32_t samples = 1, samplesRequested = 1;
  rt::DevBuf<float> sppAcc; rt::DevBuf<rt::FrameParams> sppParams;
  hipStream_t sppStream = nullptr; rt::Event evSpp;
  bool accumulate = false, accumulateRequested = false;
  uint32_t accumFrames = 0;
  rt::DevBuf<float4> accRefl, accDiff; rt::DevBuf<uint2> converged;
  bool scoring = false, scoringRequested = false;
  rt::DevBuf<uint2> reference;
  rt::DevBuf<double> scorePartial[2]; rt::DevBuf<uint32_t> scoreCounts; uint32_t scoreStride = 0;
  rt::DevBuf<RtggxScore> scoreRing;
  uint64_t scoreIndex = 0, scoreRead = 0;
  uint32_t traceGrid[4] = {};
  float rebuildRatio = 1.2f; uint32_t rebuildSteps = 16;
  rt::MeshDev mesh[2];
  rt::EnvDev env;
  rt::DevBuf<float> sh;
  rt::DevBuf<float> cosSinTab;
  uint32_t sampleSet = RTGGX_MIN_SAMPLE_SET, sampleSetRequested = RTGGX_MIN_SAMPLE_SET;
  rt::DevBuf<float> cosSinWide[8];
  static uint32_t sampleSetSlot(uint32_t m) { uint32_t k = 0; while ((512u << k) < m) ++k; return k; }
  const float* sampleTable() const { return sampleSet > RTGGX_MIN_SAMPLE_SET ? cosSinWide[sampleSetSlot(sampleSet)] : cosSinTab; }

  rt::InputSet sets[RT_SETS];
  uint32_t setIndex = 0;
  uint32_t setAhead(uint32_t k) const { return (setIndex + k) % RT_SETS; }
  rt::InputSet& cur() { return sets[setIndex]; }
  rt::InputSet& prev() { return sets[setAhead(RT_SETS - 1u)]; }
  rt::InputSet& next() { return sets[setAhead(1u)]; }
  rt::VisTarget vis[RT_VIS_RING];
  rt::VisTarget& visOf(uint32_t frame) { return vis[frame % RT_VIS_RING]; }
  rt::VisTarget& curVis() { return visOf(frameCounter); }
  void selectSet(uint32_t i) {
    setIndex = i;
    largeTris = largeTrisBuf[frameCounter & 1u]; largeCount = largeCountBase ? largeCountBase + (frameCounter & 1u) : nullptr;
    for (auto& m : mesh) { m.verts = m.vertsBuf[i]; m.fat = m.fatBuf[i]; m.nodes = m.nodesBuf[i]; m.nodes4 = m.nodes4Buf[i]; m.top = m.topBuf[i]; m.topCount = m.topCountBuf[i]; m.tris = m.trisBuf[i]; }
    binWork = binWorkBuf[frameCounter & 1u]; rayCounter32 = rayCounterBuf + (frameCounter & 3u) * 256u;
  }
  rt::DevBuf<uint32_t> backbuffer;
  rt::DevBuf<uint2> tss[2], fltRfl, fltDff;
  uint32_t frameParity = 0;

  void* largeTris = nullptr; rt::DevBuf<void> largeTrisBuf[2];
  uint32_t* largeCount = nullptr;
  rt::DevBuf<uint32_t> largeCountBase;
  uint32_t* binWork = nullptr;
  rt::DevBuf<uint32_t> binWorkBuf[2];
  const uint32_t* tileWords(uint32_t rb, uint32_t re) {
    const rt::VisTarget& v = curVis();
    return useTileWords && !traversalBound && v.flags.rasterFrame == frameCounter && v.flags.rows[0] == rb && v.flags.rows[1] == re ? v.dirty.get() : visDirtyOnes.get();
  }
  bool staticSky = true;
  uint32_t skyEpoch = 1u; bool skyEpochWrapped = false; size_t skyTiles = 0;
  void breakSkyRuns() { skyEpoch = (skyEpoch + 1u) & 0xFFFFFFu; if (skyEpoch == 0u) skyEpochWrapped = true; }
  struct SkyGen { bool any = false, adaptive = false; uint32_t frame = 0, epoch = 0, rows[2] = {0, 0}, rate = 0, sliceShift = 0, tilesX = 0, tilesY = 0; hipStream_t stream = nullptr; float camera[20] = {}; } skyGen;
  struct SkyV { bool any = false, fltRflNull = false; uint32_t frame = 0, genEpoch = 0, rows[2] = {0, 0}; } skyV;
  bool useTileWords = true;
  bool traversalBound = false;
  const uint32_t* traceTileWords = nullptr;
  rt::DevBuf<uint32_t> visDirtyOnes;
  uint32_t splitDemand = 0;
  uint32_t splitCapForced = 0xFFFFFFFFu;
  uint32_t splitWork = 0, splitMaxShift = 0;
  uint32_t largeCapacity = 0;

  uint32_t numBinsMax = 0, binSlots = 64;
  rt::DevBuf<void> testRayRange; void* traceRayRange = nullptr;
  rt::DevBuf<int32_t> stackOverflow;
  uint32_t spillEntries = 0;
  rt::DevBuf<void> dummyRecord;
  rt::DevBuf<uint32_t> dEnvMipOffset;
  bool lastTraceSmall = false; uint32_t traceSpillHalf = 0;
  hipStream_t shadeStream = nullptr;
  bool genCarriesDiff = false, shadeWroteDiff = false, lastFrameDiffuse = false;
  hipStream_t diffStream = nullptr;
  uint32_t numCUs = 256;
  uint32_t traceWaves = 12, traceWavesForced = 0; float traceShare = 0.0f; rt::DevBuf<unsigned long long> traceStamps; uint32_t traceStampLaunch = 0;
  unsigned long long traceStampSum = 0, traceStampStart = 0; uint32_t traceStampAt = 0, traceSampleLaunch = 0;
  uint32_t traceTrial = 0, traceCooldown = 0, traceWavesSince = 0; float traceTrialBase = 0.0f;

  rt::PinnedBuf<uint32_t> hostRayCounters;
  rt::Event evRayCounters; bool rayCountersInFlight = false; uint32_t traceLaunches = 0;
  uint32_t lastFrameRays = 0xFFFFFFFFu;
  uint32_t* rayCounter32 = nullptr;
  rt::DevBuf<uint32_t> rayCounterBuf;
  uint32_t* lastRayCounter32 = nullptr;
  rt::DevBuf<unsigned long long> rayCounter;

  rt::FrameParams slots[RT_SLOTS];
  uint32_t slot = 0;
  rt::DevBuf<rt::FrameParams> dParams;
  bool slotUploaded = false;
  bool slotRendered = false;
  RtggxCBMaterial material;
  float invWorld[2][16];
  bool haveConstants = false, asBuilt = false, shDone = false;

  bool timing = false;
  bool kernelRing = false;
  uint32_t ringStride = 1, ringTick = 0;
  std::vector<rt::Event> kevBegin, kevEnd;
  uint32_t kevCount = 0;
  rt::Event tev[16];
  bool timingsPending = false;
};

namespace rt {
enum RowPass { ROWS_GBUFFER , ROWS_VFILTER , ROWS_TEMPORAL , ROWS_FINAL };
inline void passRows(const FrameParams& fp, RowPass pass, uint32_t& b, uint32_t& e) {
  const uint32_t apron = pass == ROWS_GBUFFER ? 18u : pass == ROWS_VFILTER ? 2u : pass == ROWS_TEMPORAL ? 1u : 0u;
  b = fp.rowBegin > apron ? fp.rowBegin - apron : 0u;
  e = fp.rowEnd + apron < fp.H ? fp.rowEnd + apron : fp.H;
  if (fp.rowEnd <= fp.rowBegin) { b = e = 0; }
}
void setError(const char* fmt, ...);
#define RT_HIP(expr) do { hipError_t _e = (expr); if (_e != hipSuccess) { rt::setError("%s failed: %s (%s:%d)", #expr, hipGetErrorString(_e), __FILE__, __LINE__); return -2; } } while (0)
template <class... P, class... A>
inline void launch(void (*k)(P...), dim3 grid, dim3 block, hipStream_t s, hipEvent_t start, hipEvent_t stop, A&&... a) {
  if (start || stop) hipExtLaunchKernelGGL(k, grid, block, 0, s, start, stop, 0, static_cast<P>(a)...);
  else hipLaunchKernelGGL(k, grid, block, 0, s, static_cast<P>(a)...);
}

int uploadParams(rtggx_context* c, uint32_t slot, hipStream_t s);
int launchVisibility(rtggx_context* c, const FrameParams& fp, hipStream_t s, hipEvent_t done = nullptr);
int buildLbvh(rtggx_context* c, uint32_t slot, hipStream_t s);
int startRebuild(rtggx_context* c, uint32_t slot, uint32_t set);
int continueRebuild(rtggx_context* c, uint32_t slot, hipStream_t s, uint32_t maxSteps, bool* swapped);
int prepareRebuild(rtggx_context* c, uint32_t slot);
void abandonRebuild(rtggx_context* c, uint32_t slot);
int refitLbvh(rtggx_context* c, uint32_t slot, uint32_t set, hipStream_t s);
void freeBuildProducts(MeshDev& m);
int buildFatTris(rtggx_context* c, uint32_t slot, uint32_t set, hipStream_t s);
int launchRayTrace(rtggx_context* c, const FrameParams& fp, hipStream_t sGen, hipStream_t sTrace, hipEvent_t done = nullptr);
int launchShade(rtggx_context* c, const FrameParams& fp, hipStream_t s, hipEvent_t done = nullptr);
int launchReconstruct(rtggx_context* c, const FrameParams& fp, hipStream_t s);
int allocSamples(rtggx_context* c);
int allocAccumulation(rtggx_context* c);
int launchAccumulate(rtggx_context* c, const FrameParams& fp, hipStream_t s);
int launchPresentAccumulation(rtggx_context* c, hipStream_t s);
#define RT_SCORE_CHUNK 1024u
#define RT_SCORE_SUMS 9u
int launchScore(rtggx_context* c, const FrameParams& fp, hipStream_t s);
int launchReferenceFromAccumulation(rtggx_context* c, hipStream_t s);
int launchTraceRays(rtggx_context* c, const FrameParams& fp, const float* dRays, uint32_t n, float* dOut, hipStream_t s);
int launchDebugEnvironment(rtggx_context* c, const float* dDirs, const float* dLevels, uint32_t n, int level0, float* dOut, hipStream_t s);
int launchDenoise(rtggx_context* c, const FrameParams& fp, int useLds, hipStream_t s, hipEvent_t done = nullptr, bool fuseToneMap = false);
int launchToneMap(rtggx_context* c, const FrameParams& fp, hipStream_t s, hipEvent_t done = nullptr, const uint2* source = nullptr);
int decodeEnv(rtggx_context* c, int format, uint32_t size, uint32_t mips, const void* hostData, size_t bytes, hipStream_t s);
int buildEnvFromImage(rtggx_context* c, int layout, int pixels, uint32_t width, uint32_t height, const void* hostData, uint32_t size, hipStream_t s);
int generateEnvMips(rtggx_context* c, hipStream_t s);
int projectSH(rtggx_context* c, hipStream_t s);
int unpackVisDepth(rtggx_context* c, uint32_t* dVis, uint32_t* dDepth, hipStream_t s);
int packVisDepth(rtggx_context* c, const uint32_t* dVis, const uint32_t* dDepth, hipStream_t s);
}
```

Measured before the change: 3166 Mrays/s.

## Skip temporal and tone-map blocks whose sky pixels have settled across frames

Adds per-block settled words, double-buffered by frame parity. The temporal kernel records whether a block lies in a static-sky window and its output equals the existing history. On the next frame, blocks whose 3x3 neighbourhood is settled in the current sky epoch skip the temporal pass, and tone-map blocks over fully settled regions skip writing the backbuffer. This removes redundant work on static sky regions, at the cost of a comparison, a block-wide reduction and scalar loads of flag words, plus fragile validity bookkeeping across frames.

```diff
diff --git a/include/rtggx.h b/include/rtggx.h
--- a/include/rtggx.h
+++ b/include/rtggx.h
@@ -163,6 +163,8 @@
 int  rtggx_debug_tile_words(rtggx_context* ctx, int enable);
 int  rtggx_debug_static_sky(rtggx_context* ctx, int enable);
 int  rtggx_debug_sky_runs(rtggx_context* ctx, uint32_t* runs, uint32_t capacity, uint32_t* tiles_x, uint32_t* tiles_y, uint32_t* threshold);
+int  rtggx_debug_settled_sky(rtggx_context* ctx, int enable);
+int  rtggx_debug_settled_words(rtggx_context* ctx, uint32_t* words0, uint32_t* words1, uint32_t capacity, uint32_t* blocks_x, uint32_t* blocks_y, uint32_t* epoch);
 int  rtggx_debug_collapse_weights(rtggx_context* ctx, const float* set, float* get);
 int  rtggx_debug_fence_wait(rtggx_context* ctx, double* us_total, uint32_t* waits, int reset);
 
diff --git a/raytracedggx_amd/capi.py b/raytracedggx_amd/capi.py
--- a/raytracedggx_amd/capi.py
+++ b/raytracedggx_amd/capi.py
@@ -28,7 +28,7 @@
            "rtggx_transform_sh", "rtggx_render_visibility", "rtggx_ray_trace", "rtggx_denoise", "rtggx_tone_map", "rtggx_sync",
            "rtggx_ray_count", "rtggx_get_timings", "rtggx_enable_timing", "rtggx_buffer_size", "rtggx_readback", "rtggx_buffer_ptr",
            "rtggx_upload", "rtggx_frame_parity", "rtggx_bvh_root", "rtggx_trace_rays", "rtggx_ray_total", "rtggx_kernel_times", "rtggx_debug_counters", "rtggx_debug_trace_split", "rtggx_debug_trace_residency", "rtggx_get_stream", "rtggx_set_history_peers", "rtggx_history_ipc_export", "rtggx_history_ipc_open",
-           "rtggx_set_async_compute", "rtggx_set_history_apron", "rtggx_history_overreach", "rtggx_copy_bandwidth", "rtggx_refit_as", "rtggx_refit_as_device", "rtggx_refit_stats", "rtggx_set_refit_policy", "rtggx_set_sampler", "rtggx_set_ray_rate", "rtggx_set_max_recursion_depth", "rtggx_set_samples_per_pixel", "rtggx_debug_fuse_tone_map", "rtggx_debug_placement", "rtggx_debug_tile_words", "rtggx_debug_static_sky", "rtggx_debug_sky_runs", "rtggx_debug_collapse_weights", "rtggx_debug_fence_wait", "rtggx_debug_shader_clock", "rtggx_debug_environment",
+           "rtggx_set_async_compute", "rtggx_set_history_apron", "rtggx_history_overreach", "rtggx_copy_bandwidth", "rtggx_refit_as", "rtggx_refit_as_device", "rtggx_refit_stats", "rtggx_set_refit_policy", "rtggx_set_sampler", "rtggx_set_ray_rate", "rtggx_set_max_recursion_depth", "rtggx_set_samples_per_pixel", "rtggx_debug_fuse_tone_map", "rtggx_debug_placement", "rtggx_debug_tile_words", "rtggx_debug_static_sky", "rtggx_debug_settled_sky", "rtggx_debug_settled_words", "rtggx_debug_sky_runs", "rtggx_debug_collapse_weights", "rtggx_debug_fence_wait", "rtggx_debug_shader_clock", "rtggx_debug_environment",
            "rtggx_set_accumulation", "rtggx_reset_accumulation", "rtggx_accumulated_frames", "rtggx_present_accumulation", "rtggx_set_sample_set",
            "rtggx_set_reference", "rtggx_reference_from_accumulation", "rtggx_set_scoring", "rtggx_read_scores",
            "rtggx_set_env_image", "rtggx_generate_env_mips"]
@@ -210,6 +210,18 @@
         self._check(self.L.rtggx_debug_sky_runs(self.h, _p(runs), tiles, C.byref(tx), C.byref(ty), C.byref(th)))
         return runs[:tx.value * ty.value].reshape(ty.value, tx.value), int(th.value)
 
+    def settled_sky(self, enable):
+        self.L.rtggx_debug_settled_sky.argtypes = [C.c_void_p, C.c_int]
+        self._check(self.L.rtggx_debug_settled_sky(self.h, 1 if enable else 0))
+
+    def settled_words(self):
+        n = ((self.W + 63) // 64) * ((self.H + 3) // 4)
+        w = np.zeros((2, n), np.uint32)
+        bx, by, ep = C.c_uint32(), C.c_uint32(), C.c_uint32()
+        self.L.rtggx_debug_settled_words.argtypes = [C.c_void_p, C.c_void_p, C.c_void_p, C.c_uint32, C.c_void_p, C.c_void_p, C.c_void_p]
+        self._check(self.L.rtggx_debug_settled_words(self.h, _p(w[0]), _p(w[1]), n, C.byref(bx), C.byref(by), C.byref(ep)))
+        return np.ascontiguousarray(w.reshape(2, bx.value, by.value).transpose(0, 2, 1)), int(ep.value)
+
     def placement(self, force_small=-1):
         k, w = C.c_uint32(), C.c_uint32()
         self.L.rtggx_debug_placement.argtypes = [C.c_void_p, C.c_int, C.c_void_p, C.c_void_p]
diff --git a/raytracedggx_amd/csrc/context.hip b/raytracedggx_amd/csrc/context.hip
--- a/raytracedggx_amd/csrc/context.hip
+++ b/raytracedggx_amd/csrc/context.hip
@@ -26,6 +26,14 @@
 int uploadParams(rtggx_context* c, uint32_t slot, hipStream_t s) {
   hipLaunchKernelGGL(uploadParamsKernel, dim3(1), dim3(64), 0, s, c->slots[slot], c->dParams + slot);
   RT_HIP(hipGetLastError());
+  return 0;
+}
+int resetSettled(rtggx_context* c) {
+  for (auto& w : c->settled) {
+    RT_HIP(hipMemset(w, 0xFF, c->settledWords() * 4));
+    RT_HIP(hipMemset2D(w + c->settledPitch + 1u, (size_t)c->settledPitch * 4, 0, (size_t)c->settledY * 4, c->settledX));
+  }
+  RT_HIP(hipStreamSynchronize(nullptr));
   return 0;
 }
 int allocSet(rtggx_context* c, uint32_t i) {
@@ -74,6 +82,10 @@
   for (uint32_t i = 0; i < RT_SETS; ++i) { const int r = allocSet(c, i); if (r) return r; }
   for (auto& v : c->vis) { RT_HIP(allocFilled(v.depth, n)); RT_HIP(allocFilled(v.dirty, c->skyTiles, 0xFF)); }
   RT_HIP(allocFilled(c->visDirtyOnes, c->skyTiles, 0xFF));
+  c->settledX = (width + 63) / 64; c->settledY = (height + 3) / 4;
+  c->settledPitch = (c->settledY + 3u) / 4u * 4u + 2u;
+  for (auto& w : c->settled) RT_HIP(alloc(w, c->settledWords()));
+  { const int r = resetSettled(c); if (r) return r; }
   RT_HIP(allocFilled(c->backbuffer, n));
   RT_HIP(allocFilled(c->tss[0], n)); RT_HIP(allocFilled(c->tss[1], n)); RT_HIP(allocFilled(c->fltRfl, n)); RT_HIP(allocFilled(c->fltDff, n));
   RT_HIP(allocFilled(c->rayCounter, 512));
diff --git a/raytracedggx_amd/csrc/debug.hip b/raytracedggx_amd/csrc/debug.hip
--- a/raytracedggx_amd/csrc/debug.hip
+++ b/raytracedggx_amd/csrc/debug.hip
@@ -66,6 +66,25 @@
   if (tilesX) *tilesX = c->skyGen.tilesX;
   if (tilesY) *tilesY = c->skyGen.tilesY;
   if (threshold) *threshold = RT_SKY_PREV_RUN + 1u;
+  return 0;
+}
+int rtggx_debug_settled_sky(rtggx_context* c, int enable) {
+  RT_CHECK_CTX(c);
+  c->settledSky = enable != 0;
+  c->breakSkyRuns();
+  return 0;
+}
+int rtggx_debug_settled_words(rtggx_context* c, uint32_t* words0, uint32_t* words1, uint32_t capacity, uint32_t* blocksX, uint32_t* blocksY, uint32_t* epoch) {
+  RT_CHECK_CTX(c);
+  const uint32_t n = c->settledX * c->settledY;
+  if (!words0 || !words1 || capacity < n) { setError("rtggx_debug_settled_words: room for %u words each", n); return -1; }
+  RT_HIP(syncStreams(c));
+  uint32_t* const out[2] = {words0, words1};
+  for (int p = 0; p < 2 && n; ++p)
+    RT_HIP(hipMemcpy2D(out[p], (size_t)c->settledY * 4, c->settled[p] + c->settledPitch + 1u, (size_t)c->settledPitch * 4, (size_t)c->settledY * 4, c->settledX, hipMemcpyDeviceToHost));
+  if (blocksX) *blocksX = c->settledX;
+  if (blocksY) *blocksY = c->settledY;
+  if (epoch) *epoch = c->skyEpoch;
   return 0;
 }
 int rtggx_debug_placement(rtggx_context* c, int forceSmall, uint32_t* key, uint32_t* where) {
diff --git a/raytracedggx_amd/csrc/denoise.hip b/raytracedggx_amd/csrc/denoise.hip
--- a/raytracedggx_amd/csrc/denoise.hip
+++ b/raytracedggx_amd/csrc/denoise.hip
@@ -41,6 +41,7 @@
   int outBegin, outEnd;
   const uint32_t* tileWords; int tilesX, tileRow0;
   const uint32_t* skyRun; uint32_t skyEpoch;
+  uint32_t* settledOut; const uint32_t* settledIn; uint32_t settledPitch;
 };
 #define RT_SGPR(v) ((uint32_t)__builtin_amdgcn_readfirstlane((int)(v)))
 RT_DEV uint32_t tileWordsOr(const uint32_t* words, uint32_t i0, uint32_t i1, uint32_t i2, uint32_t i3) {
@@ -66,6 +67,21 @@
 #pragma unroll
   for (int k = 0; k < 6; ++k) run = min(run, (w[k] >> 8) == epoch ? w[k] & 0xFFu : 0u);
   return run;
+}
+
+typedef uint32_t U2 __attribute__((ext_vector_type(2)));
+typedef uint32_t U4 __attribute__((ext_vector_type(4)));
+RT_DEV void loadTemporalWords(const uint32_t* rowA, const uint32_t* rowB, const uint32_t* col0, const uint32_t* col1, const uint32_t* col2,
+                              U4& a4, U2& a2, U4& b4, U2& b2, U4& c0, U4& c1, U4& c2) {
+  asm volatile("s_load_dwordx4 %0, %7, 0x0\n\ts_load_dwordx2 %1, %7, 0x10\n\ts_load_dwordx4 %2, %8, 0x0\n\ts_load_dwordx2 %3, %8, 0x10\n\t"
+               "s_load_dwordx4 %4, %9, 0x0\n\ts_load_dwordx4 %5, %10, 0x0\n\ts_load_dwordx4 %6, %11, 0x0\n\ts_waitcnt lgkmcnt(0)"
+               : "=&s"(a4), "=&s"(a2), "=&s"(b4), "=&s"(b2), "=&s"(c0), "=&s"(c1), "=&s"(c2)
+               : "s"(rowA), "s"(rowB), "s"(col0), "s"(col1), "s"(col2) : "memory");
+}
+RT_DEV void loadToneMapWords(const uint32_t* col0, const uint32_t* col1, const uint32_t* col2, U4& a4, U2& a2, U4& b4, U2& b2, U4& c4, U2& c2) {
+  asm volatile("s_load_dwordx4 %0, %6, 0x0\n\ts_load_dwordx2 %1, %6, 0x10\n\ts_load_dwordx4 %2, %7, 0x0\n\ts_load_dwordx2 %3, %7, 0x10\n\t"
+               "s_load_dwordx4 %4, %8, 0x0\n\ts_load_dwordx2 %5, %8, 0x10\n\ts_waitcnt lgkmcnt(0)"
+               : "=&s"(a4), "=&s"(a2), "=&s"(b4), "=&s"(b2), "=&s"(c4), "=&s"(c2) : "s"(col0), "s"(col1), "s"(col2) : "memory");
 }
 
 #define RT_LOG2E 1.44269504088896341f
@@ -437,17 +453,58 @@
     velSq[t / PITCH][t % PITCH] = vx * vx + vy * vy;
   }
 }
+RT_DEV bool settledWord(uint32_t w, uint32_t epoch) { return (w & ~RT_SETTLED_SKIPPED) == ((epoch << 8) | RT_SETTLED) || w == RT_SETTLED_BORDER; }
 #define RT_TP_ROWS 4
+template <bool WORDS>
 __global__ void __launch_bounds__(256) temporalKernel(Targets T) {
   __shared__ float4 tile[RT_TP_ROWS + 2][66];
   __shared__ uint32_t velRaw[RT_TP_ROWS + 2][66];
   __shared__ float velSq[RT_TP_ROWS + 2][66];
+  const uint32_t wordAt = (blockIdx.x + 1u) * T.settledPitch + blockIdx.y + 1u;
+  bool windowSky = false;
+  if (WORDS && T.settledIn != nullptr) {
+    const int bx = (int)blockIdx.x, by = (int)blockIdx.y;
+    const int txa = max(bx * 64 - 1, 0) >> 4, txb = min(bx * 64 + 64, T.W - 1) >> 4, tx0 = min(txa, T.tilesX - 6);
+    const int tya = max(by * RT_TP_ROWS - 1, 0) >> 4, tyb = min(by * RT_TP_ROWS + RT_TP_ROWS, T.H - 1) >> 4;
+    const uint32_t* col = T.settledIn + (uint32_t)bx * T.settledPitch + (uint32_t)by;
+    U4 a4, b4, c0, c1, c2; U2 a2, b2;
+    loadTemporalWords(T.skyRun + tya * T.tilesX + tx0, T.skyRun + tyb * T.tilesX + tx0, col, col + T.settledPitch, col + 2u * T.settledPitch, a4, a2, b4, b2, c0, c1, c2);
+    const uint32_t ra[6] = {a4.x, a4.y, a4.z, a4.w, a2.x, a2.y}, rb[6] = {b4.x, b4.y, b4.z, b4.w, b2.x, b2.y};
+    uint32_t run = RT_SKY_RUN_CAP;
+#pragma unroll
+    for (int k = 0; k < 6; ++k) {
+      const bool inWindow = tx0 + k >= txa && tx0 + k <= txb;
+      const uint32_t r = min((ra[k] >> 8) == T.skyEpoch ? ra[k] & 0xFFu : 0u, (rb[k] >> 8) == T.skyEpoch ? rb[k] & 0xFFu : 0u);
+      run = min(run, inWindow ? r : RT_SKY_RUN_CAP);
+    }
+    windowSky = run >= RT_SKY_WINDOW_RUN;
+    const uint32_t w[9] = {c0.x, c0.y, c0.z, c1.x, c1.y, c1.z, c2.x, c2.y, c2.z};
+    bool skip = windowSky;
+#pragma unroll
+    for (int k = 0; k < 9; ++k) skip = skip & settledWord(w[k], T.skyEpoch);
+    if (skip) {
+      if (threadIdx.x == 0) T.settledOut[wordAt] = (T.skyEpoch << 8) | RT_SETTLED | RT_SETTLED_SKIPPED;
+      return;
+    }
+  }
   stageTemporalTiles<RT_TP_ROWS + 2, 66, 256>(T, tile, velRaw, velSq, (int)blockIdx.x * 64 - 1, T.rowBegin + (int)blockIdx.y * RT_TP_ROWS - 1);
   __syncthreads();
   const int lx = (threadIdx.x & 63) + 1, ly = (threadIdx.x >> 6) + 1;
   const int x = blockIdx.x * 64 + (threadIdx.x & 63), y = T.rowBegin + blockIdx.y * RT_TP_ROWS + (threadIdx.x >> 6);
-  if (x >= T.W || y >= T.rowEnd) return;
-  T.scratch[(size_t)y * T.W + x] = temporalPixel<RT_TP_ROWS + 2, 66>(T, tile, velRaw, velSq, x, y, lx, ly);
+  bool equal = true;
+  if (x < T.W && y < T.rowEnd) {
+    const size_t pix = (size_t)y * T.W + x;
+    uint2 inPlace = make_uint2(0u, 0u);
+    if (WORDS && windowSky) inPlace = T.history[pix];
+    const uint2 out = temporalPixel<RT_TP_ROWS + 2, 66>(T, tile, velRaw, velSq, x, y, lx, ly);
+    T.scratch[pix] = out;
+#ifndef RT_SETTLED_NO_COMPARE
+    equal = inPlace.x == out.x && inPlace.y == out.y;
+#endif
+  }
+  if (!WORDS || T.settledOut == nullptr) return;
+  const uint32_t flag = windowSky && __syncthreads_and(equal ? 1 : 0) ? RT_SETTLED : 0u;
+  if (threadIdx.x == 0) T.settledOut[wordAt] = (T.skyEpoch << 8) | flag;
 }
 
 #ifndef RT_TT_TW
@@ -496,10 +553,22 @@
 #ifndef RT_TM_ROWS
 #define RT_TM_ROWS 16
 #endif
+template <bool WORDS>
 __global__ void __launch_bounds__(256) toneMapKernel(Targets T) {
 #pragma clang fp contract(fast)
   __shared__ float4 tile[RT_TM_ROWS + 2][66];
   const int W = T.W, H = T.H;
+  if (WORDS && T.settledIn != nullptr) {
+    static_assert(RT_TM_ROWS == 4 * RT_TP_ROWS, "a tone-map block is four blocks of the temporal pass high");
+    const uint32_t* col = T.settledIn + blockIdx.x * T.settledPitch + blockIdx.y * 4u;
+    U4 a4, b4, c4; U2 a2, b2, c2;
+    loadToneMapWords(col, col + T.settledPitch, col + 2u * T.settledPitch, a4, a2, b4, b2, c4, c2);
+    const uint32_t w[18] = {a4.x, a4.y, a4.z, a4.w, a2.x, a2.y, b4.x, b4.y, b4.z, b4.w, b2.x, b2.y, c4.x, c4.y, c4.z, c4.w, c2.x, c2.y};
+    bool skip = true;
+#pragma unroll
+    for (int k = 0; k < 18; ++k) skip = skip & settledWord(w[k], T.skyEpoch);
+    if (skip) return;
+  }
   {
     const int ox = blockIdx.x * 64 - 1, oy = T.rowBegin + blockIdx.y * RT_TM_ROWS - 1;
     constexpr int N = (RT_TM_ROWS + 2) * 66, PER = (N + 255) / 256;
@@ -553,6 +622,7 @@
   { uint32_t gb, ge; passRows(fp, ROWS_GBUFFER, gb, ge);
     T.tileWords = c->tileWords(gb, ge); T.tilesX = (int)((fp.W + 15) / 16); T.tileRow0 = (int)gb; }
   T.skyRun = nullptr; T.skyEpoch = 0u;
+  T.settledOut = nullptr; T.settledIn = nullptr; T.settledPitch = c->settledPitch;
   return T;
 }
 
@@ -566,6 +636,23 @@
                    && was.rows[0] == now.rows[0] && was.rows[1] == now.rows[1] && was.fltRflNull == now.fltRflNull;
   c->skyV = now;
   *epoch = c->skyEpoch;
+  return may;
+}
+
+static bool skyTemporalMaySkip(rtggx_context* c, const Targets& TT, const FrameParams& fp, bool fused, bool* words) {
+  rtggx_context::SkyT now;
+  const rtggx_context::SkyT& was = c->skyT;
+  const bool whole = fp.rowBegin == 0u && fp.rowEnd == fp.H && fp.W == c->W && fp.H == c->H;
+  const bool genValid = c->skyGen.any && c->skyGen.frame == c->frameCounter && c->skyGen.epoch == c->skyEpoch && c->skyGen.rows[0] == (uint32_t)TT.tileRow0;
+  now.any = true; now.frame = c->frameCounter; now.epoch = c->skyEpoch; now.parity = c->frameParity;
+  now.words = c->staticSky && c->settledSky && !fused && whole && fp.W >= 96u
+              && was.any && was.epoch == now.epoch;
+  now.rows[0] = (uint32_t)TT.rowBegin; now.rows[1] = (uint32_t)TT.rowEnd;
+  const bool may = now.words && genValid && was.words && was.frame + 1u == now.frame && was.parity == (now.parity ^ 1u)
+                   && was.rows[0] == now.rows[0] && was.rows[1] == now.rows[1];
+  c->skyT = now;
+  ++c->tssWrites[now.parity];
+  *words = now.words;
   return may;
 }
 
@@ -597,10 +684,16 @@
     hipLaunchKernelGGL(spatialDirectKernel<2>, grid(TH, 64, 4), block, 0, s, TH); mark(6);
     hipLaunchKernelGGL(spatialDirectKernel<3>, grid(TV, 64, 4), block, 0, s, TV); mark(7);
   }
+  Targets TTs = TT;
+  { bool words;
+    const bool may = skyTemporalMaySkip(c, TT, fp, fuseToneMap, &words);
+    if (words) { TTs.settledOut = c->settled[c->frameParity]; TTs.skyEpoch = c->skyEpoch; }
+    if (may) { TTs.settledIn = c->settled[c->frameParity ^ 1u]; TTs.skyRun = c->cur().skyRun; } }
   if (fuseToneMap) {
     const dim3 g((fp.W + RT_TT_W - 1) / RT_TT_W, (uint32_t)(TT.outEnd - TT.outBegin + RT_TT_H - 1) / RT_TT_H), b(RT_TT_TW * RT_TT_TH);
     launch(temporalToneKernel, g, b, s, nullptr, done, TT);
-  } else launch(temporalKernel, grid(TT, 64, RT_TP_ROWS), block, s, nullptr, done, TT);
+    c->skyTM.any = false;
+  } else launch(TTs.settledOut ? temporalKernel<true> : temporalKernel<false>, grid(TT, 64, RT_TP_ROWS), block, s, nullptr, done, TTs);
   mark(8);
   RT_HIP(hipGetLastError());
   return 0;
@@ -610,8 +703,18 @@
   if (fp.rowEnd <= fp.rowBegin) return 0;
   Targets T = makeTargets(c, fp, ROWS_FINAL);
   if (source) T.scratch = const_cast<uint2*>(source);
+  { rtggx_context::SkyTM now;
+    now.any = true; now.fromTss = source == nullptr; now.frame = c->frameCounter; now.epoch = c->skyEpoch; now.parity = c->frameParity; now.writes = c->tssWrites[c->frameParity];
+    now.rows[0] = (uint32_t)T.rowBegin; now.rows[1] = (uint32_t)T.rowEnd;
+    const rtggx_context::SkyTM& was = c->skyTM; const rtggx_context::SkyT& t = c->skyT;
+    const bool whole = fp.rowBegin == 0u && fp.rowEnd == fp.H && fp.W == c->W && fp.H == c->H;
+    const bool may = c->staticSky && c->settledSky && whole && now.fromTss && t.any && t.words && t.frame == now.frame && t.parity == now.parity && t.epoch == now.epoch
+                     && was.any && was.fromTss && was.frame + 1u == now.frame && was.epoch == now.epoch && was.rows[0] == now.rows[0] && was.rows[1] == now.rows[1]
+                     && was.parity == (now.parity ^ 1u) && was.writes == c->tssWrites[now.parity ^ 1u];
+    c->skyTM = now;
+    if (may) { T.settledIn = c->settled[c->frameParity]; T.skyEpoch = c->skyEpoch; } }
   const dim3 grid((fp.W + 63) / 64, (uint32_t)(T.rowEnd - T.rowBegin + RT_TM_ROWS - 1) / RT_TM_ROWS), block(256);
-  launch(toneMapKernel, grid, block, s, nullptr, done, T);
+  launch(T.settledIn ? toneMapKernel<true> : toneMapKernel<false>, grid, block, s, nullptr, done, T);
   RT_HIP(hipGetLastError());
   return 0;
 }
diff --git a/raytracedggx_amd/csrc/raytrace.hip b/raytracedggx_amd/csrc/raytrace.hip
--- a/raytracedggx_amd/csrc/raytrace.hip
+++ b/raytracedggx_amd/csrc/raytrace.hip
@@ -866,6 +866,7 @@
   if (c->skyEpochWrapped) {
     RT_HIP(hipDeviceSynchronize());
     for (auto& st : c->sets) RT_HIP(hipMemset(st.skyRun, 0, c->skyTiles * 4));
+    { const int r = resetSettled(c); if (r) return r; }
     RT_HIP(hipStreamSynchronize(nullptr));
     c->skyEpochWrapped = false;
   }
diff --git a/raytracedggx_amd/csrc/rtggx_context.h b/raytracedggx_amd/csrc/rtggx_context.h
--- a/raytracedggx_amd/csrc/rtggx_context.h
+++ b/raytracedggx_amd/csrc/rtggx_context.h
@@ -18,6 +18,10 @@
 #define RT_VIS_CLEAR 0x00FFFFFF00000000ull
 #define RT_SKY_PREV_RUN (RT_SETS + 2)
 #define RT_SKY_V_RUN 2u
+#define RT_SKY_WINDOW_RUN 1u
+#define RT_SETTLED 1u
+#define RT_SETTLED_SKIPPED 2u
+#define RT_SETTLED_BORDER 0xFFFFFFFFu
 #define RT_SKY_RUN_CAP 255u
 namespace rt {
 
@@ -229,6 +233,12 @@
   void breakSkyRuns() { skyEpoch = (skyEpoch + 1u) & 0xFFFFFFu; if (skyEpoch == 0u) skyEpochWrapped = true; }
   struct SkyGen { bool any = false, adaptive = false; uint32_t frame = 0, epoch = 0, rows[2] = {0, 0}, rate = 0, sliceShift = 0, tilesX = 0, tilesY = 0; hipStream_t stream = nullptr; float camera[20] = {}; } skyGen;
   struct SkyV { bool any = false, fltRflNull = false; uint32_t frame = 0, genEpoch = 0, rows[2] = {0, 0}; } skyV;
+  bool settledSky = true;
+  rt::DevBuf<uint32_t> settled[2]; uint32_t settledX = 0, settledY = 0, settledPitch = 0;
+  size_t settledWords() const { return (size_t)(settledX + 2u) * settledPitch + 8u; }
+  struct SkyT { bool any = false, words = false; uint32_t frame = 0, epoch = 0, parity = 0, rows[2] = {0, 0}; } skyT;
+  struct SkyTM { bool any = false, fromTss = false; uint32_t frame = 0, epoch = 0, parity = 0, writes = 0, rows[2] = {0, 0}; } skyTM;
+  uint32_t tssWrites[2] = {0, 0};
   bool useTileWords = true;
   bool traversalBound = false;
   const uint32_t* traceTileWords = nullptr;
@@ -318,6 +328,7 @@
 int launchReferenceFromAccumulation(rtggx_context* c, hipStream_t s);
 int launchTraceRays(rtggx_context* c, const FrameParams& fp, const float* dRays, uint32_t n, float* dOut, hipStream_t s);
 int launchDebugEnvironment(rtggx_context* c, const float* dDirs, const float* dLevels, uint32_t n, int level0, float* dOut, hipStream_t s);
+int resetSettled(rtggx_context* c);
 int launchDenoise(rtggx_context* c, const FrameParams& fp, int useLds, hipStream_t s, hipEvent_t done = nullptr, bool fuseToneMap = false);
 int launchToneMap(rtggx_context* c, const FrameParams& fp, hipStream_t s, hipEvent_t done = nullptr, const uint2* source = nullptr);
 int decodeEnv(rtggx_context* c, int format, uint32_t size, uint32_t mips, const void* hostData, size_t bytes, hipStream_t s);
```

New measurement: 3306 Mrays/s, median of 6. +4.4%, better.
